# TigreGotico/phoonnx

Measured on AMD Instinct MI355X. Metric: audio samples/sec (22.05 kHz), batch-32 256-phoneme utterances, higher is better.
Workload: dtype f32 (f16x3 split: fp32 operands as two fp16 planes, three MFMA products, fp32 accumulate)

## Files before the change

include/vitsmi.h:

```cpp
#ifndef VITSMI_H
#define VITSMI_H

#include <stddef.h>
#include <stdint.h>

#ifdef __cplusplus
extern "C" {
#endif

typedef struct vits_handle vits_handle;

enum {
    VITS_OK = 0,
    VITS_E_IO = -1,
    VITS_E_FORMAT = -2,
    VITS_E_ARG = -3,
    VITS_E_DEVICE = -4,
    VITS_E_NOMEM = -5,
    VITS_E_RANGE = -6
};

#define VITS_MAX_DIMS 4


// ... 280 lines not shown
                                        vits_enc_chunk_fn fn, void *user);

typedef struct vits_stream_onset {
    int32_t mode;
    float threshold;
    int32_t keep_lead;
    int32_t reserved;
} vits_stream_onset;
typedef int (*vits_enc_chunk_trim_fn)(void *user, const void *bytes, int B, int64_t row_pitch_bytes, int64_t first_sample,
                                      int64_t n_samples, const int32_t *valid, const int32_t *skip, const float *peak,
                                      int64_t total_samples);
int vits_stream_onset_check(const vits_stream_onset *onsets, const vits_stream_format *fmt, int B);
int vits_stream_onset_start(int64_t f, int64_t keep_lead, int64_t delivered_before, int64_t *a);
int vits_run_chunked_enc_trimmed(vits_handle *h, const int64_t *ids, const int64_t *lens, int B, int T, const int64_t *sid,
                                 const vits_noise *noise, const vits_controls *ctl, const vits_stream_format *fmt,
                                 const vits_stream_shaping *shaping, const vits_stream_onset *onsets, int chunk_frames,
                                 vits_enc_chunk_trim_fn fn, void *user);
int vits_run_vocoder_chunked_enc_trimmed(vits_handle *h, const float *z, int B, int F, const int64_t *sid,
                                         const vits_stream_format *fmt, const vits_stream_shaping *shaping,
                                         const vits_stream_onset *onsets, int chunk_frames, vits_enc_chunk_trim_fn fn, void *user);

int vits_warp_emit_end(const vits_warp_seg *segs, int n_segs, int64_t n_in, int64_t n_out, int64_t X, int64_t *ready);
int vits_glide_emit_end(const vits_glide_seg *segs, int n_segs, int64_t n_in, int64_t n_out, int64_t X, int64_t *ready);
int64_t vits_warp_stream_cap(int64_t piece_samples, int64_t S_w);
int vits_run_chunked_glided(vits_handle *h, const int64_t *ids, const int64_t *lens, int B, int T, const int64_t *sid,
                            const vits_noise *noise, const vits_controls *ctl, const vits_contour *contour, int chunk_frames,
                            vits_chunk_fn fn, void *user);
int vits_run_chunked_enc_glided(vits_handle *h, const int64_t *ids, const int64_t *lens, int B, int T, const int64_t *sid,
                                const vits_noise *noise, const vits_controls *ctl, const vits_stream_format *fmt,
                                const vits_stream_shaping *shaping, const vits_stream_onset *onsets, const vits_contour *contour,
                                int chunk_frames, vits_enc_chunk_trim_fn fn, void *user);

enum { VITS_FIT_MET = 0, VITS_FIT_FLOOR = 1, VITS_FIT_CEIL = 2, VITS_FIT_KEPT = 3 };
typedef struct {
    const int32_t *group;
    int n_groups;
    const int64_t *target_frames;
    const int32_t *mode;
} vits_fit;
int vits_fit_plan(const float *w, const int64_t *lens, int B, int T, const vits_fit *fit, int64_t *durations, double *scale,
                  int64_t *frames, int32_t *status);
int vits_run_async_fitted(vits_handle *h, const int64_t *ids, const int64_t *lens, int B, int T, const int64_t *sid,
                          const vits_noise *noise, const vits_controls *ctl, const vits_fit *fit);
int vits_run_chunked_fitted(vits_handle *h, const int64_t *ids, const int64_t *lens, int B, int T, const int64_t *sid,
                            const vits_noise *noise, const vits_controls *ctl, const vits_fit *fit, int chunk_frames,
                            vits_chunk_fn fn, void *user);
int vits_run_chunked_enc_fitted(vits_handle *h, const int64_t *ids, const int64_t *lens, int B, int T, const int64_t *sid,
                                const vits_noise *noise, const vits_controls *ctl, const vits_stream_format *fmt,
                                const vits_stream_shaping *shaping, const vits_stream_onset *onsets, const vits_fit *fit,
                                int chunk_frames, vits_enc_chunk_trim_fn fn, void *user);
int vits_last_fit(vits_handle *h, double *scale, int64_t *frames, int32_t *status, int n);

int vits_reserve(vits_handle *h, int B, int T, int F);
int vits_get_stats(vits_handle *h, vits_stats *out);

typedef struct {
    char kernel[128];
    double flops, bytes;
    float ms;
    int stage;
    int cin, cout, k, dil, t;
} vits_launch_record;
int vits_launch_records(vits_handle *h, vits_launch_record *buf, int n);

void *vits_stream(vits_handle *h);


int vits_test_conv1d(int device_id, const float *x, int B, int Cin, int T, const float *w, const float *bias,
                     int Cout, int K, int dil, int pad_l, int flags, float slope, float *out);
int vits_bench_conv1d(int device_id, int B, int Cin, int Cout, int T, int K, int dil, int hint, int iters,
                      int cfg_override, int ck_override, float *ms_out);
int vits_test_conv_transpose1d(int device_id, const float *x, int B, int Cin, int T, const float *w,
                               const float *bias, int Cout, int K, int stride, float *out);
enum {
    VITS_CONV_PRO_LRELU = 1, VITS_CONV_PRO_MASK = 2, VITS_CONV_EPI_RELU = 4, VITS_CONV_EPI_MASK = 8, VITS_CONV_EPI_RES = 16,
    VITS_CONV_EPI_ACC = 32, VITS_CONV_EPI_DIV = 64, VITS_CONV_EPI_COUPLING = 128, VITS_CONV_EPI_WN = 256,
    VITS_CONV_EPI_WN_FIRST = 512
};
typedef struct {
    int B, Cin, T, Cout;
    int K, dil, pad_l;
    int stride;
    int hint, cfg, ck;
    int flags;
    float slope, div, oslope, oslope2;
    int wn_split;
    const float *x;
    const float *w, *bias;
    const int64_t *lens;
    const float *bias_b;
    int bias_b_stride;
    const float *res;
    int x_cstride;
    int out_cstride;
    int out_rows, out_row0;
    const float *old_out, *old_out2;
    float sentinel;
    float *out, *out2;
    int pl_rows;
    float *planes_out;
    char kernel[128];
    int cfg_used, ck_used;
} vits_test_conv_epi_args;
int vits_test_conv1d_epi(int device_id, vits_test_conv_epi_args *a);
int vits_test_wn_gate(int device_id, const float *a, int B, int H, int T, int form, float *acts);
int vits_test_cond_matvec(int device_id, const float *emb_g, int n_speakers, int gin, const int64_t *sid, int B,
                          const float *W, const float *bias, int rows, float *out);
int vits_test_conv1d_sx(int device_id, const float *x, int B, int Cin, int T, const float *w, const float *bias,
                        int Cout, int K, int dil, int pad_l, int flags, float slope, float *out);
enum { VITS_SX_EPI_RES = 1, VITS_SX_EPI_ACC = 2, VITS_SX_EPI_DIV = 4, VITS_SX_EPI_NO_RAW_STORE = 8 };
enum { VITS_SX_BF16X6 = 0, VITS_SX_F16X3 = 1, VITS_SX_F16 = 2 };
typedef struct {
    int B, Cin, T, Cout;
    int K, dil, pad_l;
    int stride;
    int precision;
    int force16, no_s16, min_cfg;
    int run_cfg;
    int flags;
    const float *x;
    const float *w, *bias;
    const float *res;
    int res_is_x;
    int res_planes;
    float res_slope;
    const float *old_out;
    const float *bias_b;
    int bias_b_stride;
    float div, oslope, oslope2, islope;
    const int64_t *lens;
    int rag_add, rag_mul;
    float sentinel;
    float *out;
    float *planes_out;
    float *res_seen;
    char kernel[128];
    int pack_cfg, run_cfg_used, rawin, s16, ck;
    float peak;
} vits_test_conv_sx_epi_args;
int vits_test_conv1d_sx_epi(int device_id, vits_test_conv_sx_epi_args *a);
int vits_test_conv1d_sx_planar(int device_id, const float *x, int B, int Cin, int T, const float *w, const float *bias,
                               int Cout, int K, int dil, int flags, const int64_t *lens, const float *old, int row_split,
                               int pl_rows, float *out, float *planes_out);
long long vits_test_set_sx_small_max(long long wgs);
int vits_test_conv1d_sx_gate(int device_id, const float *x, int B, int Cin, int T, const float *w, const float *bias,
                             const float *bias_b, int Cout, int K, int dil, int flags, float *out);
int vits_test_conv_transpose1d_sx(int device_id, const float *x, int B, int Cin, int T, const float *w,
                                  const float *bias, int Cout, int K, int stride, float *out);
int vits_bench_conv1d_sx(int device_id, int B, int Cin, int Cout, int T, int K, int dil, int dbg, int iters,
                         float *ms_out);
int vits_test_conv_pair_sx(int device_id, const float *x, int B, int C, int T, const float *w1, const float *b1,
                           const float *w2, const float *b2, int K, int dil1, int dil2, int chain, float slope, float *out,
                           float *ms_out);
enum { VITS_P16_EPI_ACC = 1, VITS_P16_EPI_DIV = 2, VITS_P16_EPI_RAW = 4, VITS_P16_EPI_PLANES = 8 };
typedef struct {
    int B, C, T, K, dil1, dil2, chain;
    int precision;
    int flags;
    float slope, div, sentinel;
    const float *x;
    const float *w1, *b1, *w2, *b2;
    const float *old_out;
    const float *x_tail;
    const int64_t *lens;
    int rag_add, rag_mul;
    float *out;
    float *planes_out;
    float *x_seen;
    float *ms_out;
    char kernel[128];
    int BN, BNo, ovl;
    float peak;
    int guard_ok;
} vits_test_conv_pair16_epi_args;
int vits_test_conv_pair16_epi(int device_id, vits_test_conv_pair16_epi_args *a);
int vits_test_attention(int device_id, const float *qkv, int B, int C, int T, int n_heads, const float *rel_k,
                        const float *rel_v, int window, const int64_t *lens, float *out);
int vits_test_attention16(int device_id, const float *qkv, int B, int C, int T, int n_heads, const float *rel_k,
                          const float *rel_v, int window, const int64_t *lens, float *out, uint16_t *out_planes, int kernel,
                          int reps, float *ms_out);
typedef struct {
    int kernel;
    const float *qkv;
    const uint16_t *qkv_planes;
    int B, C, T, n_heads, window;
    const float *rel_k, *rel_v;
    const int64_t *lens;
    int want_out;
    int want_planes;
    int ns, qt;
    int kh;
    float *out;
    uint16_t *out_planes;
    float peak;
    char kernel_name[128];
} vits_test_attention_form_args;
int vits_test_attention_form(int device_id, vits_test_attention_form_args *a);

int vits_test_resample(int device_id, const float *x, const int64_t *lens, int B, int S, int in_rate, int out_rate, float *y,
                       int64_t S_out);
int vits_test_resample_pieces(int device_id, const float *x, const int64_t *lens, int B, int S, int in_rate, int out_rate,
                              int piece_samples, float *y, int64_t S_out, int64_t *ranges, int max_ranges);
int vits_test_resample_rows(int device_id, const float *x, const int64_t *lens, int B, int S, int in_rate,
                            const int32_t *out_rates, float *y, size_t y_elems, int64_t *n_out);
int vits_test_warp(int device_id, const float *x, const int64_t *counts, int B, int S, const vits_warp_seg *segs,
                   const int32_t *seg_first , float *y, int S_w);
int vits_test_glide(int device_id, const float *x, const int64_t *counts, int B, int S, const vits_glide_seg *segs,
                    const int32_t *seg_first , float *y, int S_w);
int vits_test_warp_pieces(int device_id, const float *x, const int64_t *counts, int B, int S, const vits_warp_seg *segs,
                          const int32_t *seg_first , const int64_t *piece_bounds, int n_pieces, float *y, int S_w,
                          int64_t *ranges, int max_ranges);
int vits_test_glide_pieces(int device_id, const float *x, const int64_t *counts, int B, int S, const vits_glide_seg *segs,
                           const int32_t *seg_first , const int64_t *piece_bounds, int n_pieces, float *y, int S_w,
                           int64_t *ranges, int max_ranges);

int vits_test_durations(int device_id, const float *logw, const int64_t *dur, const int64_t *lens, int B, int T, float length_scale,
                        const float *rows, const float *token_rate, float *w_ceil, int32_t *cum, int32_t *y_len);
int vits_test_fit_durations(int device_id, const float *w, const int64_t *lens, int B, int T, const vits_fit *fit, float *w_ceil,
                            int32_t *cum, int32_t *y_len, double *scale, int64_t *frames, int32_t *status);
int vits_test_expand_prior(int device_id, const float *m_logs, int B, int C, int T, const int32_t *cum, const int64_t *lens,
                           const int32_t *y_len, int F, const float *noise, int64_t noise_stride, int noise_frames,
                           float noise_scale, const float *rows, const uint64_t *seeds, float *z_p);
int vits_test_fill_normal(int device_id, int64_t n, uint64_t seed, uint64_t stream_id, float *out);
int vits_test_fill_normal_rows(int device_id, int B, int channels, int T, const uint64_t *seeds, uint32_t stream, const float *rows,
                               int col, float *out);
int vits_test_post_conv(int device_id, const float *x, int B, int C, int T, const float *w, int K, float slope, const int64_t *vlen,
                        int hop, int kernel, float *out);

int vits_test_layernorm(int device_id, const float *x, const float *out_init, int B, int C, int T, const float *gamma,
                        const float *beta, const int64_t *lens, int flags, int form, int in_place, const float *dw_w,
                        const float *dw_b, int K, int dil, float *out, uint16_t *planes);
typedef struct vits_test_dds_layer {
    const float *dw_w, *dw_b;
    const float *ln1_g, *ln1_b;
    const float *pw_w, *pw_b;
    const float *ln2_g, *ln2_b;
    int32_t dil;
} vits_test_dds_layer;
int vits_test_dds(int device_id, int form, const float *x, int B, int C, int T, const int64_t *lens, int n_layers,
                  const vits_test_dds_layer *layers, int mask_out, const float *head_cond, const float *head_z, int head_ch,
                  const float *head_w, const float *head_b, const float *tail_w, const float *tail_b, int tail_rows, float *out);
int vits_test_cf_pre(int device_id, const float *z, int ch, const float *w, const float *bias, const float *cond, int B, int C, int T,
                     float *out);
int vits_test_rqs_inverse(int device_id, const float *pr, const float *z, int B, int T, const int64_t *lens, int ch0, int nb,
                          float sqrt_c, float *out);
int vits_test_ea_logw(int device_id, const float *z, int ch, float m0, float logs0, const int64_t *lens, int B, int T, float *out);

int vits_test_deliver(int device_id, const float *x, const int64_t *counts, int B, int S, const vits_segment *segs, int n_segs,
                      int n_streams, int encoding, void *dst, size_t dst_bytes, int64_t *stream_samples, int64_t *stream_offsets);

int vits_test_deliver_trimmed(int device_id, const float *x, const int64_t *counts, int B, int S, const vits_segment *segs,
                              const vits_trim *trims, int n_segs, int n_streams, int encoding, void *dst, size_t dst_bytes,
                              int64_t *stream_samples, int64_t *stream_offsets, int64_t *kept_first, int64_t *kept_count);

int vits_test_loudness_blocks(int device_id, const float *x, const int64_t *counts, const int64_t *firsts, int B, int S,
                              int sample_rate, float *e, size_t e_cap, int32_t *n_sub, int32_t *chunk);

int vits_test_deliver_leveled(int device_id, const float *x, const int64_t *counts, int B, int S, const vits_segment *segs,
                              const vits_trim *trims, const vits_level *levels, int n_segs, int n_streams, int encoding,
                              int sample_rate, void *dst, size_t dst_bytes, int64_t *stream_samples, int64_t *stream_offsets,
                              int64_t *kept_first, int64_t *kept_count, double *loudness, float *gain);

int vits_test_deliver_shaped(int device_id, const float *x, const int64_t *counts, int B, int S, const vits_segment *segs,
                             const vits_trim *trims, const vits_level *levels, const vits_shape *shapes, const vits_env_point *points,
                             int64_t n_points, int n_segs, int n_streams, int encoding, int sample_rate, void *dst, size_t dst_bytes,
                             int64_t *stream_samples, int64_t *stream_offsets, int64_t *kept_first, int64_t *kept_count,
                             double *loudness, float *gain);

int vits_test_deliver_limited(int device_id, const float *x, const int64_t *counts, int B, int S, const vits_segment *segs,
                              const vits_trim *trims, const vits_level *levels, const vits_shape *shapes, const vits_env_point *points,
                              int64_t n_points, const vits_limit *limits, int n_segs, int n_streams, int encoding, int sample_rate,
                              void *dst, size_t dst_bytes, int64_t *stream_samples, int64_t *stream_offsets, int64_t *kept_first,
                              int64_t *kept_count, double *loudness, float *gain);

int vits_test_stream_pack(int device_id, const float *x, const int64_t *counts, int B, int S, int piece_samples,
                          const vits_stream_format *fmt, void *bytes, size_t bytes_cap, int64_t *pitches, int32_t *valid,
                          float *peaks, int max_pieces);

int vits_test_stream_pack_shaped(int device_id, const float *x, const int64_t *counts, int B, int S, int piece_samples,
                                 const vits_stream_format *fmt, const vits_stream_shaping *shaping, void *bytes, size_t bytes_cap,
                                 int64_t *pitches, int32_t *valid, float *peaks, int64_t *firsts, int64_t *ns, int max_pieces);

int vits_test_stream_pack_trimmed(int device_id, const float *x, const int64_t *counts, int B, int S, int piece_samples,
                                  const vits_stream_format *fmt, const vits_stream_shaping *shaping, const vits_stream_onset *onsets,
                                  void *bytes, size_t bytes_cap, int64_t *pitches, int32_t *valid, int32_t *skip, float *peaks,
                                  int64_t *firsts, int64_t *ns, int32_t *start, int max_pieces);

#ifdef __cplusplus
}
#endif
#endif
```

phoonnx_amd/_ffi.py:

```python
import ctypes as C
import os

import numpy as np

from . import audio_encoding

_HERE = os.path.dirname(os.path.abspath(__file__))
_LIB = None

VITS_MAX_DIMS = 4


class VitsNoise(C.Structure):
    _fields_ = [("noise_dp", C.c_void_p), ("noise_z", C.c_void_p), ("noise_z_stride", C.c_int64),
                ("seed", C.c_uint64)]


class VitsOutput(C.Structure):
    _fields_ = [("data", C.POINTER(C.c_float)), ("dims", C.c_int64 * 4), ("y_lengths", C.POINTER(C.c_int64))]


class VitsStats(C.Structure):
    _fields_ = [("conv_flops", C.c_double), ("conv_bytes", C.c_double), ("dec_flops", C.c_double),
                ("dec_bytes", C.c_double), ("flow_flops", C.c_double), ("enc_flops", C.c_double),
                ("dp_flops", C.c_double), ("conv_ms", C.c_float), ("dec_ms", C.c_float), ("flow_ms", C.c_float),
                ("enc_ms", C.c_float), ("dp_ms", C.c_float), ("total_ms", C.c_float), ("conv_launches", C.c_int),
                ("total_launches", C.c_int), ("sx_flops", C.c_double), ("sx_ms", C.c_float), ("sx_launches", C.c_int),
                ("f16_peak_max", C.c_float), ("f16_peak_min", C.c_float), ("f16_tracked", C.c_int),
                ("f16_saturated", C.c_int), ("sx_bytes", C.c_double)]


class VitsLaunchRecord(C.Structure):
    _fields_ = [("kernel", C.c_char * 128), ("flops", C.c_double), ("bytes", C.c_double), ("ms", C.c_float),
                ("stage", C.c_int), ("cin", C.c_int), ("cout", C.c_int), ("k", C.c_int), ("dil", C.c_int), ("t", C.c_int)]


class VitsTestConvEpiArgs(C.Structure):
    _fields_ = [(n, C.c_int) for n in ("B", "Cin", "T", "Cout", "K", "dil", "pad_l", "stride", "hint", "cfg", "ck", "flags")] + \
               [(n, C.c_float) for n in ("slope", "div", "oslope", "oslope2")] + [("wn_split", C.c_int)] + \
               [(n, C.c_void_p) for n in ("x", "w", "bias", "lens", "bias_b")] + [("bias_b_stride", C.c_int), ("res", C.c_void_p)] + \
               [(n, C.c_int) for n in ("x_cstride", "out_cstride", "out_rows", "out_row0")] + \
               [("old_out", C.c_void_p), ("old_out2", C.c_void_p), ("sentinel", C.c_float), ("out", C.c_void_p), ("out2", C.c_void_p),
                ("pl_rows", C.c_int), ("planes_out", C.c_void_p), ("kernel", C.c_char * 128), ("cfg_used", C.c_int), ("ck_used", C.c_int)]


class VitsTestConvSxEpiArgs(C.Structure):
    _fields_ = [(n, C.c_int) for n in ("B", "Cin", "T", "Cout", "K", "dil", "pad_l", "stride", "precision", "force16", "no_s16",
                                       "min_cfg", "run_cfg", "flags")] + \
               [(n, C.c_void_p) for n in ("x", "w", "bias", "res")] + \
               [("res_is_x", C.c_int), ("res_planes", C.c_int), ("res_slope", C.c_float), ("old_out", C.c_void_p),
                ("bias_b", C.c_void_p), ("bias_b_stride", C.c_int)] + \
               [(n, C.c_float) for n in ("div", "oslope", "oslope2", "islope")] + \
               [("lens", C.c_void_p), ("rag_add", C.c_int), ("rag_mul", C.c_int), ("sentinel", C.c_float), ("out", C.c_void_p),
                ("planes_out", C.c_void_p), ("res_seen", C.c_void_p), ("kernel", C.c_char * 128)] + \
               [(n, C.c_int) for n in ("pack_cfg", "run_cfg_used", "rawin", "s16", "ck")] + [("peak", C.c_float)]


class VitsTestConvPair16EpiArgs(C.Structure):
    _fields_ = [(n, C.c_int) for n in ("B", "C", "T", "K", "dil1", "dil2", "chain", "precision", "flags")] + \
               [(n, C.c_float) for n in ("slope", "div", "sentinel")] + \
               [(n, C.c_void_p) for n in ("x", "w1", "b1", "w2", "b2", "old_out", "x_tail", "lens")] + \
               [("rag_add", C.c_int), ("rag_mul", C.c_int)] + \
               [(n, C.c_void_p) for n in ("out", "planes_out", "x_seen", "ms_out")] + [("kernel", C.c_char * 128)] + \
               [(n, C.c_int) for n in ("BN", "BNo", "ovl")] + [("peak", C.c_float), ("guard_ok", C.c_int)]


class VitsTestAttentionFormArgs(C.Structure):
    _fields_ = [("kernel", C.c_int), ("qkv", C.c_void_p), ("qkv_planes", C.c_void_p)] + \
               [(n, C.c_int) for n in ("B", "C", "T", "n_heads", "window")] + \
               [(n, C.c_void_p) for n in ("rel_k", "rel_v", "lens")] + \
               [(n, C.c_int) for n in ("want_out", "want_planes", "ns", "qt", "kh")] + \
               [("out", C.c_void_p), ("out_planes", C.c_void_p), ("peak", C.c_float), ("kernel_name", C.c_char * 128)]


class VitsOpenOptions(C.Structure):
    _fields_ = [("device_id", C.c_int), ("gen_precision", C.c_char_p), ("arena_dev", C.c_void_p),
                ("arena_bytes", C.c_size_t), ("host_only", C.c_int), ("layout_only", C.c_int)]


class VitsControls(C.Structure):
    _fields_ = [("scales_rows", C.c_void_p), ("seeds", C.c_void_p), ("durations", C.c_void_p), ("token_rate", C.c_void_p)]


class VitsFit(C.Structure):
    _fields_ = [("group", C.c_void_p), ("n_groups", C.c_int), ("target_frames", C.c_void_p), ("mode", C.c_void_p)]


VITS_FIT_MET, VITS_FIT_FLOOR, VITS_FIT_CEIL, VITS_FIT_KEPT = 0, 1, 2, 3


class VitsWarpSeg(C.Structure):
    _fields_ = [("n0", C.c_int64), ("pos0", C.c_int64), ("k", C.c_int64), ("step", C.c_int32), ("c", C.c_int32),
                ("half_taps", C.c_int32), ("pad_", C.c_int32)]


class VitsIntonation(C.Structure):
    _fields_ = [("token_semitones", C.c_void_p), ("compensate", C.c_int)]


class VitsGlideSeg(C.Structure):
    _fields_ = [("n0", C.c_int64), ("pos0", C.c_int64), ("k", C.c_int64), ("step0", C.c_int32), ("step1", C.c_int32),
                ("pad_", C.c_int32 * 2)]


class VitsContour(C.Structure):
    _fields_ = [("token_semitones", C.c_void_p), ("token_semitones_end", C.c_void_p), ("compensate", C.c_int)]


class VitsSegment(C.Structure):
    _fields_ = [("row", C.c_int32), ("stream", C.c_int32), ("lead_samples", C.c_int64), ("normalize", C.c_int32),
                ("volume", C.c_float)]


class VitsTrim(C.Structure):
    _fields_ = [("mode", C.c_int32), ("threshold", C.c_float), ("keep_lead", C.c_int32), ("keep_tail", C.c_int32),
                ("tail_samples", C.c_int64)]


class VitsTestDdsLayer(C.Structure):
    _fields_ = [("dw_w", C.c_void_p), ("dw_b", C.c_void_p), ("ln1_g", C.c_void_p), ("ln1_b", C.c_void_p), ("pw_w", C.c_void_p),
                ("pw_b", C.c_void_p), ("ln2_g", C.c_void_p), ("ln2_b", C.c_void_p), ("dil", C.c_int32)]


class VitsLevel(C.Structure):
    _fields_ = [("mode", C.c_int32), ("target_lufs", C.c_float), ("max_gain_db", C.c_float), ("peak_ceiling", C.c_float)]


class VitsEnvPoint(C.Structure):
    _fields_ = [("pos", C.c_int32), ("gain", C.c_float)]


class VitsShape(C.Structure):
    _fields_ = [("fade_in", C.c_int32), ("fade_out", C.c_int32), ("curve", C.c_int32), ("n_points", C.c_int32),
                ("first_point", C.c_int64)]


class VitsLimit(C.Structure):
    _fields_ = [("mode", C.c_int32), ("ceiling", C.c_float), ("lookahead", C.c_int32), ("reserved", C.c_int32)]


class VitsStreamFormat(C.Structure):
    _fields_ = [("encoding", C.c_int32), ("ref_peak", C.c_void_p), ("volume", C.c_void_p)]


class VitsStreamShaping(C.Structure):
    pass


STREAM_PLAN_FN = C.CFUNCTYPE(C.c_int, C.c_void_p, C.c_int, C.c_int, C.POINTER(C.c_int64), C.POINTER(C.c_int64), C.POINTER(VitsStreamShaping))

VitsStreamShaping._fields_ = [("shapes", C.c_void_p), ("points", C.c_void_p), ("n_points", C.c_int64), ("ceiling", C.c_void_p),
                              ("lookahead", C.c_int32), ("reserved", C.c_int32), ("plan", STREAM_PLAN_FN), ("plan_user", C.c_void_p)]


class VitsStreamOnset(C.Structure):
    _fields_ = [("mode", C.c_int32), ("threshold", C.c_float), ("keep_lead", C.c_int32), ("reserved", C.c_int32)]


ENCODINGS = {name: (code, audio_encoding.DTYPES[name]) for code, name in enumerate(audio_encoding.ENCODINGS)}


CHUNK_FN = C.CFUNCTYPE(C.c_int, C.c_void_p, C.POINTER(C.c_float), C.c_int, C.c_int64, C.c_int64, C.c_int64)

ENC_CHUNK_FN = C.CFUNCTYPE(C.c_int, C.c_void_p, C.c_void_p, C.c_int, C.c_int64, C.c_int64, C.c_int64, C.POINTER(C.c_int32),
                           C.POINTER(C.c_float), C.c_int64)

ENC_CHUNK_TRIM_FN = C.CFUNCTYPE(C.c_int, C.c_void_p, C.c_void_p, C.c_int, C.c_int64, C.c_int64, C.c_int64, C.POINTER(C.c_int32),
                                C.POINTER(C.c_int32), C.POINTER(C.c_float), C.c_int64)

VITS_E_RANGE = -6


EXPORTS = [
    "vits_open", "vits_open_with_arena", "vits_open_host", "vits_open_layout", "vits_open_opts", "vits_close",
    "vits_run_chunked", "vits_run_vocoder_chunked", "vits_last_error", "vits_num_inputs",
    "vits_input_name", "vits_meta", "vits_hparam", "vits_arena_bytes", "vits_arena_host", "vits_arena_device",
    "vits_run", "vits_free_output", "vits_run_device", "vits_sync", "vits_last_y_lengths", "vits_last_pcm16", "vits_run_vocoder",
    "vits_tap",
    "vits_set_timing", "vits_set_tails", "vits_reserve", "vits_get_stats", "vits_stream", "vits_test_conv1d", "vits_test_conv_transpose1d",
    "vits_test_attention", "vits_test_attention16", "vits_bench_conv1d", "vits_test_conv1d_sx", "vits_test_conv1d_sx_planar", "vits_test_conv1d_sx_gate", "vits_test_set_sx_small_max",
    "vits_test_conv_transpose1d_sx",
    "vits_bench_conv1d_sx", "vits_test_conv_pair_sx", "vits_fetch_output", "vits_run_async", "vits_host_alloc", "vits_host_free",
    "vits_launch_records", "vits_run_async_rows", "vits_run_device_rows", "vits_run_chunked_rows",
    "vits_run_async_ctl", "vits_run_chunked_ctl", "vits_last_durations",
    "vits_set_output_rate", "vits_last_sample_counts", "vits_resample_plan", "vits_test_resample", "vits_test_resample_pieces",
    "vits_set_output_rates", "vits_last_sample_rates", "vits_test_resample_rows",
    "vits_run_async_warped", "vits_last_token_spans", "vits_warp_token", "vits_warp_plan", "vits_test_warp",
    "vits_run_async_glided", "vits_glide_token", "vits_glide_cutoff", "vits_glide_plan", "vits_test_glide",
    "vits_warp_emit_end", "vits_glide_emit_end", "vits_warp_stream_cap", "vits_run_chunked_glided", "vits_run_chunked_enc_glided",
    "vits_test_warp_pieces", "vits_test_glide_pieces",
    "vits_fit_plan", "vits_run_async_fitted", "vits_run_chunked_fitted", "vits_run_chunked_enc_fitted", "vits_last_fit",
    "vits_test_fit_durations",
    "vits_test_durations", "vits_test_expand_prior", "vits_test_fill_normal", "vits_test_fill_normal_rows", "vits_test_post_conv",
    "vits_delivery_plan", "vits_deliver", "vits_test_deliver",
    "vits_trim_range", "vits_delivery_plan_trimmed", "vits_deliver_trimmed", "vits_test_deliver_trimmed",
    "vits_loudness_filter", "vits_loudness_gate", "vits_level_gain", "vits_delivery_plan_leveled", "vits_deliver_leveled",
    "vits_test_loudness_blocks", "vits_test_deliver_leveled",
    "vits_shape_check", "vits_shape_gain", "vits_deliver_shaped", "vits_test_deliver_shaped",
    "vits_limit_check", "vits_limit_gains", "vits_deliver_limited", "vits_test_deliver_limited",
    "vits_run_chunked_enc", "vits_run_vocoder_chunked_enc", "vits_test_stream_pack",
    "vits_stream_shaping_check", "vits_stream_emit_range", "vits_run_chunked_enc_shaped", "vits_run_vocoder_chunked_enc_shaped",
    "vits_test_stream_pack_shaped",
    "vits_stream_onset_check", "vits_stream_onset_start", "vits_run_chunked_enc_trimmed", "vits_run_vocoder_chunked_enc_trimmed",
    "vits_test_stream_pack_trimmed",
    "vits_test_layernorm", "vits_test_dds", "vits_test_cf_pre", "vits_test_rqs_inverse", "vits_test_ea_logw",
    "vits_test_conv1d_epi", "vits_test_wn_gate", "vits_test_cond_matvec", "vits_test_conv1d_sx_epi",
    "vits_test_conv_pair16_epi", "vits_test_attention_form",
]


G2P_EXPORTS = ["g2p_open", "g2p_close", "g2p_last_error", "g2p_hparam", "g2p_num_outputs", "g2p_output_name", "g2p_bucket",
               "g2p_run", "g2p_generate", "g2p_generate_batch", "g2p_test_forced_steps", "g2p_test_linear", "g2p_test_step"]


def lib_path():
    return os.environ.get("VITSMI_LIB") or os.path.join(_HERE, "libvitsmi.so")


def load():
    global _LIB
    if _LIB is not None:
        return _LIB
    path = lib_path()
    if not os.environ.get("VITSMI_LIB"):
        from . import build as _build
        if _build.stale():
            try:
                _build.build()
            except Exception as e:
                raise RuntimeError(f"{path} is missing or was not built from the sources in this tree (source_sha "
                                   f"{_build.source_sha()} vs recorded {_build.read_build_info().get('source_sha')}) "
                                   f"and cannot be rebuilt here: {e}") from e
    lib = C.CDLL(path)
    vp, i64p, f32p = C.c_void_p, C.POINTER(C.c_int64), C.POINTER(C.c_float)
    lib.vits_open.argtypes = [C.c_char_p, C.c_int, C.POINTER(vp)]
    lib.vits_open_with_arena.argtypes = [C.c_char_p, C.c_int, vp, C.c_size_t, C.POINTER(vp)]
    lib.vits_open_host.argtypes = [C.c_char_p, C.POINTER(vp)]
    lib.vits_open_layout.argtypes = [C.c_char_p, C.POINTER(vp)]
    lib.vits_open_opts.argtypes = [C.c_char_p, C.POINTER(VitsOpenOptions), C.POINTER(vp)]
    lib.vits_run_chunked.argtypes = [vp, vp, vp, C.c_int, C.c_int, vp, vp, C.POINTER(VitsNoise), C.c_int, CHUNK_FN, vp]
    lib.vits_run_vocoder_chunked.argtypes = [vp, vp, C.c_int, C.c_int, vp, C.c_int, CHUNK_FN, vp]
    lib.vits_close.argtypes = [vp]
    lib.vits_close.restype = None
    lib.vits_last_error.argtypes = [vp]
    lib.vits_last_error.restype = C.c_char_p
    lib.vits_num_inputs.argtypes = [vp]
    lib.vits_input_name.argtypes = [vp, C.c_int]
    lib.vits_input_name.restype = C.c_char_p
    lib.vits_meta.argtypes = [vp, C.c_char_p, C.c_char_p, C.c_size_t]
    lib.vits_hparam.argtypes = [vp, C.c_char_p, i64p]
    lib.vits_arena_bytes.argtypes = [vp]
    lib.vits_arena_bytes.restype = C.c_size_t
    lib.vits_arena_host.argtypes = [vp]
    lib.vits_arena_host.restype = vp
    lib.vits_arena_device.argtypes = [vp]
    lib.vits_arena_device.restype = vp
    run_args = [vp, vp, vp, C.c_int, C.c_int, vp, vp, C.POINTER(VitsNoise), C.POINTER(VitsOutput)]
    lib.vits_run.argtypes = run_args
    lib.vits_run_device.argtypes = run_args
    lib.vits_run_async.argtypes = run_args[:-1]
    lib.vits_run_async_rows.argtypes = run_args[:-1] + [vp]
    lib.vits_run_device_rows.argtypes = run_args[:-1] + [vp, C.POINTER(VitsOutput)]
    lib.vits_run_chunked_rows.argtypes = [vp, vp, vp, C.c_int, C.c_int, vp, vp, C.POINTER(VitsNoise), vp, C.c_int, CHUNK_FN, vp]
    lib.vits_run_async_ctl.argtypes = [vp, vp, vp, C.c_int, C.c_int, vp, C.POINTER(VitsNoise), C.POINTER(VitsControls)]
    lib.vits_run_chunked_ctl.argtypes = [vp, vp, vp, C.c_int, C.c_int, vp, C.POINTER(VitsNoise), C.POINTER(VitsControls),
                                         C.c_int, CHUNK_FN, vp]
    lib.vits_run_chunked_enc.argtypes = [vp, vp, vp, C.c_int, C.c_int, vp, C.POINTER(VitsNoise), C.POINTER(VitsControls),
                                         C.POINTER(VitsStreamFormat), C.c_int, ENC_CHUNK_FN, vp]
    lib.vits_run_vocoder_chunked_enc.argtypes = [vp, vp, C.c_int, C.c_int, vp, C.POINTER(VitsStreamFormat), C.c_int, ENC_CHUNK_FN, vp]
    lib.vits_stream_shaping_check.argtypes = [C.POINTER(VitsStreamShaping), C.POINTER(VitsStreamFormat), C.c_int]
    lib.vits_stream_emit_range.argtypes = [C.c_int64, C.c_int64, C.c_int, C.c_int64, C.c_int, i64p, i64p]
    lib.vits_run_chunked_enc_shaped.argtypes = [vp, vp, vp, C.c_int, C.c_int, vp, C.POINTER(VitsNoise), C.POINTER(VitsControls),
                                                C.POINTER(VitsStreamFormat), C.POINTER(VitsStreamShaping), C.c_int, ENC_CHUNK_FN, vp]
    lib.vits_run_vocoder_chunked_enc_shaped.argtypes = [vp, vp, C.c_int, C.c_int, vp, C.POINTER(VitsStreamFormat),
                                                        C.POINTER(VitsStreamShaping), C.c_int, ENC_CHUNK_FN, vp]
    lib.vits_test_stream_pack_shaped.argtypes = [C.c_int, vp, vp, C.c_int, C.c_int, C.c_int, C.POINTER(VitsStreamFormat),
                                                 C.POINTER(VitsStreamShaping), vp, C.c_size_t, vp, vp, vp, vp, vp, C.c_int]
    lib.vits_stream_onset_check.argtypes = [C.POINTER(VitsStreamOnset), C.POINTER(VitsStreamFormat), C.c_int]
    lib.vits_stream_onset_start.argtypes = [C.c_int64, C.c_int64, C.c_int64, i64p]
    lib.vits_run_chunked_enc_trimmed.argtypes = [vp, vp, vp, C.c_int, C.c_int, vp, C.POINTER(VitsNoise), C.POINTER(VitsControls),
                                                 C.POINTER(VitsStreamFormat), C.POINTER(VitsStreamShaping), C.POINTER(VitsStreamOnset),
                                                 C.c_int, ENC_CHUNK_TRIM_FN, vp]
    lib.vits_run_vocoder_chunked_enc_trimmed.argtypes = [vp, vp, C.c_int, C.c_int, vp, C.POINTER(VitsStreamFormat),
                                                         C.POINTER(VitsStreamShaping), C.POINTER(VitsStreamOnset), C.c_int,
                                                         ENC_CHUNK_TRIM_FN, vp]
    lib.vits_test_stream_pack_trimmed.argtypes = [C.c_int, vp, vp, C.c_int, C.c_int, C.c_int, C.POINTER(VitsStreamFormat),
                                                  C.POINTER(VitsStreamShaping), C.POINTER(VitsStreamOnset), vp, C.c_size_t, vp, vp, vp, vp,
                                                  vp, vp, vp, C.c_int]
    lib.vits_test_stream_pack.argtypes = [C.c_int, vp, vp, C.c_int, C.c_int, C.c_int, C.POINTER(VitsStreamFormat), vp, C.c_size_t,
                                          vp, vp, vp, C.c_int]
    lib.vits_last_durations.argtypes = [vp, i64p, C.c_size_t]
    lib.vits_set_output_rate.argtypes = [vp, C.c_int, C.c_int]
    lib.vits_last_sample_counts.argtypes = [vp, i64p, C.c_int]
    lib.vits_resample_plan.argtypes = [C.c_int, C.c_int, i64p, i64p, i64p, vp, C.c_size_t]
    lib.vits_test_resample.argtypes = [C.c_int, vp, vp, C.c_int, C.c_int, C.c_int, C.c_int, vp, C.c_int64]
    lib.vits_test_resample_pieces.argtypes = [C.c_int, vp, vp, C.c_int, C.c_int, C.c_int, C.c_int, C.c_int, vp, C.c_int64, vp, C.c_int]
    lib.vits_set_output_rates.argtypes = [vp, C.c_int, vp, C.c_int]
    lib.vits_last_sample_rates.argtypes = [vp, vp, C.c_int]
    lib.vits_test_resample_rows.argtypes = [C.c_int, vp, vp, C.c_int, C.c_int, C.c_int, vp, vp, C.c_size_t, vp]
    lib.vits_run_async_warped.argtypes = [vp, vp, vp, C.c_int, C.c_int, vp, C.POINTER(VitsNoise), C.POINTER(VitsControls),
                                          C.POINTER(VitsIntonation)]
    lib.vits_last_token_spans.argtypes = [vp, i64p, C.c_size_t]
    lib.vits_warp_token.argtypes = [C.c_float, i64p, i64p, C.POINTER(C.c_int32)]
    lib.vits_warp_plan.argtypes = [vp, vp, C.c_int, C.c_int, vp, vp, i64p]
    lib.vits_test_warp.argtypes = [C.c_int, vp, vp, C.c_int, C.c_int, vp, vp, vp, C.c_int]
    lib.vits_run_async_glided.argtypes = [vp, vp, vp, C.c_int, C.c_int, vp, C.POINTER(VitsNoise), C.POINTER(VitsControls),
                                          C.POINTER(VitsContour)]
    lib.vits_glide_token.argtypes = [C.c_float, C.c_float, i64p, i64p, C.POINTER(C.c_float)]
    lib.vits_glide_cutoff.argtypes = [C.c_int64, i64p, C.POINTER(C.c_int32)]
    lib.vits_glide_plan.argtypes = [vp, vp, vp, C.c_int, C.c_int, vp, vp, i64p]
    lib.vits_test_glide.argtypes = [C.c_int, vp, vp, C.c_int, C.c_int, vp, vp, vp, C.c_int]
    for name in ("vits_warp_emit_end", "vits_glide_emit_end"):
        getattr(lib, name).argtypes = [vp, C.c_int, C.c_int64, C.c_int64, C.c_int64, i64p]
    lib.vits_warp_stream_cap.argtypes = [C.c_int64, C.c_int64]
    lib.vits_warp_stream_cap.restype = C.c_int64
    lib.vits_run_chunked_glided.argtypes = [vp, vp, vp, C.c_int, C.c_int, vp, C.POINTER(VitsNoise), C.POINTER(VitsControls),
                                            C.POINTER(VitsContour), C.c_int, CHUNK_FN, vp]
    lib.vits_run_chunked_enc_glided.argtypes = [vp, vp, vp, C.c_int, C.c_int, vp, C.POINTER(VitsNoise), C.POINTER(VitsControls),
                                                C.POINTER(VitsStreamFormat), C.POINTER(VitsStreamShaping), C.POINTER(VitsStreamOnset),
                                                C.POINTER(VitsContour), C.c_int, ENC_CHUNK_TRIM_FN, vp]
    for name in ("vits_test_warp_pieces", "vits_test_glide_pieces"):
        getattr(lib, name).argtypes = [C.c_int, vp, vp, C.c_int, C.c_int, vp, vp, vp, C.c_int, vp, C.c_int, vp, C.c_int]
    lib.vits_fit_plan.argtypes = [vp, vp, C.c_int, C.c_int, C.POINTER(VitsFit), vp, vp, vp, vp]
    lib.vits_run_async_fitted.argtypes = [vp, vp, vp, C.c_int, C.c_int, vp, C.POINTER(VitsNoise), C.POINTER(VitsControls),
                                          C.POINTER(VitsFit)]
    lib.vits_run_chunked_fitted.argtypes = [vp, vp, vp, C.c_int, C.c_int, vp, C.POINTER(VitsNoise), C.POINTER(VitsControls),
                                            C.POINTER(VitsFit), C.c_int, CHUNK_FN, vp]
    lib.vits_run_chunked_enc_fitted.argtypes = [vp, vp, vp, C.c_int, C.c_int, vp, C.POINTER(VitsNoise), C.POINTER(VitsControls),
                                                C.POINTER(VitsStreamFormat), C.POINTER(VitsStreamShaping), C.POINTER(VitsStreamOnset),
                                                C.POINTER(VitsFit), C.c_int, ENC_CHUNK_TRIM_FN, vp]
    lib.vits_last_fit.argtypes = [vp, vp, vp, vp, C.c_int]
    lib.vits_test_fit_durations.argtypes = [C.c_int, vp, vp, C.c_int, C.c_int, C.POINTER(VitsFit), vp, vp, vp, vp, vp, vp]
    lib.vits_test_durations.argtypes = [C.c_int, vp, vp, vp, C.c_int, C.c_int, C.c_float, vp, vp, vp, vp, vp]
    lib.vits_test_expand_prior.argtypes = [C.c_int, vp, C.c_int, C.c_int, C.c_int, vp, vp, vp, C.c_int, vp, C.c_int64, C.c_int,
                                           C.c_float, vp, vp, vp]
    lib.vits_test_fill_normal.argtypes = [C.c_int, C.c_int64, C.c_uint64, C.c_uint64, vp]
    lib.vits_test_fill_normal_rows.argtypes = [C.c_int, C.c_int, C.c_int, C.c_int, vp, C.c_uint32, vp, C.c_int, vp]
    lib.vits_test_post_conv.argtypes = [C.c_int, vp, C.c_int, C.c_int, C.c_int, vp, C.c_int, C.c_float, vp, C.c_int, C.c_int, vp]
    lib.vits_test_layernorm.argtypes = [C.c_int, vp, vp, C.c_int, C.c_int, C.c_int, vp, vp, vp, C.c_int, C.c_int, C.c_int, vp, vp,
                                        C.c_int, C.c_int, vp, vp]
    lib.vits_test_dds.argtypes = [C.c_int, C.c_int, vp, C.c_int, C.c_int, C.c_int, vp, C.c_int, C.POINTER(VitsTestDdsLayer), C.c_int,
                                  vp, vp, C.c_int, vp, vp, vp, vp, C.c_int, vp]
    lib.vits_test_cf_pre.argtypes = [C.c_int, vp, C.c_int, vp, vp, vp, C.c_int, C.c_int, C.c_int, vp]
    lib.vits_test_rqs_inverse.argtypes = [C.c_int, vp, vp, C.c_int, C.c_int, vp, C.c_int, C.c_int, C.c_float, vp]
    lib.vits_test_ea_logw.argtypes = [C.c_int, vp, C.c_int, C.c_float, C.c_float, vp, C.c_int, C.c_int, vp]
    lib.vits_delivery_plan.argtypes = [vp, C.c_int, vp, C.c_int, C.c_int, C.c_int, vp, vp, i64p]
    lib.vits_deliver.argtypes = [vp, vp, C.c_int, C.c_int, C.c_int, vp, C.c_size_t, vp, vp]
    lib.vits_test_deliver.argtypes = [C.c_int, vp, vp, C.c_int, C.c_int, vp, C.c_int, C.c_int, C.c_int, vp, C.c_size_t, vp, vp]
    lib.vits_trim_range.argtypes = [C.c_int64, C.c_int64, C.c_int64, C.POINTER(VitsTrim), i64p, i64p]
    lib.vits_delivery_plan_trimmed.argtypes = [vp, C.c_int, vp, vp, C.c_int, C.c_int, C.c_int, vp, vp, i64p]
    lib.vits_deliver_trimmed.argtypes = [vp, vp, vp, C.c_int, C.c_int, C.c_int, vp, C.c_size_t, vp, vp, vp, vp]
    lib.vits_test_deliver_trimmed.argtypes = [C.c_int, vp, vp, C.c_int, C.c_int, vp, vp, C.c_int, C.c_int, C.c_int, vp, C.c_size_t,
                                              vp, vp, vp, vp]
    lib.vits_loudness_filter.argtypes = [C.c_int, vp, vp]
    lib.vits_loudness_gate.argtypes = [vp, vp, C.c_int, C.c_int32, vp, vp, vp, vp]
    lib.vits_level_gain.argtypes = [C.c_double, C.c_float, C.POINTER(VitsLevel), C.POINTER(C.c_float)]
    lib.vits_delivery_plan_leveled.argtypes = [vp, C.c_int, vp, vp, vp, C.c_int, C.c_int, C.c_int, C.c_int, vp, vp, i64p]
    lib.vits_deliver_leveled.argtypes = [vp, vp, vp, vp, C.c_int, C.c_int, C.c_int, C.c_int, vp, C.c_size_t, vp, vp, vp, vp, vp, vp]
    lib.vits_test_loudness_blocks.argtypes = [C.c_int, vp, vp, vp, C.c_int, C.c_int, C.c_int, vp, C.c_size_t, vp, vp]
    lib.vits_test_deliver_leveled.argtypes = [C.c_int, vp, vp, C.c_int, C.c_int, vp, vp, vp, C.c_int, C.c_int, C.c_int, C.c_int, vp,
                                              C.c_size_t, vp, vp, vp, vp, vp, vp]
    lib.vits_shape_check.argtypes = [vp, C.c_int, vp, C.c_int64]
    lib.vits_shape_gain.argtypes = [C.POINTER(VitsShape), vp, C.c_int64, C.c_int64, C.c_int64, C.POINTER(C.c_float)]
    lib.vits_deliver_shaped.argtypes = [vp, vp, vp, vp, vp, vp, C.c_int64, C.c_int, C.c_int, C.c_int, C.c_int, vp, C.c_size_t, vp, vp, vp,
                                        vp, vp, vp]
    lib.vits_test_deliver_shaped.argtypes = [C.c_int, vp, vp, C.c_int, C.c_int, vp, vp, vp, vp, vp, C.c_int64, C.c_int, C.c_int, C.c_int,
                                             C.c_int, vp, C.c_size_t, vp, vp, vp, vp, vp, vp]
    lib.vits_limit_check.argtypes = [vp, vp, C.c_int]
    lib.vits_limit_gains.argtypes = [vp, C.c_int64, C.POINTER(VitsLimit), vp]
    lib.vits_deliver_limited.argtypes = [vp, vp, vp, vp, vp, vp, C.c_int64, vp, C.c_int, C.c_int, C.c_int, C.c_int, vp, C.c_size_t, vp,
                                         vp, vp, vp, vp, vp]
    lib.vits_test_deliver_limited.argtypes = [C.c_int, vp, vp, C.c_int, C.c_int, vp, vp, vp, vp, vp, C.c_int64, vp, C.c_int, C.c_int,
                                              C.c_int, C.c_int, vp, C.c_size_t, vp, vp, vp, vp, vp, vp]
    lib.vits_free_output.argtypes = [vp, C.POINTER(VitsOutput)]
    lib.vits_free_output.restype = None
    lib.vits_sync.argtypes = [vp]
    lib.vits_last_y_lengths.argtypes = [vp, i64p, C.c_int]
    lib.vits_last_pcm16.argtypes = [vp, C.c_int, C.c_float, vp, C.c_size_t]
    lib.vits_run_vocoder.argtypes = [vp, vp, C.c_int, C.c_int, vp, C.POINTER(VitsOutput)]
    lib.vits_tap.argtypes = [vp, C.c_char_p, vp, C.c_size_t, i64p]
    lib.vits_set_timing.argtypes = [vp, C.c_int]
    lib.vits_set_tails.argtypes = [vp, C.c_int]
    lib.vits_reserve.argtypes = [vp, C.c_int, C.c_int, C.c_int]
    lib.vits_get_stats.argtypes = [vp, C.POINTER(VitsStats)]
    lib.vits_stream.argtypes = [vp]
    lib.vits_stream.restype = vp
    lib.vits_fetch_output.argtypes = [vp, vp, C.c_size_t, C.c_size_t]
    lib.vits_host_alloc.argtypes = [C.c_size_t]
    lib.vits_host_alloc.restype = vp
    lib.vits_host_free.argtypes = [vp]
    lib.vits_host_free.restype = None
    lib.vits_launch_records.argtypes = [vp, C.POINTER(VitsLaunchRecord), C.c_int]
    lib.vits_test_conv1d.argtypes = [C.c_int, vp, C.c_int, C.c_int, C.c_int, vp, vp, C.c_int, C.c_int, C.c_int,
                                     C.c_int, C.c_int, C.c_float, vp]
    lib.vits_test_conv_transpose1d.argtypes = [C.c_int, vp, C.c_int, C.c_int, C.c_int, vp, vp, C.c_int, C.c_int,
                                               C.c_int, vp]
    lib.vits_test_attention.argtypes = [C.c_int, vp, C.c_int, C.c_int, C.c_int, C.c_int, vp, vp, C.c_int, vp, vp]
    lib.vits_test_attention16.argtypes = [C.c_int, vp, C.c_int, C.c_int, C.c_int, C.c_int, vp, vp, C.c_int, vp, vp, vp,
                                          C.c_int, C.c_int, f32p]
    lib.vits_bench_conv1d.argtypes = [C.c_int] * 11 + [f32p]
    lib.vits_test_conv1d_sx.argtypes = lib.vits_test_conv1d.argtypes
    lib.vits_test_conv_transpose1d_sx.argtypes = lib.vits_test_conv_transpose1d.argtypes
    lib.vits_test_conv1d_sx_planar.argtypes = [C.c_int, vp, C.c_int, C.c_int, C.c_int, vp, vp, C.c_int, C.c_int, C.c_int, C.c_int,
                                               vp, vp, C.c_int, C.c_int, vp, vp]
    lib.vits_test_set_sx_small_max.argtypes = [C.c_longlong]
    lib.vits_test_set_sx_small_max.restype = C.c_longlong
    lib.vits_test_conv1d_sx_gate.argtypes = [C.c_int, vp, C.c_int, C.c_int, C.c_int, vp, vp, vp, C.c_int, C.c_int, C.c_int, C.c_int, vp]
    lib.vits_bench_conv1d_sx.argtypes = [C.c_int] * 9 + [f32p]
    lib.vits_test_conv1d_epi.argtypes = [C.c_int, C.POINTER(VitsTestConvEpiArgs)]
    lib.vits_test_conv1d_sx_epi.argtypes = [C.c_int, C.POINTER(VitsTestConvSxEpiArgs)]
    lib.vits_test_conv_pair16_epi.argtypes = [C.c_int, C.POINTER(VitsTestConvPair16EpiArgs)]
    lib.vits_test_attention_form.argtypes = [C.c_int, C.POINTER(VitsTestAttentionFormArgs)]
    lib.vits_test_wn_gate.argtypes = [C.c_int, vp, C.c_int, C.c_int, C.c_int, C.c_int, vp]
    lib.vits_test_cond_matvec.argtypes = [C.c_int, vp, C.c_int, C.c_int, vp, C.c_int, vp, vp, C.c_int, vp]
    lib.vits_test_conv_pair_sx.argtypes = [C.c_int, vp, C.c_int, C.c_int, C.c_int, vp, vp, vp, vp, C.c_int, C.c_int,
                                           C.c_int, C.c_int, C.c_float, vp, f32p]
    lib.g2p_open.argtypes = [C.c_char_p, C.c_int, C.POINTER(vp)]
    lib.g2p_close.argtypes = [vp]
    lib.g2p_close.restype = None
    lib.g2p_last_error.argtypes = [vp]
    lib.g2p_last_error.restype = C.c_char_p
    lib.g2p_hparam.argtypes = [vp, C.c_char_p, i64p]
    lib.g2p_num_outputs.argtypes = [vp]
    lib.g2p_output_name.argtypes = [vp, C.c_int]
    lib.g2p_output_name.restype = C.c_char_p
    lib.g2p_bucket.argtypes = [vp, C.c_int, C.c_int]
    lib.g2p_run.argtypes = [vp, vp, C.c_int, vp, vp, C.c_int, vp]
    lib.g2p_generate.argtypes = [vp, vp, C.c_int, C.c_int, C.c_int64, C.c_int64, vp, C.POINTER(C.c_int)]
    lib.g2p_generate_batch.argtypes = [vp, vp, vp, C.c_int, C.c_int, C.c_int64, C.c_int64, vp, vp]
    lib.g2p_test_forced_steps.argtypes = [vp, vp, vp, C.c_int, vp, C.c_int, vp]
    lib.g2p_test_linear.argtypes = [C.c_int, C.c_int, vp, vp, C.c_int, vp, C.c_int, C.c_int, vp, C.c_int64, C.c_int64, C.c_int, vp]
    lib.g2p_test_step.argtypes = [C.c_int, C.c_int, C.c_int, vp, vp, vp, C.c_int, vp, vp, C.c_int, C.c_float, C.c_float, vp, vp]
    _LIB = lib
    return lib


def ptr(a):
    return None if a is None else a.ctypes.data_as(C.c_void_p)


def last_error(h=None):
    return load().vits_last_error(h).decode("utf-8", "replace")
```

phoonnx_amd/csrc/conv_sx_pair.hip.hpp:

```cpp
#pragma once
#include <cstdlib>
#include "conv_geom.hpp"
#include "conv_sx_engine.hip.hpp"

namespace vitsmi {

struct SxPairArgs {
    const float *xr;
    float islope, mslope;
    int T;
    const u32x4 *wp1, *wp2;
    const float *bias1, *bias2;
    float wscale1, wscale2;
    float *out_raw;
    const float *zeros;
    int C, nchunks;
    int K1, dil1, pad1;
    int K2, dil2, pad2;
    int LW1;
    unsigned x_bytes;
    int LW2;
    unsigned y_chunk_bytes;
    int BNo, NT, B;
    int flags;
    float div;
    unsigned *peak;
    struct Chain {
        const u32x4 *wp1, *wp2;
        const float *bias1, *bias2;
        float wscale1, wscale2;
        int K1, dil1, K2, dil2;
        int xoff, yoff;
    } ch[3];
    int nchain;
    unsigned a_ring;
    unsigned bias_off;
    unsigned long long *prof;
    SxRagged rag;
    int xgs = 0;
};

#ifndef SX_PAIR_PROF
#define SX_PAIR_PROF 0
#endif
#ifndef SX_PAIR_SHARED_A
#define SX_PAIR_SHARED_A 0
#endif
#ifndef SX_PAIR_ALIAS
#define SX_PAIR_ALIAS 0
#endif
#ifndef SX_PAIR_DEPTH32
#define SX_PAIR_DEPTH32 2
#endif
#ifndef SX_PAIR_DEPTH64
#define SX_PAIR_DEPTH64 2
#endif
#ifndef SX_PAIR_EARLY_ACC
#define SX_PAIR_EARLY_ACC 0
#endif
#ifndef SX_PAIR_WGS32
#define SX_PAIR_WGS32 3
#endif
#ifndef SX_PAIR_EARLY32
#define SX_PAIR_EARLY32 1
#endif
#ifndef SX_PAIR_ST_SC1
#define SX_PAIR_ST_SC1 0
#endif
#ifndef SX_PAIR_ONE_READ64
#define SX_PAIR_ONE_READ64 1
#endif
#ifndef SX_PAIR_ONE_READ32
#define SX_PAIR_ONE_READ32 1
#endif
template <int MW, int NW, int WM, int WN, int EPI, bool CHAIN, int NCH = 1>
__global__ __launch_bounds__(256, (NW == 2 && !SX_PAIR_EARLY_ACC && NCH == 1) ? SX_PAIR_WGS32 : 2) void conv_sx_pair_kernel(SxPairArgs a) {
    constexpr int BN = NW * WN * 32, NH = NW / 2;
    static_assert(NCH == 1 || (CHAIN && NW == 2 && (EPI & EPI_ACC) == 0), "fused chains: 32 channels, no external running sum");
    constexpr bool ONE_READ = NW == 4 ? SX_PAIR_ONE_READ64 != 0 : SX_PAIR_ONE_READ32 != 0;
    constexpr bool EARLY = ONE_READ || (NW == 2 && SX_PAIR_EARLY32);
    constexpr int DEPTH = NW == 2 ? SX_PAIR_DEPTH32 : SX_PAIR_DEPTH64;
    static_assert(DEPTH >= 2 && DEPTH <= 6, "wait_a covers up to five younger sets");
    constexpr bool ACC = (EPI & EPI_ACC) != 0 && SX_PAIR_EARLY_ACC;
    static_assert(!(ONE_READ && ACC), "the running sum is not pulled into the single-read prologue");
    static_assert(WM * WN == 4 && MW == 1 && BN == 256, "one block row per wave, 256 columns");
    constexpr int NPW = 2, STEPBYTES = WM * MW * NPW * 1024;
    constexpr int MAXCH = WM * 2;
    extern __shared__ __attribute__((aligned(16))) unsigned char lds_sx[];
    const int tid = threadIdx.x, lane = tid & 63;
    const int wave = __builtin_amdgcn_readfirstlane(tid >> 6);
    const int wm = wave / WN, wn = wave % WN;
    const int l31 = lane & 31, hi = lane >> 5;
    const int wg_xcd = blockIdx.x & 7, wg_seq = blockIdx.x >> 3;
    const int tile_nb = __builtin_amdgcn_readfirstlane(sx_xcd_tile(wg_seq, wg_xcd, a.xgs));
    if (tile_nb >= a.NT * a.B) return;
    const int b = tile_nb / a.NT, t0 = (tile_nb - b * a.NT) * a.BNo;
    const int t1 = t0 - a.pad2;
    const int T = a.T, LW = a.LW1;
    const int TV = __builtin_amdgcn_readfirstlane(sx_valid_cols(a.rag, b, T));
    if (t0 >= TV) return;
    const uint32_t lds0 = (uint32_t)(uintptr_t)lds_sx;
    const uint32_t XB = a.x_bytes;
    const char *wbase1 = reinterpret_cast<const char *>(a.wp1) + wm * (MW * NPW * 1024);
    const char *wbase2 = reinterpret_cast<const char *>(a.wp2) + wm * (MW * NPW * 1024);
    const float *xrb = a.xr + (int64_t)b * a.C * T;
    float pk = 0.f;

    struct ASet {
        u32x4 fa[2];
    };
    const uint32_t voff0 = (uint32_t)lane * 16u;
    auto load_a = [&](ASet &f, const char *wb, int step) {
        const char *sb = wb + (int64_t)step * STEPBYTES;
        f.fa[0] = global_read128<0>(voff0, sb);
        f.fa[1] = global_read128<1024>(voff0, sb);
    };

    f32x4 pre[NW / 2][2][4], ad[EARLY && ACC ? NW / 2 : 1][2][4];
    auto load_res = [&](const float *base, f32x4 (*dst)[2][4]) {
        static_for<NW / 2>([&](auto R) {
            constexpr int rr = decltype(R)::value;
#pragma unroll
            for (int j = 0; j < 2; j++) {
                const int row0 = wm * 32;
                const int t = t1 + (wn * NW + rr * 2 + j) * 32 + l31;
                const int tl = t < 0 ? 0 : (t < T ? t : T - 1);
#pragma unroll
                for (int q = 0; q < 4; q++) {
                    const float *p = base + ((int64_t)((row0 >> 3) + q) * T + tl) * 8 + 4 * hi;
                    if constexpr (EARLY) dst[rr][j][q] = __builtin_bit_cast(f32x4, global_read128_v<0>(p));
                    else dst[rr][j][q] = *reinterpret_cast<const f32x4 *>(p);
                }
            }
        });
    };
    auto load_pre = [&]() { load_res(xrb, pre); };

#if SX_PAIR_PROF
    auto stamp = [&]() {
        unsigned long long t;
        __builtin_amdgcn_sched_barrier(0);
        asm volatile("s_memtime %0\n\ts_waitcnt lgkmcnt(0)" : "=s"(t)::"memory");
        __builtin_amdgcn_sched_barrier(0);
        return t;
    };
    unsigned long long tp[8];
    tp[0] = stamp();
#endif
    if constexpr (NW == 2 && WM == 1 && NCH == 1 && SX_PAIR_SHARED_A != 0)
        for (int g = 0; g < 3; g++)
            if (g < ((a.nchunks * a.K1) >> 1)) {
                const int sub = wave >> 1, pl = wave & 1;
                lds_dma<16>(wbase1 + (int64_t)(2 * g + sub) * STEPBYTES + pl * 1024 + lane * 16,
                            reinterpret_cast<float *>(lds_sx + a.a_ring + (unsigned)((g * 2 + sub) * 2048 + pl * 1024)));
            }
    constexpr bool BIAS_LDS = NCH == 1;
    if constexpr (BIAS_LDS) {
        if (wave == 0) {
            constexpr int CC = WM * 32;
            const int k = lane - (lane >= CC / 4 ? CC / 4 : 0);
            const float *bp = lane < CC / 4 ? a.bias1 : a.bias2;
            const void *src = (bp && lane < CC / 2) ? static_cast<const void *>(bp + 4 * k) : static_cast<const void *>(a.zeros + 4 * (lane & 31));
            lds_dma<16>(src, reinterpret_cast<float *>(lds_sx + a.bias_off));
        }
    }
    auto bias_from_lds = [&](int conv, f32x4 (&bq)[4]) __attribute__((always_inline)) {
        u32x4 t4[4];
#pragma unroll
        for (int q = 0; q < 4; q++)
            asm volatile("ds_read_b128 %0, %1" : "=v"(t4[q]) : "v"(lds0 + a.bias_off + (uint32_t)(conv * (WM * 32) + wm * 32 + 8 * q + 4 * hi) * 4u) : "memory");
        asm volatile("s_waitcnt lgkmcnt(0)" ::: "memory");
        __builtin_amdgcn_sched_barrier(0);
#pragma unroll
        for (int q = 0; q < 4; q++) bq[q] = __builtin_bit_cast(f32x4, t4[q]);
    };
    constexpr int NXC = 3;
    if constexpr (ONE_READ) {
        constexpr int NXH = MAXCH, NG = 2 * MAXCH;
        const int HW = LW - 256, pad1 = a.pad1;
        const int nhc = HW * NG, nxh = (nhc + 255) >> 8;
        u32x4 hst[NXH][2];
        bool hin[NXH], hok[NXH];
        uint32_t hlds[NXH];
        const float *hp[NXH];
#pragma unroll
        for (int it = 0; it < NXH; it++) {
            const int h = it * 256 + tid;
            hin[it] = h < nhc;
            const int g = hin[it] ? h / HW : 0;
            const int c = hin[it] ? h - g * HW : 0;
            const int col = c < pad1 ? c : c + 256;
            const int t = t1 - pad1 + col;
            hok[it] = hin[it] && t >= 0 && t < TV;
            hp[it] = xrb + (hok[it] ? ((int64_t)g * T + t) * 8 : (int64_t)0);
            hlds[it] = lds0 + (uint32_t)(g >> 1) * XB + (uint32_t)((g & 1) * LW + col) * 16u;
        }
        static_for<NXH>([&](auto I) {
            constexpr int it = decltype(I)::value;
            if (it < nxh) {
                hst[it][0] = global_read128_v<0>(hp[it]);
                hst[it][1] = global_read128_v<16>(hp[it]);
            }
        });
        load_pre();
        const float isl = a.islope;
        static_for<NW>([&](auto N) {
            constexpr int n = decltype(N)::value;
            asm volatile("s_waitcnt vmcnt(%0)" ::"n"(4 * (NW - 1 - n)) : "memory");
            __builtin_amdgcn_sched_barrier(0);
#if SX_PAIR_PROF
            if constexpr (n == 0) tp[1] = stamp();
#endif
            if constexpr (n == 0) {
                static_for<NXH>([&](auto I) {
                    constexpr int it = decltype(I)::value;
                    if (it < nxh && hin[it]) {
                        float v[8];
#pragma unroll
                        for (int e = 0; e < 8; e++) {
                            const float x = hok[it] ? __uint_as_float(hst[it][e >> 2][e & 3]) : 0.f;
                            v[e] = fmaxf(x, x * isl);
                        }
                        unsigned p0[4], p1[4];
#pragma unroll
                        for (int e = 0; e < 4; e++) split2h_pair_pk(v[2 * e], v[2 * e + 1], p0[e], p1[e], pk);
                        ds_write128(hlds[it], u32x4{p0[0], p0[1], p0[2], p0[3]});
                        ds_write128(hlds[it] + (uint32_t)(2 * LW) * 16u, u32x4{p1[0], p1[1], p1[2], p1[3]});
                    }
                });
            }
            const int col = (wn * NW + n) * 32 + l31;
            const int t = t1 + col;
            const bool ok = t >= 0 && t < TV;
#pragma unroll
            for (int q = 0; q < 4; q++) {
                float v[4];
#pragma unroll
                for (int e = 0; e < 4; e++) {
                    const float x = ok ? pre[n / 2][n % 2][q][e] : 0.f;
                    v[e] = fmaxf(x, x * isl);
                }
                unsigned wa[2], wb[2];
                split2h_pair_pk(v[0], v[1], wa[0], wa[1], pk);
                split2h_pair_pk(v[2], v[3], wb[0], wb[1], pk);
                const int g = 4 * wm + q;
                const uint32_t cell = lds0 + (uint32_t)(g >> 1) * XB + (uint32_t)((g & 1) * LW + pad1 + col) * 16u + 8u * hi;
                asm volatile("ds_write_b64 %0, %1" ::"v"(cell), "v"(u32x2{wa[0], wb[0]}) : "memory");
                asm volatile("ds_write_b64 %0, %1" ::"v"(cell + (uint32_t)(2 * LW) * 16u), "v"(u32x2{wa[1], wb[1]}) : "memory");
            }
            asm volatile("" : "+v"(pk));
        });
    } else {
        u32x4 xst[MAXCH][NXC][2];
        const int nxc = (2 * LW + 255) >> 8;
        uint32_t xroff[NXC];
        bool xrok[NXC];
        int xkh[NXC], xcol[NXC];
#pragma unroll
        for (int it = 0; it < NXC; it++) {
            const int i = it * 256 + tid;
            const int kh = (i >= LW ? 1 : 0) + (i >= 2 * LW ? 1 : 0);
            const int col = i - kh * LW;
            const int t = t1 - a.pad1 + col;
            xkh[it] = kh;
            xcol[it] = col;
            xrok[it] = it < nxc && kh < 2 && t >= 0 && t < TV;
            xroff[it] = xrok[it] ? (uint32_t)(((int64_t)kh * T + t) * 32) : 0u;
        }
        static_for<MAXCH>([&](auto CH) {
            constexpr int ch = decltype(CH)::value;
            const float *cbase = xrb + (int64_t)(2 * ch) * T * 8;
            static_for<NXC>([&](auto I) {
                constexpr int it = decltype(I)::value;
                if (it < nxc) {
                    xst[ch][it][0] = global_read128_x<0>(xroff[it], cbase);
                    xst[ch][it][1] = global_read128_x<16>(xroff[it], cbase);
                }
            });
        });
        if constexpr (EARLY) {
            load_pre();
            if constexpr (ACC) {
                load_res(a.out_raw + (int64_t)b * a.C * T, ad);
                asm volatile("s_waitcnt vmcnt(16)" ::: "memory");
            } else
                asm volatile("s_waitcnt vmcnt(8)" ::: "memory");
        } else
            asm volatile("s_waitcnt vmcnt(0)" ::: "memory");
#if SX_PAIR_PROF
        tp[1] = stamp();
#endif
        const float isl = a.islope;
        static_for<MAXCH>([&](auto CH) {
            constexpr int ch = decltype(CH)::value;
            static_for<NXC>([&](auto I) {
                constexpr int it = decltype(I)::value;
                if (it < nxc && xkh[it] < 2) {
                    float v[8];
#pragma unroll
                    for (int e = 0; e < 8; e++) {
                        const float x = xrok[it] ? __uint_as_float(xst[ch][it][e >> 2][e & 3]) : 0.f;
                        v[e] = fmaxf(x, x * isl);
                    }
                    unsigned p0[4], p1[4];
#pragma unroll
                    for (int e = 0; e < 4; e++) split2h_pair_pk(v[2 * e], v[2 * e + 1], p0[e], p1[e], pk);
                    const uint32_t ad = lds0 + (uint32_t)ch * XB + (uint32_t)(xkh[it] * LW + xcol[it]) * 16u;
                    ds_write128(ad, u32x4{p0[0], p0[1], p0[2], p0[3]});
                    ds_write128(ad + (uint32_t)(2 * LW) * 16u, u32x4{p1[0], p1[1], p1[2], p1[3]});
                }
            });
        });
    }

    f32x16 acc[NW];
    auto zero_acc = [&]() {
#pragma unroll
        for (int n = 0; n < NW; n++)
#pragma unroll
            for (int r = 0; r < 16; r++) acc[n][r] = 0.f;
    };
    zero_acc();
    u32x4 fb[NW][2];
    auto load_b_half = [&](auto H, uint32_t rows, uint32_t pstride) {
        constexpr int h = decltype(H)::value;
        static_for<NH>([&](auto N) {
            constexpr int n = h * NH + decltype(N)::value;
            fb[n][0] = ds_read128<n * 512>(rows);
            fb[n][1] = ds_read128<n * 512>(rows + pstride);
        });
    };
    auto mma_half = [&](const ASet &f, auto H) {
        constexpr int h = decltype(H)::value;
#pragma unroll
        for (int c = 0; c < 3; c++)
#pragma unroll
            for (int n = h * NH; n < (h + 1) * NH; n++) {
                const f16x8 ga = c == 0 ? __builtin_bit_cast(f16x8, f.fa[1])
                                        : (c == 1 ? __builtin_bit_cast(f16x8, f.fa[0]) * (_Float16)0.00048828125f
                                                  : __builtin_bit_cast(f16x8, f.fa[0]));
                const f16x8 gb = __builtin_bit_cast(f16x8, fb[n][c == 1 ? 1 : 0]);
                acc[n] = __builtin_amdgcn_mfma_f32_32x32x16_f16(ga, gb, acc[n], 0, 0, 0);
            }
    };
    auto wait_lds_older_half = [&]() {
        if constexpr (NH * 2 == 2) asm volatile("s_waitcnt lgkmcnt(2)" ::: "memory");
        else asm volatile("s_waitcnt lgkmcnt(4)" ::: "memory");
    };
    const std::integral_constant<int, 0> H0{};
    const std::integral_constant<int, 1> H1{};

    auto wait_a = [&](int younger) {
        switch (younger) {
            case 0: asm volatile("s_waitcnt vmcnt(0)" ::: "memory"); break;
            case 1: asm volatile("s_waitcnt vmcnt(2)" ::: "memory"); break;
            case 2: asm volatile("s_waitcnt vmcnt(4)" ::: "memory"); break;
            case 3: asm volatile("s_waitcnt vmcnt(6)" ::: "memory"); break;
            case 4: asm volatile("s_waitcnt vmcnt(8)" ::: "memory"); break;
            default: asm volatile("s_waitcnt vmcnt(10)" ::: "memory"); break;
        }
    };
    auto run_conv = [&](ASet(&fs)[DEPTH + 1], const char *wb, int K, int dil, uint32_t rows0, uint32_t chunk_bytes,
                        uint32_t pstride) {
        constexpr int NS = DEPTH + 1;
        const int S = a.nchunks * K;
        int chunk = 0, tap = 0;
        static_for<DEPTH - 1>([&](auto I) {
            constexpr int i = decltype(I)::value + 1;
            if (i < S) load_a(fs[i], wb, i);
        });
        load_b_half(H0, rows0, pstride);
        load_b_half(H1, rows0, pstride);
        auto step = [&](ASet &fc, ASet &fload, int s) {
            const int left = S - 1 - s;
            wait_a(left < DEPTH - 1 ? left : DEPTH - 1);
            __builtin_amdgcn_sched_barrier(0);
            if (s + DEPTH < S && !SX_NOA) load_a(fload, wb, s + DEPTH);
            int ntap = tap + 1, nchunk = chunk;
            if (ntap == K) {
                ntap = 0;
                nchunk++;
            }
            const bool more = s + 1 < S;
            const uint32_t next = rows0 + (uint32_t)nchunk * chunk_bytes + (uint32_t)(ntap * dil) * 16u;
            __builtin_amdgcn_sched_barrier(0);
            wait_lds_older_half();
            __builtin_amdgcn_sched_barrier(0);
            mma_half(fc, H0);
            __builtin_amdgcn_sched_barrier(0);
            if (more) {
                load_b_half(H0, next, pstride);
                wait_lds_older_half();
            } else
                asm volatile("s_waitcnt lgkmcnt(0)" ::: "memory");
            __builtin_amdgcn_sched_barrier(0);
            mma_half(fc, H1);
            __builtin_amdgcn_sched_barrier(0);
            if (more) load_b_half(H1, next, pstride);
            __builtin_amdgcn_sched_barrier(0);
            tap = ntap;
            chunk = nchunk;
        };
        int s = 0;
        for (; s + NS <= S; s += NS)
            static_for<NS>([&](auto I) {
                constexpr int i = decltype(I)::value;
                step(fs[i], fs[(i + DEPTH) % NS], s + i);
            });
        __builtin_amdgcn_sched_barrier(0);
        asm volatile("s_waitcnt lgkmcnt(0)" ::: "memory");
        __builtin_amdgcn_sched_barrier(0);
        static_for<NS - 1>([&](auto I) {
            constexpr int i = decltype(I)::value;
            if (s + i < S) step(fs[i], fs[(i + DEPTH) % NS], s + i);
        });
    };

    constexpr bool SHA = NW == 2 && WM == 1 && NCH == 1 && SX_PAIR_SHARED_A != 0;
    constexpr int RG = 3;
    auto sha_dma = [&](const char *wb, int g) {
        const int sub = wave >> 1, pl = wave & 1;
        const char *src = wb + (int64_t)(2 * g + sub) * STEPBYTES + pl * 1024 + lane * 16;
        lds_dma<16>(src, reinterpret_cast<float *>(lds_sx + a.a_ring + (unsigned)(((g % RG) * 2 + sub) * 2048 + pl * 1024)));
    };
    auto sha_prefetch = [&](const char *wb, int K) {
        const int NG = (a.nchunks * K) >> 1;
#pragma unroll
        for (int g = 0; g < RG; g++)
            if (g < NG) sha_dma(wb, g);
    };
    auto wait_vm_le = [&](int n) {
        switch (n) {
            case 0: asm volatile("s_waitcnt vmcnt(0)" ::: "memory"); break;
            case 1: asm volatile("s_waitcnt vmcnt(1)" ::: "memory"); break;
            default: asm volatile("s_waitcnt vmcnt(2)" ::: "memory"); break;
        }
    };
    auto run_conv_sha = [&](ASet &fa0, ASet &fa1, const char *wb, int K, int dil, uint32_t rows0, uint32_t chunk_bytes,
                            uint32_t pstride) {
        const int S = a.nchunks * K, NG = S >> 1;
        const uint32_t alds = lds0 + a.a_ring + (uint32_t)lane * 16u;
        auto read_a = [&](ASet &f, int st) {
            const uint32_t ad = alds + (uint32_t)((((st >> 1) % RG) * 2 + (st & 1)) * 2048);
            f.fa[0] = ds_read128<0>(ad);
            f.fa[1] = ds_read128<1024>(ad);
        };
        int chunk = 0, tap = 0;
        wait_vm_le((NG < RG ? NG : RG) - 1);
        __builtin_amdgcn_s_barrier();
        __builtin_amdgcn_sched_barrier(0);
        read_a(fa0, 0);
        load_b_half(H0, rows0, pstride);
        load_b_half(H1, rows0, pstride);
        auto step = [&](ASet &fc, ASet &fload, int st, bool boundary) {
            int ntap = tap + 1, nchunk = chunk;
            if (ntap == K) {
                ntap = 0;
                nchunk++;
            }
            const bool more = st + 1 < S;
            const uint32_t next = rows0 + (uint32_t)nchunk * chunk_bytes + (uint32_t)(ntap * dil) * 16u;
            __builtin_amdgcn_sched_barrier(0);
            wait_lds_older_half();
            __builtin_amdgcn_sched_barrier(0);
            mma_half(fc, H0);
            __builtin_amdgcn_sched_barrier(0);
            if (more) {
                if (boundary && NG > RG) {
                    const int g = st >> 1;
                    const int last = g + RG - 1 < NG - 1 ? g + RG - 1 : NG - 1;
                    wait_vm_le(last - (g + 1));
                    __builtin_amdgcn_s_barrier();
                    __builtin_amdgcn_sched_barrier(0);
                    if (g + RG < NG) sha_dma(wb, g + RG);
                }
                read_a(fload, st + 1);
                load_b_half(H0, next, pstride);
                asm volatile("s_waitcnt lgkmcnt(4)" ::: "memory");
            } else
                asm volatile("s_waitcnt lgkmcnt(0)" ::: "memory");
            __builtin_amdgcn_sched_barrier(0);
            mma_half(fc, H1);
            __builtin_amdgcn_sched_barrier(0);
            if (more) load_b_half(H1, next, pstride);
            __builtin_amdgcn_sched_barrier(0);
            tap = ntap;
            chunk = nchunk;
        };
        for (int g = 0; g < NG; g++) {
            step(fa0, fa1, 2 * g, false);
            step(fa1, fa0, 2 * g + 1, true);
        }
    };

    struct ChainPar {
        const char *wb1, *wb2;
        const float *bias1, *bias2;
        float ws1, ws2;
        int K1, dil1, K2, dil2;
        uint32_t xoff, yoff;
    };
    auto chain_par = [&](int ci) {
        ChainPar c;
        if constexpr (NCH == 1) {
            c = ChainPar{wbase1, wbase2, a.bias1, a.bias2, a.wscale1, a.wscale2, a.K1, a.dil1, a.K2, a.dil2, 0u, 0u};
        } else {
            const auto &h = a.ch[ci];
            c = ChainPar{reinterpret_cast<const char *>(h.wp1) + wm * (MW * NPW * 1024),
                         reinterpret_cast<const char *>(h.wp2) + wm * (MW * NPW * 1024),
                         h.bias1, h.bias2, h.wscale1, h.wscale2, h.K1, h.dil1, h.K2, h.dil2, (uint32_t)h.xoff, (uint32_t)h.yoff};
        }
        return c;
    };
    static_assert(NCH == 1 || EARLY, "fused chains keep x in registers from the prologue on");
    const uint32_t ylds = NCH > 1 ? lds0 + (uint32_t)a.nchunks * XB : lds0;
    f32x4 xkeep[NCH > 1 ? NW / 2 : 1][2][4], tot[NCH > 1 ? NW / 2 : 1][2][4];
#if SX_PAIR_ALIAS
    ASet f1s[DEPTH + 1];
    ASet(&f2s)[DEPTH + 1] = f1s;
#else
    ASet f1s[DEPTH + 1], f2s[DEPTH + 1];
#endif
#pragma unroll 1
    for (int ci = 0; ci < NCH; ci++) {
    const ChainPar cp = chain_par(ci);
    if constexpr (NCH > 1) {
        if (ci > 0) {
#pragma unroll
            for (int rr = 0; rr < NW / 2; rr++)
#pragma unroll
                for (int j = 0; j < 2; j++)
#pragma unroll
                    for (int q = 0; q < 4; q++) pre[rr][j][q] = xkeep[rr][j][q];
            zero_acc();
        }
    }
    if constexpr (!SHA) load_a(f1s[0], cp.wb1, 0);
    if (ci == 0) {
        asm volatile("s_waitcnt lgkmcnt(0)" ::: "memory");
#if SX_PAIR_PROF
        tp[2] = stamp();
#endif
        __builtin_amdgcn_s_barrier();
#if SX_PAIR_PROF
        tp[3] = stamp();
#endif
    }
    __builtin_amdgcn_sched_barrier(0);
    if constexpr (SHA)
        run_conv_sha(f1s[0], f1s[1], cp.wb1, cp.K1, cp.dil1, lds0 + (uint32_t)(hi * LW + wn * (NW * 32) + l31 + (int)cp.xoff) * 16u,
                     XB, (uint32_t)(2 * LW) * 16u);
    else
        run_conv(f1s, cp.wb1, cp.K1, cp.dil1, lds0 + (uint32_t)(hi * LW + wn * (NW * 32) + l31 + (int)cp.xoff) * 16u, XB,
                 (uint32_t)(2 * LW) * 16u);

#if SX_PAIR_PROF
    tp[4] = stamp();
#endif
    if constexpr (CHAIN && !EARLY) load_pre();

    if constexpr (!SHA) load_a(f2s[0], cp.wb2, 0);
    asm volatile("s_waitcnt lgkmcnt(0)" ::: "memory");
    __builtin_amdgcn_s_barrier();
    __builtin_amdgcn_sched_barrier(0);
    if constexpr (SHA) sha_prefetch(cp.wb2, cp.K2);
    {
        const float wsc = cp.ws1, msl = a.mslope;
        const float *biasp = cp.bias1 ? cp.bias1 : a.zeros;
        const int b_on = cp.bias1 ? 1 : 0;
        const uint32_t YC = a.y_chunk_bytes, LW2 = (uint32_t)a.LW2;
        const int row0 = wm * 32;
        f32x4 bq[4];
        if constexpr (BIAS_LDS) bias_from_lds(0, bq);
        else {
#pragma unroll
            for (int q = 0; q < 4; q++) bq[q] = *reinterpret_cast<const f32x4 *>(biasp + (row0 + 8 * q + 4 * hi) * b_on);
        }
#pragma unroll
        for (int n = 0; n < NW; n++) {
            const int col = (wn * NW + n) * 32 + l31;
            const int t = t1 + col;
            const bool live = t >= 0 && t < TV;
#pragma unroll
            for (int q = 0; q < 4; q++) {
                float o[4];
#pragma unroll
                for (int e = 0; e < 4; e++) {
                    float v = __builtin_fmaf(acc[n][4 * q + e], wsc, bq[q][e]);
                    if constexpr (CHAIN) {
                        if constexpr (NCH > 1) {
                            if (ci == 0) xkeep[n / 2][n % 2][q][e] = pre[n / 2][n % 2][q][e];
                        }
                        v += pre[n / 2][n % 2][q][e];
                        pre[n / 2][n % 2][q][e] = v;
                    }
                    o[e] = live ? fmaxf(v, v * msl) : 0.f;
                }
                unsigned wa[2], wb[2];
                split2h_pair_pk(o[0], o[1], wa[0], wa[1], pk);
                split2h_pair_pk(o[2], o[3], wb[0], wb[1], pk);
                const int g = 4 * wm + q;
                const uint32_t cell = ylds + (uint32_t)(g >> 1) * YC + ((uint32_t)(g & 1) * LW2 + (uint32_t)(col + a.pad2)) * 16u + 8u * hi;
                asm volatile("ds_write_b64 %0, %1" ::"v"(cell), "v"(u32x2{wa[0], wb[0]}) : "memory");
                asm volatile("ds_write_b64 %0, %1" ::"v"(cell + 2u * LW2 * 16u), "v"(u32x2{wa[1], wb[1]}) : "memory");
            }
            asm volatile("" : "+v"(pk));
        }
    }
    zero_acc();
    asm volatile("s_waitcnt lgkmcnt(0)" ::: "memory");
    __builtin_amdgcn_s_barrier();
    __builtin_amdgcn_sched_barrier(0);
#if SX_PAIR_PROF
    tp[5] = stamp();
#endif

    if constexpr (SHA)
        run_conv_sha(f2s[0], f2s[1], cp.wb2, cp.K2, cp.dil2, ylds + (uint32_t)(hi * a.LW2 + wn * (NW * 32) + l31 + (int)cp.yoff) * 16u,
                     a.y_chunk_bytes, (uint32_t)(2 * a.LW2) * 16u);
    else
        run_conv(f2s, cp.wb2, cp.K2, cp.dil2, ylds + (uint32_t)(hi * a.LW2 + wn * (NW * 32) + l31 + (int)cp.yoff) * 16u,
                 a.y_chunk_bytes, (uint32_t)(2 * a.LW2) * 16u);
#if SX_PAIR_PROF
    tp[6] = stamp();
#endif
    if constexpr (!CHAIN && !EARLY) load_pre();

    {
        constexpr int flags = EPI;
        float *rawb = a.out_raw + (int64_t)b * a.C * T;
        const float wsc = cp.ws2, rdiv = a.div;
        const float *biasp = cp.bias2 ? cp.bias2 : a.zeros;
        const int b_on = cp.bias2 ? 1 : 0;
        const int row0 = wm * 32;
        f32x4 bq[4];
        if constexpr (BIAS_LDS) bias_from_lds(1, bq);
        else {
#pragma unroll
            for (int q = 0; q < 4; q++) bq[q] = *reinterpret_cast<const f32x4 *>(biasp + (row0 + 8 * q + 4 * hi) * b_on);
        }
        static_for<NW / 2>([&](auto R) {
            constexpr int rr = decltype(R)::value;
            f32x4 adl[2][4];
            if constexpr ((flags & EPI_ACC) != 0 && !(EARLY && ACC)) {
#pragma unroll
                for (int j = 0; j < 2; j++) {
                    const int t = t1 + (wn * NW + rr * 2 + j) * 32 + l31;
                    const int tl = t < 0 ? 0 : (t < T ? t : T - 1);
#pragma unroll
                    for (int q = 0; q < 4; q++)
                        adl[j][q] = *reinterpret_cast<const f32x4 *>(rawb + ((int64_t)((row0 >> 3) + q) * T + tl) * 8 + 4 * hi);
                }
            }
#pragma unroll
            for (int j = 0; j < 2; j++) {
                const int n = rr * 2 + j;
                const int col = (wn * NW + n) * 32 + l31;
                const int t = t1 + col;
                const bool kept = !(col < a.pad2 || col >= a.pad2 + a.BNo || t >= TV);
                if constexpr (NCH == 1) {
                    if (!kept) continue;
                }
#pragma unroll
                for (int q = 0; q < 4; q++) {
                    f32x4 v;
#pragma unroll
                    for (int e = 0; e < 4; e++) v[e] = __builtin_fmaf(acc[n][4 * q + e], wsc, bq[q][e]);
                    v += pre[rr][j][q];
                    if constexpr (NCH > 1) {
                        if (ci > 0) v += tot[rr][j][q];
                        tot[rr][j][q] = v;
                        if (ci < NCH - 1 || !kept) continue;
                    }
                    if constexpr ((flags & EPI_ACC) != 0) {
                        if constexpr (EARLY && ACC) v += ad[rr][j][q];
                        else v += adl[j][q];
                    }
                    if constexpr ((flags & EPI_DIV) != 0) {
#pragma unroll
                        for (int e = 0; e < 4; e++) v[e] = v[e] / rdiv;
                    }
#if SX_PAIR_ST_SC1
                    {
                        float *sp = rawb + ((int64_t)((row0 >> 3) + q) * T + t) * 8 + 4 * hi;
                        const f32x4 sv = v;
                        asm volatile("global_store_dwordx4 %0, %1, off sc1" ::"v"(sp), "v"(sv) : "memory");
                    }
#else
                    *reinterpret_cast<f32x4 *>(rawb + ((int64_t)((row0 >> 3) + q) * T + t) * 8 + 4 * hi) = v;
#endif
                }
            }
        });
    }
    }
#if SX_PAIR_PROF
    asm volatile("s_waitcnt vmcnt(0)" ::: "memory");
    tp[7] = stamp();
    if (a.prof && tid == 0) {
        for (int i = 0; i < 7; i++) atomicAdd(a.prof + i, tp[i + 1] - tp[i]);
        atomicAdd(a.prof + 7, 1ull);
    }
#endif
    if (a.peak) sx_publish_peak(a.peak, (int)blockIdx.x, pk);
}

template <int MW, int NW, int WM, int WN, int EPI, bool CHAIN, int NCH = 1>
inline hipError_t launch_conv_sx_pair_k(const SxPairArgs &a, dim3 grid, size_t lds, hipStream_t stream) {
    static std::atomic<uint64_t> attr_done{0};
    auto kern = conv_sx_pair_kernel<MW, NW, WM, WN, EPI, CHAIN, NCH>;
    if (hipError_t e = sx_allow_big_lds(reinterpret_cast<const void *>(kern), attr_done); e != hipSuccess) return e;
    if (g_launch_name_on)
        snprintf(g_launch_name, sizeof g_launch_name, "conv_sx_pair_kernel<%d, %d, %d, %d, %d, %s, %d>", MW, NW, WM, WN, EPI,
                 CHAIN ? "true" : "false", NCH);
    kern<<<grid, 256, lds, stream>>>(a);
    return hipGetLastError();
}

inline bool sx_pair_supported(int C, int cfg, int K1, int dil1, int K2, int dil2) {
    if (K1 < 3 || K2 < 3 || dil1 < 1 || dil2 < 1) return false;
    if (!((C == 64 && cfg == 1) || (C == 32 && cfg == 2))) return false;
    const int LW1 = 256 + (K1 - 1) * dil1;
    if (2 * LW1 > kSxRawStageCells) return false;
    const int halo2 = (K2 - 1) * dil2;
    static const int keep_min = [] {
        const char *e = std::getenv("VITSMI_PAIR_MIN_KEEP");
        return e ? std::atoi(e) : 160;
    }();
    if (halo2 % 2 || 256 - halo2 < keep_min) return false;
    static const int keep64 = [] {
        const char *e = std::getenv("VITSMI_PAIR_MIN_KEEP64");
        return e ? std::atoi(e) : 200;
    }();
    if (C == 64 && 256 - halo2 < keep64) return false;
    const size_t lds_y = (size_t)(C / 16) * 4 * (size_t)((256 + halo2 / 2 + 7) / 8 * 8) * 16 + (size_t)(halo2 / 2) * 16;
    const size_t lds_x = (size_t)(C / 16) * 4 * LW1 * 16;
    return (lds_y > lds_x ? lds_y : lds_x) <= kLdsTwoPerCu;
}

hipError_t launch_conv_sx_pair(SxPairArgs a, int cfg, int B, hipStream_t stream, bool chain = false);
hipError_t launch_conv_sx_mrf(SxPairArgs a, int B, hipStream_t stream);
#ifdef VITSMI_IMPL_PAIR
hipError_t launch_conv_sx_pair(SxPairArgs a, int cfg, int B, hipStream_t stream, bool chain) {
    a.LW1 = 256 + (a.K1 - 1) * a.dil1;
    a.x_bytes = (unsigned)((size_t)4 * a.LW1 * 16);
    if (a.dil2 < 1) a.dil2 = 1;
    const int halo2 = (a.K2 - 1) * a.dil2;
    if (a.pad2 * 2 != halo2) return hipErrorInvalidValue;
    a.LW2 = (256 + a.pad2 + 7) / 8 * 8;
    a.y_chunk_bytes = (unsigned)(4 * a.LW2 * 16);
    a.BNo = 256 - halo2;
    a.NT = (a.T + a.BNo - 1) / a.BNo;
    a.B = B;
    a.nchunks = a.C / 16;
    if (a.islope == 0.f) a.islope = 1.f;
    if (a.mslope == 0.f) a.mslope = 1.f;
    if (a.wscale1 == 0.f) a.wscale1 = 1.f;
    if (a.wscale2 == 0.f) a.wscale2 = 1.f;
    if ((long long)a.T * 64 + 64 >= (1ll << 32)) return hipErrorInvalidValue;
    const size_t lds_x = (size_t)a.nchunks * a.x_bytes, lds_y = (size_t)a.nchunks * a.y_chunk_bytes + (size_t)a.pad2 * 16;
    size_t lds = lds_x > lds_y ? lds_x : lds_y;
    if (lds > kLdsTwoPerCu || !sx_pair_supported(a.C, cfg, a.K1, a.dil1, a.K2, a.dil2)) return hipErrorInvalidValue;
    if (cfg != 1 && SX_PAIR_SHARED_A) {
        a.a_ring = (unsigned)((lds + 1023) / 1024 * 1024);
        lds = a.a_ring + 3 * 4096;
    }
    a.bias_off = (unsigned)((lds + 15) / 16 * 16);
    lds = a.bias_off + 1024;
    const long long nb = (long long)a.NT * B;
    if (nb == 0) return hipSuccess;
    a.xgs = a.NT >= (2 << sx_xcd_group_shift()) ? sx_xcd_group_shift() : 0;
    const long long per_round = 8ll << a.xgs;
    const long long wgs = (nb + per_round - 1) / per_round * per_round;
    if (wgs >= (1ll << 31)) return hipErrorInvalidValue;
    dim3 grid((unsigned)wgs, 1, 1);
    const int epi = a.flags & (EPI_ACC | EPI_DIV);
    if ((epi & EPI_DIV) && !(epi & EPI_ACC)) return hipErrorInvalidValue;
#define SX_PAIR_CASES(MW, NW, WM, WN, CH)                                                                        \
    switch (epi) {                                                                                               \
        case 0: return launch_conv_sx_pair_k<MW, NW, WM, WN, 0, CH>(a, grid, lds, stream);                       \
        case EPI_ACC: return launch_conv_sx_pair_k<MW, NW, WM, WN, EPI_ACC, CH>(a, grid, lds, stream);           \
        default: return launch_conv_sx_pair_k<MW, NW, WM, WN, EPI_ACC | EPI_DIV, CH>(a, grid, lds, stream);      \
    }
    if (cfg == 1) {
        if (chain) {
            SX_PAIR_CASES(1, 4, 2, 2, true)
        }
        SX_PAIR_CASES(1, 4, 2, 2, false)
    }
    if (chain) {
        SX_PAIR_CASES(1, 2, 1, 4, true)
    }
    SX_PAIR_CASES(1, 2, 1, 4, false)
#undef SX_PAIR_CASES
}
#endif

struct SxMrfGeom {
    int pad1, pad2, LW1, LW2;
    size_t lds;
};
inline bool sx_mrf_geom(int C, int n, const int *K1, const int *dil1, const int *K2, const int *dil2, SxMrfGeom *g) {
    if (C != 32 || n < 2 || n > 3) return false;
    int p1 = 0, p2 = 0;
    for (int i = 0; i < n; i++) {
        if (K1[i] < 3 || K2[i] < 3 || !(K1[i] & 1) || !(K2[i] & 1) || dil1[i] < 1 || dil2[i] < 1) return false;
        const int a1 = (K1[i] - 1) / 2 * dil1[i], a2 = (K2[i] - 1) / 2 * dil2[i];
        p1 = a1 > p1 ? a1 : p1;
        p2 = a2 > p2 ? a2 : p2;
    }
    const int LW1 = 256 + 2 * p1;
    if (2 * LW1 > kSxRawStageCells) return false;
    if (256 - 2 * p2 < 160) return false;
    const int LW2 = (256 + p2 + 7) / 8 * 8;
    const size_t lds = (size_t)(C / 16) * 4 * LW1 * 16 + (size_t)(C / 16) * 4 * LW2 * 16 + (size_t)p2 * 16;
    if (lds > kLdsTwoPerCu) return false;
    if (g) *g = SxMrfGeom{p1, p2, LW1, LW2, lds};
    return true;
}

#ifdef VITSMI_IMPL_PAIR
hipError_t launch_conv_sx_mrf(SxPairArgs a, int B, hipStream_t stream) {
    int K1[3], d1[3], K2[3], d2[3];
    if (a.nchain < 2 || a.nchain > 3) return hipErrorInvalidValue;
    for (int i = 0; i < a.nchain; i++) {
        K1[i] = a.ch[i].K1;
        d1[i] = a.ch[i].dil1;
        K2[i] = a.ch[i].K2;
        d2[i] = a.ch[i].dil2;
    }
    SxMrfGeom g;
    if (!sx_mrf_geom(a.C, a.nchain, K1, d1, K2, d2, &g)) return hipErrorInvalidValue;
    for (int i = 0; i < a.nchain; i++) {
        a.ch[i].xoff = g.pad1 - (K1[i] - 1) / 2 * d1[i];
        a.ch[i].yoff = g.pad2 - (K2[i] - 1) / 2 * d2[i];
        if (a.ch[i].wscale1 == 0.f) a.ch[i].wscale1 = 1.f;
        if (a.ch[i].wscale2 == 0.f) a.ch[i].wscale2 = 1.f;
    }
    a.pad1 = g.pad1;
    a.pad2 = g.pad2;
    a.LW1 = g.LW1;
    a.x_bytes = (unsigned)((size_t)4 * a.LW1 * 16);
    a.LW2 = g.LW2;
    a.y_chunk_bytes = (unsigned)(4 * a.LW2 * 16);
    a.BNo = 256 - 2 * g.pad2;
    a.NT = (a.T + a.BNo - 1) / a.BNo;
    a.B = B;
    a.nchunks = a.C / 16;
    if (a.islope == 0.f) a.islope = 1.f;
    if (a.mslope == 0.f) a.mslope = 1.f;
    if ((long long)a.T * 64 + 64 >= (1ll << 32)) return hipErrorInvalidValue;
    const long long nb = (long long)a.NT * B;
    if (nb == 0) return hipSuccess;
    a.xgs = a.NT >= (2 << sx_xcd_group_shift()) ? sx_xcd_group_shift() : 0;
    const long long per_round = 8ll << a.xgs;
    const long long wgs = (nb + per_round - 1) / per_round * per_round;
// ... 10 lines not shown
```

phoonnx_amd/csrc/sx_split.hip.hpp:

```cpp
#pragma once
#include <hip/hip_runtime.h>
#include <stdint.h>

#include <atomic>

#include "conv_geom.hpp"

namespace vitsmi {

typedef float sxf32x2 __attribute__((ext_vector_type(2)));
typedef _Float16 f16x2 __attribute__((ext_vector_type(2)));
typedef unsigned u32x4 __attribute__((ext_vector_type(4)));
typedef unsigned u32x2 __attribute__((ext_vector_type(2)));

constexpr int kSxPeakSlots = 64;
constexpr float kF16Max = 65504.f;

inline thread_local bool g_launch_name_on = false;
inline thread_local char g_launch_name[128];

__device__ __forceinline__ unsigned cvt_pk_f16(float lo, float hi) {
    const sxf32x2 v = {lo, hi};
    return __builtin_bit_cast(unsigned, __builtin_convertvector(v, f16x2));
}
__device__ __forceinline__ void split2h_pair(float x, float y, unsigned &w0, unsigned &w1) {
    x = __builtin_amdgcn_fmed3f(x, -65504.f, 65504.f);
    y = __builtin_amdgcn_fmed3f(y, -65504.f, 65504.f);
    w0 = cvt_pk_f16(x, y);
    const f16x2 h = __builtin_bit_cast(f16x2, w0);
    w1 = cvt_pk_f16((x - (float)h[0]) * 2048.f, (y - (float)h[1]) * 2048.f);
}
__device__ __forceinline__ void split2h_pair_pk(float x, float y, unsigned &w0, unsigned &w1, float &pk) {
    pk = __builtin_fmaxf(pk, __builtin_fmaxf(__builtin_fabsf(x), __builtin_fabsf(y)));
    split2h_pair(x, y, w0, w1);
}
__device__ __forceinline__ unsigned cvt1h_pair_pk(float x, float y, float &pk) {
    pk = __builtin_fmaxf(pk, __builtin_fmaxf(__builtin_fabsf(x), __builtin_fabsf(y)));
    return cvt_pk_f16(__builtin_amdgcn_fmed3f(x, -65504.f, 65504.f), __builtin_amdgcn_fmed3f(y, -65504.f, 65504.f));
}
__device__ __forceinline__ void unact4h(u32x2 w, float unslope, float (&o)[4]) {
    const unsigned wx = w.x, wy = w.y;
    const f16x2 a = __builtin_bit_cast(f16x2, wx), b = __builtin_bit_cast(f16x2, wy);
    const float v[4] = {(float)a[0], (float)a[1], (float)b[0], (float)b[1]};
#pragma unroll
    for (int e = 0; e < 4; e++) o[e] = v[e] < 0.f ? v[e] * unslope : v[e];
}

constexpr int kSxPeakStride = 32;
inline hipError_t sx_allow_big_lds(const void *kern, std::atomic<uint64_t> &done) {
    int dev = 0;
    if (hipGetDevice(&dev) != hipSuccess) return hipGetLastError();
    const uint64_t bit = 1ull << (dev & 63);
    if (done.load(std::memory_order_acquire) & bit) return hipSuccess;
    const hipError_t e = hipFuncSetAttribute(kern, hipFuncAttributeMaxDynamicSharedMemorySize, kSxMaxDynLds);
    if (e == hipSuccess) done.fetch_or(bit, std::memory_order_release);
    return e;
}
__device__ __forceinline__ void sx_publish_peak_at(unsigned *slots, int slot_idx, float pk, float *s_pk) {
#pragma unroll
    for (int o = 32; o > 0; o >>= 1) pk = __builtin_fmaxf(pk, __shfl_xor(pk, o, 64));
    __syncthreads();
    if ((threadIdx.x & 63) == 0) s_pk[threadIdx.x >> 6] = pk;
    __syncthreads();
    if (threadIdx.x == 0) {
        pk = __builtin_fmaxf(__builtin_fmaxf(s_pk[0], s_pk[1]), __builtin_fmaxf(s_pk[2], s_pk[3]));
        unsigned *slot = slots + (slot_idx & (kSxPeakSlots - 1)) * kSxPeakStride;
        const unsigned bits = __float_as_uint(pk);
        if (bits > __builtin_nontemporal_load(slot)) atomicMax(slot, bits);
    }
}
__device__ __forceinline__ void sx_publish_peak(unsigned *slots, int slot_idx, float pk) {
    __shared__ float s_pk[4];
#pragma unroll
    for (int o = 32; o > 0; o >>= 1) pk = __builtin_fmaxf(pk, __shfl_xor(pk, o, 64));
    if ((threadIdx.x & 63) == 0) s_pk[threadIdx.x >> 6] = pk;
    __syncthreads();
    if (threadIdx.x == 0) {
        pk = __builtin_fmaxf(__builtin_fmaxf(s_pk[0], s_pk[1]), __builtin_fmaxf(s_pk[2], s_pk[3]));
        unsigned *slot = slots + (slot_idx & (kSxPeakSlots - 1)) * kSxPeakStride;
        const unsigned bits = __float_as_uint(pk);
        if (bits > __builtin_nontemporal_load(slot)) atomicMax(slot, bits);
    }
}

__device__ __forceinline__ float tanh_nb(float v) {
    const float t = __builtin_fabsf(v), s = v * v;
    float p = 62.0f / 2835.0f;
    p = __builtin_fmaf(p, s, -17.0f / 315.0f);
    p = __builtin_fmaf(p, s, 2.0f / 15.0f);
    p = __builtin_fmaf(p, s, -1.0f / 3.0f);
    p = __builtin_fmaf(p * s, v, v);
    const float e = __builtin_amdgcn_exp2f(t * 2.8853900817779268f);
    float r = __builtin_fmaf(-2.0f, __builtin_amdgcn_rcpf(1.0f + e), 1.0f);
    r = __builtin_copysignf(r, v);
    return t < 0.3f ? p : r;
}
__device__ __forceinline__ float sigmoid_nb(float v) {
    return __builtin_amdgcn_rcpf(1.0f + __builtin_amdgcn_exp2f(-v * 1.4426950408889634f));
}

}
```

phoonnx_amd/csrc/vitsmi.hip:

```cpp
#include <climits>
#include <hip/hip_runtime.h>

#include <cmath>
#include <cstdarg>
#include <chrono>
#include <cstdio>
#include <cstring>
#include <mutex>
#include <string>
#include <vector>

#include "../../include/vitsmi.h"
#include "conv_geom.hpp"
#include "conv_sx_engine.hip.hpp"
#include "conv_sx_pair.hip.hpp"
#include "conv_sx_pair16.hip.hpp"
#include "attention16.hip.hpp"
#include "conv_sx_small.hip.hpp"
#include "delivery.hip.hpp"
#include "delivery_run.hip.hpp"
#include "fit.hip.hpp"
#include "shape.hip.hpp"
#include "kernels.hip.hpp"
#include "loudness.hip.hpp"
// ... 525 lines not shown

constexpr int kAttMaxHeadWidth = 128;
template <int DKB, int KH>
void launch_attention_t(hipStream_t st, dim3 grid, const float *qkv, float *att, const float *rel_k, const float *rel_v,
                        const int *len, int H, int T, int dk, int window, uint16_t *planes, unsigned *peak) {
    if (g_launch_name_on) snprintf(g_launch_name, sizeof g_launch_name, "attention_relpos_kernel<%d, %d>", DKB, KH);
    attention_relpos_kernel<DKB, KH><<<grid, 256 * KH, 0, st>>>(qkv, att, rel_k, rel_v, len, H, T, dk, window, planes, peak);
}
void launch_attention(hipStream_t st, int B, int T, int n_heads, int dk, int window, const float *qkv, float *att,
                      const float *rel_k, const float *rel_v, const int *len, int H, uint16_t *planes = nullptr,
                      unsigned *peak = nullptr, int kh = 0) {
    static const bool nosplit = std::getenv("VITSMI_ATT_NOSPLIT") != nullptr;
    const bool one_half = kh ? kh == 1 : nosplit;
    dim3 ag((T + 127) / 128, n_heads, B);
    const int dkb = (dk + 31) / 32;
#define VITSMI_ATT(DKB)                                                                                             \
    do {                                                                                                            \
        if (one_half) launch_attention_t<DKB, 1>(st, ag, qkv, att, rel_k, rel_v, len, H, T, dk, window, planes, peak); \
        else launch_attention_t<DKB, 2>(st, ag, qkv, att, rel_k, rel_v, len, H, T, dk, window, planes, peak);          \
    } while (0)
    switch (dkb) {
        case 1: VITSMI_ATT(1); break;
        case 2: VITSMI_ATT(2); break;
        case 3: VITSMI_ATT(3); break;
        default: VITSMI_ATT(4); break;
    }
#undef VITSMI_ATT
}

template <int DKS, int NS, int QT>
hipError_t launch_attention16_t(hipStream_t st, const Att16Args &a) {
    constexpr int lds = NS * 4 * (DKS * 2) * 1024 + 9 * DKS * 32 * 4 + 16 + 64 * QT * kAtt16RelPitch * 4;
    static std::atomic<uint64_t> done{0};
    if (lds > 64 * 1024)
        if (hipError_t e = sx_allow_big_lds(reinterpret_cast<const void *>(&attention_relpos16_kernel<DKS, NS, QT>), done)) return e;
    const int ntile = (a.T + 64 * QT - 1) / (64 * QT), npair = a.nh * a.B;
    if (g_launch_name_on) snprintf(g_launch_name, sizeof g_launch_name, "attention_relpos16_kernel<%d, %d, %d>", DKS, NS, QT);
    attention_relpos16_kernel<DKS, NS, QT><<<dim3(((npair + 7) / 8) * 8 * ntile), 256, lds, st>>>(a);
    return hipSuccess;
}
hipError_t launch_attention16(hipStream_t st, int B, int T, int n_heads, int dk, int window, const uint16_t *qkv_pl, float *att,
                              uint16_t *att_pl, const float *rel_k, const float *rel_v, const int *len, int H, unsigned *peak,
                              unsigned long long *prof = nullptr, int ns_arg = 0, int qt_arg = 0) {
    static const int env_ns = [] { const char *e = std::getenv("VITSMI_ATT16_NS"); return e ? std::atoi(e) : 0; }();
    static const int env_qt = [] { const char *e = std::getenv("VITSMI_ATT16_QT"); return e ? std::atoi(e) : 0; }();
    Att16Args a{};
    a.qkv_pl = qkv_pl;
    a.out = att;
    a.out_pl = att_pl;
    a.relk = rel_k;
    a.relv = rel_v;
    a.len = len;
    a.Hc = H;
    a.T = T;
    a.dk = dk;
    a.win = window;
    a.nh = n_heads;
    a.B = B;
    a.peak = att_pl ? peak : nullptr;
    a.prof = prof;
    const int ns = ns_arg ? ns_arg : (env_ns ? env_ns : 2), qt = qt_arg ? qt_arg : (env_qt ? env_qt : 1);
    if (dk == 32) return launch_attention16_t<1, 3, 1>(st, a);
    if (dk == 64) return launch_attention16_t<2, 3, 1>(st, a);
    if (qt == 2) return ns >= 3 ? launch_attention16_t<3, 3, 2>(st, a) : launch_attention16_t<3, 2, 2>(st, a);
    if (ns >= 4) return launch_attention16_t<3, 4, 1>(st, a);
    return ns == 3 ? launch_attention16_t<3, 3, 1>(st, a) : launch_attention16_t<3, 2, 1>(st, a);
}

void launch_durations(hipStream_t st, int B, int T, const float *logw, const int *len, float length_scale, const float *rows,
                      const float *token_rate, float *w_ceil, int *cum, int *y_len) {
    duration_kernel<<<B, 256, 0, st>>>(logw, len, length_scale, rows, token_rate, w_ceil, cum, y_len, T);
}

void launch_fit_weights(hipStream_t st, int B, int T, const float *logw, const int *len, float length_scale, const float *rows,
                        const float *token_rate, float *w) {
    fit_weight_kernel<<<dim3((T + 255) / 256, B), 256, 0, st>>>(logw, len, length_scale, rows, token_rate, w, T);
}

void launch_fit_durations(hipStream_t st, int B, int T, int G, const float *w, const int *len, const int *group, const int64_t *target,
                          const int *mode, float *w_ceil, int *cum, int *y_len, FitResult *res) {
    fit_duration_kernel<<<G, 256, 0, st>>>(w, len, group, target, mode, B, T, w_ceil, cum, y_len, res);
}

void launch_forced_durations(hipStream_t st, int B, int T, const int64_t *dur, const int *len, float *w_ceil, int *cum, int *y_len) {
    forced_duration_kernel<<<B, 256, 0, st>>>(dur, len, w_ceil, cum, y_len, T);
}

void launch_fill_normal_rows(hipStream_t st, int B, int channels, int T, float *out, const uint64_t *seeds, uint32_t stream,
                             const float *rows, int col) {
    fill_normal_rows_kernel<<<dim3((unsigned)(((T + 3) / 4 + 63) / 64), channels, B), 64, 0, st>>>(out, T, seeds, stream, rows, col);
}

void launch_fill_normal(hipStream_t st, float *out, int64_t n, uint64_t seed, uint64_t stream_id) {
    fill_normal_kernel<<<(unsigned)((n / 4 + 256) / 256), 256, 0, st>>>(out, n, seed, stream_id);
}

void launch_expand_prior(hipStream_t st, int B, int C, int T, int F, const float *m_p, const float *logs_p, int64_t bstride,
                         const int *cum, const int *len, const int *y_len, const float *noise, int64_t noise_stride,
                         float noise_scale, const float *rows, const uint64_t *seeds, float *z_p, int Fnoise) {
    expand_prior_strided_kernel<<<dim3((F + 255) / 256, (C + 3) / 4, B), 64, 0, st>>>(m_p, logs_p, bstride, cum, len, y_len, noise,
                                                                                     noise_stride, noise_scale, rows, seeds, z_p, C,
                                                                                     T, F, Fnoise);
}

size_t post_conv_lds(int C, int K) { return ((size_t)C * (256 + K - 1) + (size_t)C * K) * sizeof(float); }
void launch_post_conv(hipStream_t st, int B, int C, int K, int T, const float *x, const float *w, float *out, float slope,
                      const int *vlen, int hop) {
    const size_t lds = post_conv_lds(C, K);
    post_conv_tanh_kernel<<<dim3((T + 255) / 256, B), 256, lds, st>>>(x, w, out, C, K, T, slope, vlen, hop);
}

size_t post_conv_blocked_lds(int C, int K) { return (size_t)C * (256 + K - 1) * sizeof(float); }
void launch_post_conv_blocked(hipStream_t st, int B, int C, int K, int T, const float *x, const float *w, float *out, float slope,
                              const int *vlen, int hop, bool generic = false) {
    const size_t lds = post_conv_blocked_lds(C, K);
    if (K == 7 && !generic)
        post_conv_tanh_blocked_kernel<7><<<dim3((T + 255) / 256, B), 256, lds, st>>>(x, w, out, C, K, T, slope, vlen, hop);
    else
        post_conv_tanh_blocked_kernel<0><<<dim3((T + 255) / 256, B), 256, lds, st>>>(x, w, out, C, K, T, slope, vlen, hop);
}

void conv_sx_planar(Ctx &c, const ConvDesc &d, const uint16_t *x_pl, int T, float *out, uint16_t *out_pl, int flags,
                    SxOpt o = {}) {
    o.row_split = d.Cout;
    o.pl_rows = out_pl ? d.Cout : 0;
    conv_sx(c, d, x_pl, T, out, out_pl, SX_WN_RMW | flags, o);
}

void split_planes(Ctx &c, const float *x, uint16_t *pl, int C, int T, const int *len) {
    sx_split_planes_kernel<<<dim3((T + 255) / 256, C / 8, c.B), 256, 0, c.st>>>(x, (int64_t)C * T, T, len, pl, C, T, 1,
                                                                                range_slots(c.h, true));
    c.note(hipGetLastError());
    c.h->stats.total_launches++;
}

void fused_launch_end(Ctx &c, bool ev, const ConvDesc *const *members, int n, const ConvDesc &rec, int T, double fl, double by) {
    vits_stats &st = c.h->stats;
    if (ev) conv_event_end(c, true, fl, by, rec, T);
    for (int i = 0; i < n; i++) conv_account(c, *members[i], T);
    st.conv_launches -= n - 1;
    st.total_launches -= n - 1;
    st.sx_flops += fl;
    st.sx_bytes += by;
    st.sx_launches++;
}

bool sx_pair_ok(const vits_handle *h, const ConvDesc &c1, const ConvDesc &c2) {
    static const bool off = std::getenv("VITSMI_SX_NO_PAIR") != nullptr;
    return !off && h->gen_nprod == 2 && c1.f16 && c2.f16 && c1.rawin && c2.rawin && c1.cfg == c2.cfg && c1.ups == 1 &&
           c2.ups == 1 && c1.Cin == c1.Cout && c2.Cin == c2.Cout && c1.Cin == c2.Cin && c2.padL * 2 == (c2.K - 1) * c2.dil &&
           sx_pair_supported(c1.Cin, c1.cfg, c1.K, c1.dil, c2.K, c2.dil);
}

void conv_sx_pair(Ctx &c, const ConvDesc &c1, const ConvDesc &c2, const float *x, int T, float *out, int flags, float div,
                  float slope, bool chain = false) {
    SxPairArgs a{};
    a.xr = x;
    a.islope = slope;
    a.mslope = slope;
    a.T = T;
    a.wp1 = reinterpret_cast<const u32x4 *>(c.P(c1.w_off));
    a.wp2 = reinterpret_cast<const u32x4 *>(c.P(c2.w_off));
    a.bias1 = c.P(c1.b_off);
    a.bias2 = c.P(c2.b_off);
    a.wscale1 = c1.wscale;
    a.wscale2 = c2.wscale;
    a.out_raw = out;
    a.zeros = c.P(c.m.zeros_off);
    a.C = c1.Cin;
    a.K1 = c1.K;
    a.dil1 = c1.dil;
    a.pad1 = c1.padL;
    a.K2 = c2.K;
    a.dil2 = c2.dil;
    a.pad2 = c2.padL;
    a.flags = flags & (EPI_ACC | EPI_DIV);
    a.div = div;
    vits_handle *h = c.h;
    a.rag = c.rag_at(T);
    a.peak = range_slots(h, true);
#if SX_PAIR_PROF
    {
        static unsigned long long *rows = nullptr;
        static int idx = 0;
        if (!rows) {
            hipMalloc((void **)&rows, 64 * 8 * sizeof(unsigned long long));
            hipMemset(rows, 0, 64 * 8 * sizeof(unsigned long long));
        }
        if (h->stats.sx_launches == 0 || idx >= 64) idx = 0;
        a.prof = rows + (idx++ % 64) * 8;
        if (std::getenv("VITSMI_PAIR_PROF_DUMP") && idx == 1) {
            unsigned long long hrows[64 * 8];
            hipDeviceSynchronize();
            hipMemcpy(hrows, rows, sizeof hrows, hipMemcpyDeviceToHost);
            for (int r = 0; r < 64; r++)
                if (hrows[r * 8 + 7]) {
                    fprintf(stderr, "pairprof row %d wgs %llu:", r, hrows[r * 8 + 7]);
                    for (int i = 0; i < 7; i++) fprintf(stderr, " %.0f", (double)hrows[r * 8 + i] / (double)hrows[r * 8 + 7]);
                    fprintf(stderr, "\n");
                }
            hipMemset(rows, 0, sizeof hrows);
        }
    }
#endif
    const bool ev = conv_event_begin(c);
    c.note(launch_conv_sx_pair(a, c1.cfg, c.B, c.st, chain));
    const double wf = c.work_frac();
    const double fl = 2.0 * (c1.macs_per_t + c2.macs_per_t) * (double)T * c.B * wf;
    const double by = 4.0 * c.B * ((double)(c1.Cin + c1.Cout) * T + (double)(c2.Cin + c2.Cout) * T) * wf;
    const ConvDesc *const members[] = {&c1, &c2};
    fused_launch_end(c, ev, members, 2, c1, T, fl, by);
}

bool sx_pair16_ok(const vits_handle *h, const ConvDesc &c1, const ConvDesc &c2) {
    static const bool off = [] {
        const char *e = std::getenv("VITSMI_PAIR16");
        return (e && e[0] == '0') || std::getenv("VITSMI_SX_NO_PAIR") != nullptr;
    }();
    if (off || c1.Cin != c1.Cout || c2.Cin != c2.Cout || c1.Cin != c2.Cin || c1.ups != 1 || c2.ups != 1) return false;
    if (c1.padL * 2 != (c1.K - 1) * c1.dil || c2.padL * 2 != (c2.K - 1) * c2.dil) return false;
    const bool h1 = c1.h1 && c2.h1, f3 = c1.f16 && c2.f16 && c1.s16 && c2.s16 && !c1.rawin && !c2.rawin;
    if (!h1 && !f3) return false;
    if (c1.cfg != c2.cfg || c1.cfg != (c1.Cin == 64 ? 1 : 2)) return false;
    (void)h;
    return sx_pair16_plan(c1.Cin, h1 ? 1 : 2, c1.K, c1.dil, c2.K, c2.dil, nullptr) != 0;
}

static SxPair16Args sx_pair16_args(const ConvDesc &c1, const ConvDesc &c2, const float *A, const float *zeros, const uint16_t *x, int T,
                                   float *out_raw, uint16_t *out_pl, int flags, float div, float slope, SxRagged rag, unsigned *peak) {
    SxPair16Args a{};
    const int C = c1.Cin;
    const auto P = [A](int64_t off) { return off >= 0 ? A + off : nullptr; };
    a.xpl = x;
    a.x_bstride = (int64_t)3 * C * T;
    a.islope = a.mslope = a.oslope = slope;
    a.T = T;
    a.wp1 = reinterpret_cast<const u32x4 *>(P(c1.w_off));
    a.wp2 = reinterpret_cast<const u32x4 *>(P(c2.w_off));
    a.bias1 = P(c1.b_off);
    a.bias2 = P(c2.b_off);
    a.wscale1 = c1.wscale;
    a.wscale2 = c2.wscale;
    a.out_raw = out_raw;
    a.raw_bstride = (int64_t)C * T;
    a.out_pl = out_pl;
    a.pl_bstride = (int64_t)3 * C * T;
    a.zeros = zeros;
    a.K1 = c1.K; a.dil1 = c1.dil; a.pad1 = c1.padL;
    a.K2 = c2.K; a.dil2 = c2.dil; a.pad2 = c2.padL;
    a.flags = flags;
    a.div = div;
    a.rag = rag;
    a.peak = peak;
    return a;
}

void conv_sx_pair16(Ctx &c, const ConvDesc &c1, const ConvDesc &c2, const uint16_t *x, int T, float *out_raw, uint16_t *out_pl, int flags,
                    float div, float slope, bool chain) {
    const bool h1 = c1.h1;
    const int C = c1.Cin;
    vits_handle *h = c.h;
    const SxPair16Args a = sx_pair16_args(c1, c2, c.A, c.P(c.m.zeros_off), x, T, out_raw, out_pl, flags, div, slope, c.rag_at(T),
                                          range_slots(h, true));
    const double ebytes = h1 ? 2.0 : 4.0;
    const bool ev = conv_event_begin(c);
    c.note(launch_conv_sx_pair16(a, C, h1 ? 1 : 2, c.B, c.st, chain));
    const double fl = 2.0 * (c1.macs_per_t + c2.macs_per_t) * (double)T * c.B * c.work_frac();
    const double by = ebytes * c.B * ((double)(c1.Cin + c1.Cout) * T + (double)(c2.Cin + c2.Cout) * T) * c.work_frac();
    const ConvDesc *const members[] = {&c1, &c2};
    fused_launch_end(c, ev, members, 2, c1, T, fl, by);
}

bool sx_mrf_ok(const vits_handle *h, const UpStageDesc &stg) {
    const bool off = std::getenv("VITSMI_SX_MRF") == nullptr;
    const int n = (int)stg.rbs.size();
    if (off || n < 2 || n > 3) return false;
    int K1[3], d1[3], K2[3], d2[3];
    for (int j = 0; j < n; j++) {
        const auto &rb = stg.rbs[j];
        if (rb.type1 || rb.n != 2 || !sx_pair_ok(h, rb.c1[0], rb.c1[1]) || rb.c1[0].padL * 2 != (rb.c1[0].K - 1) * rb.c1[0].dil)
            return false;
        K1[j] = rb.c1[0].K;
        d1[j] = rb.c1[0].dil;
        K2[j] = rb.c1[1].K;
        d2[j] = rb.c1[1].dil;
    }
    return sx_mrf_geom(stg.rbs[0].c1[0].Cin, n, K1, d1, K2, d2, nullptr);
}

void conv_sx_mrf(Ctx &c, const UpStageDesc &stg, const float *x, int T, float *out, float slope) {
    const int n = (int)stg.rbs.size();
    SxPairArgs a{};
    a.xr = x;
    a.islope = slope;
    a.mslope = slope;
    a.T = T;
    a.out_raw = out;
    a.zeros = c.P(c.m.zeros_off);
    a.C = stg.rbs[0].c1[0].Cin;
    a.div = (float)n;
    a.nchain = n;
    double macs = 0, bytes = 0;
    const ConvDesc *members[6];
    for (int j = 0; j < n; j++) {
        const ConvDesc &c1 = stg.rbs[j].c1[0], &c2 = stg.rbs[j].c1[1];
        members[2 * j] = &c1;
        members[2 * j + 1] = &c2;
        auto &ch = a.ch[j];
        ch.wp1 = reinterpret_cast<const u32x4 *>(c.P(c1.w_off));
        ch.wp2 = reinterpret_cast<const u32x4 *>(c.P(c2.w_off));
        ch.bias1 = c.P(c1.b_off);
        ch.bias2 = c.P(c2.b_off);
        ch.wscale1 = c1.wscale;
        ch.wscale2 = c2.wscale;
        ch.K1 = c1.K;
        ch.dil1 = c1.dil;
        ch.K2 = c2.K;
        ch.dil2 = c2.dil;
        macs += c1.macs_per_t + c2.macs_per_t;
        bytes += 4.0 * ((double)(c1.Cin + c1.Cout) + (double)(c2.Cin + c2.Cout));
    }
    vits_handle *h = c.h;
    a.rag = c.rag_at(T);
    a.peak = range_slots(h, true);
    macs *= c.work_frac();
    bytes *= c.work_frac();
    const bool ev = conv_event_begin(c);
    c.note(launch_conv_sx_mrf(a, c.B, c.st));
    fused_launch_end(c, ev, members, 2 * n, stg.rbs[n - 1].c1[0], T, 2.0 * macs * (double)T * c.B, bytes * T * c.B);
}

void *pinned_get(vits_handle *h, size_t bytes) {
    PinnedPool &p = h->pin;
// ... 3691 lines not shown
    unsigned *dpk = D.fill<unsigned>((size_t)kSxPeakSlots * kSxPeakStride);
    TCHECK(D.err);
    const dim3 grid((T + 255) / 256, C / 8, B);
    sx_split_planes_kernel<<<grid, 256>>>(dx, (int64_t)CT, T, nullptr, dxp, C, T, mode);
    sx_block_kernel<<<grid, 256>>>(dimg, (int64_t)CT, T, nullptr, draw, C, T);
    sx_split_planes_kernel<<<grid, 256>>>(dsen, (int64_t)CT, T, nullptr, dop, C, T, mode);
    TCHECK(hipGetLastError());
    TCHECK(hipMemcpy(draw + n, graw.data(), G * 4, hipMemcpyHostToDevice));
    TCHECK(hipMemcpy(dop + n * 3, gpl.data(), G * 2, hipMemcpyHostToDevice));
    const int kflags = ((flags & VITS_P16_EPI_ACC) ? EPI_ACC : 0) | ((flags & VITS_P16_EPI_DIV) ? EPI_DIV : 0) |
                       ((flags & VITS_P16_EPI_RAW) ? P16_HAS_RAW : 0) | ((flags & VITS_P16_EPI_PLANES) ? P16_HAS_PL : 0);
    const SxRagged rag = dlen ? SxRagged{dlen, p->rag_add, p->rag_mul} : SxRagged{nullptr, 0, 0};
    SxPair16Args a = sx_pair16_args(d1, d2, dA, dA, dxp, T, draw, dop, kflags, p->div == 0.f ? 1.f : p->div, slope, rag, dpk);
    SxPair16Tile tile{};
    auto go = [&] { return launch_conv_sx_pair16(a, C, npl, B, nullptr, chain, &tile); };
    const bool name_was_on = g_launch_name_on;
    g_launch_name_on = true;
    g_launch_name[0] = 0;
    const hipError_t le = go();
    g_launch_name_on = name_was_on;
    if (le != hipSuccess) return fail(nullptr, VITS_E_DEVICE, "pair16 epilogue hook: launch_conv_sx_pair16: %s", hipGetErrorString(le));
    TCHECK(hipDeviceSynchronize());
    std::snprintf(p->kernel, sizeof p->kernel, "%s", g_launch_name);
    p->BN = tile.BN;
    p->BNo = tile.BNo;
    p->ovl = tile.ovl ? 1 : 0;
    if (p->out) {
        sx_unblock_kernel<<<grid, 256>>>(draw, nullptr, dout, C, T, mode);
        TCHECK(hipGetLastError());
        TCHECK(hipDeviceSynchronize());
        TCHECK(download(p->out, dout, n));
    }
    if (p->planes_out) {
        sx_unblock_kernel<<<grid, 256>>>(nullptr, dop, dout, C, T, mode);
        TCHECK(hipGetLastError());
        TCHECK(hipDeviceSynchronize());
        TCHECK(download(p->planes_out, dout, n));
    }
    if (p->x_seen) {
        sx_unblock_kernel<<<grid, 256>>>(nullptr, dxp, dout, C, T, mode);
        TCHECK(hipGetLastError());
        TCHECK(hipDeviceSynchronize());
        TCHECK(download(p->x_seen, dout, n));
        const float un = 1.f / slope;
        for (size_t i = 0; i < n; i++)
            if (p->x_seen[i] < 0.f) p->x_seen[i] *= un;
    }
    {
        std::vector<float> gr(G);
        std::vector<uint16_t> hp(n * 3 + G);
        TCHECK(download(gr.data(), draw + n, G));
        TCHECK(download(hp.data(), dop, hp.size()));
        bool ok = std::memcmp(gr.data(), graw.data(), G * 4) == 0 && std::memcmp(hp.data() + n * 3, gpl.data(), G * 2) == 0;
        for (int b = 0; b < B && ok; b++)
            for (size_t i = (size_t)npl * CT; i < 3 * CT && ok; i++) ok = hp[(size_t)b * 3 * CT + i] == 0;
        p->guard_ok = ok ? 1 : 0;
    }
    {
        std::vector<unsigned> slots((size_t)kSxPeakSlots * kSxPeakStride);
        TCHECK(download(slots.data(), dpk, slots.size()));
        unsigned top = 0;
        for (int s = 0; s < kSxPeakSlots; s++) top = std::max(top, slots[(size_t)s * kSxPeakStride]);
        std::memcpy(&p->peak, &top, 4);
    }
#if P16_PROF
    {
        const size_t nwg = 1 << 17;
        unsigned long long *dprof = D.fill<unsigned long long>(nwg * 8);
        TCHECK(D.err);
        a.prof = dprof;
        TCHECK(go());
        TCHECK(hipDeviceSynchronize());
        std::vector<unsigned long long> hp(nwg * 8);
        TCHECK(download(hp.data(), dprof, nwg * 8));
        double sum[7] = {0, 0, 0, 0, 0, 0, 0};
        unsigned long long nt = 0, wgs = 0;
        for (size_t w = 0; w < nwg; w++)
            if (hp[w * 8 + 7]) {
                wgs++;
                nt += hp[w * 8 + 7];
                for (int i = 0; i < 7; i++) sum[i] += (double)hp[w * 8 + i];
            }
        fprintf(stderr, "p16prof C %d npl %d K %d wgs %llu tiles %llu | x wait %.0f  barrier %.0f  phase1 %.0f  hand-over %.0f  phase2 %.0f  epilogue %.0f  drain %.0f (cycles per TILE)\n",
                C, npl, K, wgs, nt, sum[0] / nt, sum[1] / nt, sum[2] / nt, sum[3] / nt, sum[4] / nt, sum[5] / nt, sum[6] / nt);
        a.prof = nullptr;
    }
#endif
    if (p->ms_out) TCHECK(time_launches(10, go, p->ms_out));
    return VITS_OK;
}

int vits_test_conv_pair_sx(int device_id, const float *x, int B, int C, int T, const float *w1, const float *b1,
                           const float *w2, const float *b2, int K, int dil1, int dil2, int chain, float slope, float *out,
                           float *ms_out) {
    if (int rc = test_dev(device_id)) return rc;
    const int kern = (chain >> 1) & 3;
    const bool from_plane = (chain & 8) != 0;
    chain &= 1;
    if (kern) {
        vits_test_conv_pair16_epi_args e{};
        e.B = B, e.C = C, e.T = T, e.K = K, e.dil1 = dil1, e.dil2 = dil2, e.chain = chain;
        e.precision = kern == 2 ? VITS_SX_F16 : VITS_SX_F16X3;
        e.flags = from_plane ? VITS_P16_EPI_PLANES : VITS_P16_EPI_RAW;
        e.slope = slope, e.div = 1.f, e.sentinel = 0.f;
        e.x = x, e.w1 = w1, e.b1 = b1, e.w2 = w2, e.b2 = b2;
        (from_plane ? e.planes_out : e.out) = out;
        e.ms_out = ms_out;
        return vits_test_conv_pair16_epi(device_id, &e);
    }
    ConvDesc d1, d2;
    std::vector<float> arena;
    const TestPack o = sx_test_pack(SxPack::F16X2);
    std::string e = pack_test_conv(w1, b1, C, C, K, dil1, dil1 * (K - 1) / 2, 3, &d1, &arena, o);
    if (e.empty()) e = pack_test_conv(w2, b2, C, C, K, dil2, dil2 * (K - 1) / 2, 3, &d2, &arena, o);
    if (!e.empty()) return fail(nullptr, VITS_E_ARG, "%s", e.c_str());
    const size_t n = (size_t)B * C * T;
    DevBufs D;
    if (!d1.rawin || !d2.rawin || d1.cfg != d2.cfg || !sx_pair_supported(C, d1.cfg, d1.K, d1.dil, d2.K, d2.dil))
        return fail(nullptr, VITS_E_ARG, "this conv pair cannot run fused (C %d, kernel %d, dilation %d)", C, K, dil1);
    float *dA = D.up(arena.data(), arena.size());
    float *dx = D.up(x, n, 16);
    float *dxr = D.alloc<float>(n, 16);
    float *draw = D.fill<float>(n, 0, 16);
    float *dout = D.alloc<float>(n, 16);
    TCHECK(D.err);
    sx_block_kernel<<<dim3((T + 255) / 256, C / 8, B), 256>>>(dx, (int64_t)C * T, T, nullptr, dxr, C, T);
    SxPairArgs a{};
    a.xr = dxr;
    a.islope = a.mslope = slope;
    a.T = T;
    a.wp1 = reinterpret_cast<const u32x4 *>(dA + d1.w_off);
    a.wp2 = reinterpret_cast<const u32x4 *>(dA + d2.w_off);
    a.bias1 = d1.b_off >= 0 ? dA + d1.b_off : nullptr;
    a.bias2 = d2.b_off >= 0 ? dA + d2.b_off : nullptr;
    a.wscale1 = d1.wscale;
    a.wscale2 = d2.wscale;
    a.out_raw = draw;
    a.zeros = dA;
    a.C = C;
    a.K1 = d1.K; a.dil1 = d1.dil; a.pad1 = d1.padL;
    a.K2 = d2.K; a.dil2 = d2.dil; a.pad2 = d2.padL;
    a.div = 1.f;
    auto go = [&] { return launch_conv_sx_pair(a, d1.cfg, B, nullptr, chain != 0); };
    TCHECK(go());
    TCHECK(hipDeviceSynchronize());
    if (ms_out) TCHECK(time_launches(10, go, ms_out));
    sx_unblock_kernel<<<dim3((T + 255) / 256, C / 8, B), 256>>>(draw, nullptr, dout, C, T, 1);
    TCHECK(hipGetLastError());
    TCHECK(hipDeviceSynchronize());
    TCHECK(download(out, dout, n));
    return VITS_OK;
}

int vits_bench_conv1d_sx(int device_id, int B, int Cin, int Cout, int T, int K, int dil, int dbg, int iters,
                         float *ms_out) {
    if (int rc = test_dev(device_id)) return rc;
    std::vector<float> w((size_t)Cout * Cin * K), x((size_t)B * Cin * T);
    bench_fill(w, x);
    ConvDesc d;
    std::vector<float> arena;
    TestPack o = sx_test_pack((dbg & 64) ? SxPack::F16X1 : ((dbg & 128) ? SxPack::F16X2 : SxPack::BF16X3));
    o.sx.no_s16 = (dbg & (1 | 2 | 16 | 256)) != 0;
    std::string e = pack_test_conv(w.data(), nullptr, Cin, Cout, K, dil, dil * (K - 1) / 2, 3, &d, &arena, o);
    if (!e.empty()) return fail(nullptr, VITS_E_ARG, "%s", e.c_str());
    const size_t nx = x.size(), no = (size_t)B * Cout * T;
    DevBufs D;
    float *dA = D.up(arena.data(), arena.size());
    float *dx = D.up(x.data(), nx);
    uint16_t *dxp = D.alloc<uint16_t>(nx * 3);
    float *draw = D.alloc<float>(no);
    float *dres = D.fill<float>(no);
    uint16_t *dop = D.alloc<uint16_t>(no * 3);
    unsigned long long *dprof = (dbg & 16) ? D.fill<unsigned long long>(8) : nullptr;
    TCHECK(D.err);
    sx_split_planes_kernel<<<dim3((T + 255) / 256, Cin / 8, B), 256>>>(dx, (int64_t)Cin * T, T, nullptr, dxp, Cin, T,
                                                                       d.h1 ? 2 : (d.f16 ? 1 : 0));
    SxArgs a = sx_args(d, dA, dA, T);
    a.xp = reinterpret_cast<const u32x4 *>(dxp);
    a.out_pl = dop;
    a.oslope2 = 0.1f;
    a.flags = ((dbg & 1) ? DBG_NO_DMA : 0) | ((dbg & 2) ? DBG_NO_EPI : 0);
    if (dbg & 8) {
        a.flags |= EPI_RES;
        if (d.h1) {
            a.res_pl = reinterpret_cast<const uint16_t *>(dres);
            a.res_unslope = 10.f;
        } else {
            a.res = dres;
            a.out_raw = draw;
        }
    }
    if (d.rawin) {
        a.xr = dx;
        a.islope = 0.1f;
        a.out_pl = nullptr;
        a.out_raw = draw;
    }
    a.prof = dprof;
    auto go = [&] { return launch_conv_sx(a, d.cfg, B, nullptr, d.rawin, d.h1 ? 1 : (d.f16 ? 2 : 6)); };
    for (int i = 0; i < 2; i++) TCHECK(go());
    TCHECK(hipDeviceSynchronize());
    if (dprof) TCHECK(hipMemset(dprof, 0, 64));
    float ms = 0.f;
    TCHECK(time_launches(iters, go, &ms));
    if (ms_out) {
        ms_out[0] = ms;
        ms_out[1] = (float)d.cfg;
        ms_out[2] = 0.f;
        if (dprof) {
            unsigned long long hp[8];
            TCHECK(download(hp, dprof, 8));
            for (int i = 0; i < 5; i++) ms_out[3 + i] = hp[5] ? (float)((double)hp[i] / (double)hp[5]) : 0.f;
            ms_out[2] = hp[7] ? (float)((double)hp[6] / (double)hp[7] * 0.1) : 0.f;
        }
    }
    return VITS_OK;
}

int vits_test_attention(int device_id, const float *qkv, int B, int C, int T, int n_heads, const float *rel_k,
                        const float *rel_v, int window, const int64_t *lens, float *out) {
    if (int rc = test_dev(device_id)) return rc;
    if (window > 4 || C % n_heads) return fail(nullptr, VITS_E_ARG, "bad attention test arguments");
    int dk = C / n_heads;
    if (dk > kAttMaxHeadWidth) return fail(nullptr, VITS_E_ARG, "attention head width %d > %d is unsupported", dk, kAttMaxHeadWidth);
    size_t nq = (size_t)B * 3 * C * T, no = (size_t)B * C * T, nr = (size_t)(2 * window + 1) * dk;
    std::vector<int> l32(B);
    for (int b = 0; b < B; b++) l32[b] = (int)lens[b];
    DevBufs D;
    float *dq = D.up(qkv, nq);
    float *dout = D.alloc<float>(no);
    float *drk = D.up(rel_k, nr);
    float *drv = D.up(rel_v, nr);
    int *dlen = D.up(l32.data(), (size_t)B);
    TCHECK(D.err);
    launch_attention(nullptr, B, T, n_heads, dk, window, dq, dout, drk, drv, dlen, C);
    TCHECK(hipGetLastError());
    TCHECK(hipDeviceSynchronize());
    TCHECK(download(out, dout, no));
    return VITS_OK;
}

int vits_test_attention16(int device_id, const float *qkv, int B, int C, int T, int n_heads, const float *rel_k,
                          const float *rel_v, int window, const int64_t *lens, float *out, uint16_t *out_planes, int kernel,
                          int reps, float *ms_out) {
    if (int rc = test_dev(device_id)) return rc;
    if (window > 4 || C % n_heads || C % 8) return fail(nullptr, VITS_E_ARG, "bad attention test arguments");
    int dk = C / n_heads;
    if (kernel == 1 && !(dk % 32 == 0 && dk <= 96)) return fail(nullptr, VITS_E_ARG, "attention16 needs a head width of 32, 64 or 96");
    if (dk > kAttMaxHeadWidth) return fail(nullptr, VITS_E_ARG, "attention head width %d > %d is unsupported", dk, kAttMaxHeadWidth);
    size_t nq = (size_t)B * 3 * C * T, no = (size_t)B * C * T, nr = (size_t)(2 * window + 1) * dk;
    std::vector<int> l32(B);
    for (int b = 0; b < B; b++) l32[b] = (int)lens[b];
    DevBufs D;
    float *dq = D.up(qkv, nq);
    uint16_t *dqp = D.alloc<uint16_t>(nq * 3);
    uint16_t *dop = D.fill<uint16_t>(no * 3, 0xff);
    unsigned *dpk = D.fill<unsigned>((size_t)kSxPeakSlots * kSxPeakStride);
    float *dout = D.fill<float>(no, 0xff);
    float *drk = D.up(rel_k, nr);
    float *drv = D.up(rel_v, nr);
    int *dlen = D.up(l32.data(), (size_t)B);
    unsigned long long *dprof = nullptr;
    const int prof_wgs = ((n_heads * B + 7) / 8) * 8 * ((T + 63) / 64);
#if ATT16_PROF
    dprof = D.fill<unsigned long long>((size_t)prof_wgs * 4);
#endif
    TCHECK(D.err);
    sx_split_planes_kernel<<<dim3((T + 255) / 256, 3 * C / 8, B), 256>>>(dq, (int64_t)3 * C * T, T, nullptr, dqp, 3 * C, T, 1, dpk);
    auto go = [&] {
        if (kernel == 1) (void)launch_attention16(nullptr, B, T, n_heads, dk, window, dqp, dout, dop, drk, drv, dlen, C, dpk, dprof);
        else launch_attention(nullptr, B, T, n_heads, dk, window, dq, dout, drk, drv, dlen, C, dk % 8 == 0 ? dop : nullptr, dpk);
        return hipSuccess;
    };
    go();
    TCHECK(hipGetLastError());
    TCHECK(hipDeviceSynchronize());
    if (reps > 0 && ms_out) TCHECK(time_launches(reps, go, ms_out));
    if (dprof && kernel == 1) {
        std::vector<unsigned long long> hp((size_t)prof_wgs * 4);
        TCHECK(download(hp.data(), dprof, hp.size()));
        double d[3] = {0, 0, 0};
        unsigned long long t0 = ~0ull, t1 = 0;
        int n = 0;
        for (int w = 0; w < prof_wgs; w++) {
            if (!hp[w * 4 + 3]) continue;
            for (int k = 0; k < 3; k++) d[k] += (double)(hp[w * 4 + k + 1] - hp[w * 4 + k]);
            t0 = hp[w * 4] < t0 ? hp[w * 4] : t0;
            t1 = hp[w * 4 + 3] > t1 ? hp[w * 4 + 3] : t1;
            n++;
        }
        if (n) std::fprintf(stderr, "att16 stamps B=%d T=%d: %d workgroups; cycles prologue %.0f loop %.0f epilogue %.0f; first start -> last end %llu\n",
                            B, T, n, d[0] / n, d[1] / n, d[2] / n, t1 - t0);
    }
    TCHECK(download(out, dout, no));
    if (out_planes) TCHECK(download(out_planes, dop, no * 3));
    return VITS_OK;
}

int vits_test_attention_form(int device_id, vits_test_attention_form_args *p) {
    if (int rc = test_dev(device_id)) return rc;
    if (!p) return fail(nullptr, VITS_E_ARG, "no attention test arguments");
    const int B = p->B, C = p->C, T = p->T, n_heads = p->n_heads, window = p->window;
    if (B <= 0 || C <= 0 || T <= 0 || n_heads <= 0 || window < 0 || !p->rel_k || !p->rel_v || !p->lens)
        return fail(nullptr, VITS_E_ARG, "bad attention test arguments");
    if (window > 4) return fail(nullptr, VITS_E_ARG, "attention window %d > 4 is unsupported", window);
    if (C % n_heads) return fail(nullptr, VITS_E_ARG, "%d channels do not divide into %d heads", C, n_heads);
// ... 953 lines not shown
```

phoonnx_amd/session.py:

```python
import contextlib
import ctypes as C
import dataclasses
import time
from collections import namedtuple
from dataclasses import dataclass
from typing import Dict, List, Optional, Sequence

import numpy as np

from . import _ffi


class SessionError(RuntimeError):
    """Raised for every failure of the engine (onnxruntime raises its own
    InvalidArgument/RuntimeException at voice.py:374; callers there do not catch either)."""


class RangeError(SessionError):
    """VITS_E_RANGE: the f16x3 generator arithmetic met an activation beyond the range of its fp16 operand planes
    (|x| > 65504) or a non-finite value.  The engine reports this instead of returning clamped audio; `MiSession`
    (range_fallback=True, the default) then reopens the voice with the bf16x6 arithmetic (fp32 range) and repeats the
    call, so user code only sees this when the fallback is switched off or impossible (borrowed weight arena)."""


# ... 2164 lines not shown
    a.old_out, a.old_out2, a.sentinel = _ffi.ptr(old_out), _ffi.ptr(old_out2), CONV_EPI_SENTINEL
    a.out, a.out2, a.pl_rows, a.planes_out = _ffi.ptr(out), _ffi.ptr(o2), pl_rows, _ffi.ptr(pl)
    rc = lib.vits_test_conv1d_epi(device_id, C.byref(a))
    if rc != 0:
        raise SessionError(_ffi.last_error(None))
    return {"out": out, "out2": o2, "planes": pl, "kernel": a.kernel.decode(), "cfg": a.cfg_used, "ck": a.ck_used}


SX_EPI_FLAGS = {"res": 1, "acc": 2, "div": 4, "no_raw_store": 8}
SX_PRECISIONS = {"bf16x6": 0, "f16x3": 1, "f16": 2}


def test_conv1d_sx_epi(x, w, bias=None, flags=(), precision="f16x3", dil=1, pad_l=None, stride=1, force16=False, no_s16=False,
                       min_cfg=0, run_cfg=-1, res=None, res_is_x=False, res_planes=False, res_slope=1.0, old_out=None,
                       bias_b=None, div=1.0, oslope=1.0, oslope2=1.0, islope=1.0, raw=True, planes=False, lens=None,
                       rag_add=0, rag_mul=1, sentinel=CONV_EPI_SENTINEL, device_id=0):
    lib = _ffi.load()
    f32 = lambda a: None if a is None else np.ascontiguousarray(a, np.float32)
    x, w, bias, bias_b, res, old_out = (f32(a) for a in (x, w, bias, bias_b, res, old_out))
    B, Cin, T = x.shape
    Cout, K = (w.shape[1] if stride > 1 else w.shape[0]), w.shape[2]
    To = T * stride
    ln = None if lens is None else np.ascontiguousarray(lens, np.int64)
    for name, arr, shape in (("w", w, (Cin, Cout, K) if stride > 1 else (Cout, Cin, K)), ("bias", bias, (Cout,)),
                             ("res", res, (B, Cout, To)), ("old_out", old_out, (B, Cout, To)), ("lens", ln, (B,))):
        if arr is not None and arr.shape != shape:
            raise ValueError(f"{name} has shape {arr.shape}, the launch needs {shape}")
    if bias_b is not None and (bias_b.ndim != 2 or bias_b.shape[0] != B):
        raise ValueError(f"bias_b has shape {bias_b.shape}, the launch needs ({B}, stride)")
    out = np.empty((B, Cout, To), np.float32) if raw else None
    pl = np.empty((B, Cout, To), np.float32) if planes else None
    seen = np.empty((B, Cout, To), np.float32) if (res_planes and res is not None) else None
    a = _ffi.VitsTestConvSxEpiArgs()
    a.B, a.Cin, a.T, a.Cout, a.K, a.dil, a.stride = B, Cin, T, Cout, K, dil, stride
    a.pad_l = dil * (K - 1) // 2 if pad_l is None else pad_l
    a.precision, a.force16, a.no_s16, a.min_cfg, a.run_cfg = SX_PRECISIONS[precision], int(force16), int(no_s16), min_cfg, run_cfg
    a.flags = sum(SX_EPI_FLAGS[f] for f in flags)
    a.x, a.w, a.bias, a.res, a.old_out, a.bias_b, a.lens = (_ffi.ptr(v) for v in (x, w, bias, res, old_out, bias_b, ln))
    a.res_is_x, a.res_planes, a.res_slope = int(res_is_x), int(res_planes), res_slope
    a.bias_b_stride = 0 if bias_b is None else bias_b.shape[1]
    a.div, a.oslope, a.oslope2, a.islope = div, oslope, oslope2, islope
    a.rag_add, a.rag_mul, a.sentinel = rag_add, rag_mul, sentinel
    a.out, a.planes_out, a.res_seen = _ffi.ptr(out), _ffi.ptr(pl), _ffi.ptr(seen)
    rc = lib.vits_test_conv1d_sx_epi(device_id, C.byref(a))
    if rc != 0:
        raise SessionError(_ffi.last_error(None))
    return {"out": out, "planes": pl, "res_seen": seen, "kernel": a.kernel.decode(), "pack_cfg": a.pack_cfg, "run_cfg": a.run_cfg_used,
            "rawin": bool(a.rawin), "s16": bool(a.s16), "ck": a.ck, "peak": float(a.peak)}


def test_wn_gate(a, blocked=False, device_id=0):
    lib = _ffi.load()
    a = np.ascontiguousarray(a, np.float32)
    B, C2, T = a.shape
    if C2 % 2:
        raise ValueError("a holds the tanh rows and as many sigmoid rows")
    out = np.empty((B, C2 // 2, T), np.float32)
    rc = lib.vits_test_wn_gate(device_id, _ffi.ptr(a), B, C2 // 2, T, 1 if blocked else 0, _ffi.ptr(out))
    if rc != 0:
        raise SessionError(_ffi.last_error(None))
    return out


def test_cond_matvec(emb_g, sid, W, bias=None, device_id=0):
    lib = _ffi.load()
    emb_g = np.ascontiguousarray(emb_g, np.float32)
    W = np.ascontiguousarray(W, np.float32)
    b = None if bias is None else np.ascontiguousarray(bias, np.float32)
    sid = np.ascontiguousarray(sid, np.int64)
    if emb_g.ndim != 2 or W.ndim != 2 or W.shape[1] != emb_g.shape[1] or sid.ndim != 1 or (b is not None and b.shape != W.shape[:1]):
        raise ValueError("emb_g [n_speakers, gin], W [rows, gin], bias [rows], sid [B]")
    out = np.empty((len(sid), W.shape[0]), np.float32)
    rc = lib.vits_test_cond_matvec(device_id, _ffi.ptr(emb_g), emb_g.shape[0], emb_g.shape[1], _ffi.ptr(sid), len(sid),
                                   _ffi.ptr(W), _ffi.ptr(b), W.shape[0], _ffi.ptr(out))
    if rc != 0:
        raise SessionError(_ffi.last_error(None))
    return out


def test_conv1d_sx_gate(x, w, bias, g, dil=1, small=False, planes=False, device_id=0):
    lib = _ffi.load()
    x = np.ascontiguousarray(x, np.float32)
    B, Cin, T = x.shape
    C2, _, K = w.shape
    H = C2 // 2
    perm = np.concatenate([np.concatenate([np.arange(p, p + 32), H + np.arange(p, p + 32)]) for p in range(0, H, 32)])
    wp = np.ascontiguousarray(np.asarray(w, np.float32)[perm])
    bp = np.ascontiguousarray(np.asarray(bias, np.float32)[perm])
    gg = np.ascontiguousarray(g, np.float32)
    out = np.empty((B, H, T), np.float32)
    rc = lib.vits_test_conv1d_sx_gate(device_id, _ffi.ptr(x), B, Cin, T, _ffi.ptr(wp), _ffi.ptr(bp), _ffi.ptr(gg), C2, K, dil,
                                      (1 if small else 0) | (2 if planes else 0), _ffi.ptr(out))
    if rc != 0:
        raise SessionError(_ffi.last_error(None))
    return out


def test_conv_pair_sx(x, w1, b1, w2, b2, dil1=1, dil2=1, chain=False, slope=0.1, device_id=0, timed=False, kernel="pair",
                      from_plane=False):
    lib = _ffi.load()
    x = np.ascontiguousarray(x, np.float32)
    w1 = np.ascontiguousarray(w1, np.float32)
    w2 = np.ascontiguousarray(w2, np.float32)
    B, Cc, T = x.shape
    K = w1.shape[2]
    if w1.shape != (Cc, Cc, K) or w2.shape != (Cc, Cc, K):
        raise ValueError("both convs are C -> C with the same kernel size")
    b1 = None if b1 is None else np.ascontiguousarray(b1, np.float32)
    b2 = None if b2 is None else np.ascontiguousarray(b2, np.float32)
    out = np.empty_like(x)
    ms = C.c_float(0.0)
    rc = lib.vits_test_conv_pair_sx(device_id, _ffi.ptr(x), B, Cc, T, _ffi.ptr(w1), _ffi.ptr(b1), _ffi.ptr(w2),
                                    _ffi.ptr(b2), K, dil1, dil2,
                                    (1 if chain else 0) | ({"pair": 0, "pair16": 1, "pair16_f16": 2}[kernel] << 1) | (8 if from_plane else 0),
                                    float(slope), _ffi.ptr(out),
                                    C.byref(ms) if timed else None)
    if rc != 0:
        raise SessionError(_ffi.last_error(None))
    return (out, float(ms.value)) if timed else out


P16_EPI_FLAGS = {"acc": 1, "div": 2, "raw": 4, "planes": 8}


def test_conv_pair16_epi(x, w1, b1, w2, b2, flags=("raw",), dil1=1, dil2=1, chain=False, slope=0.1, precision="f16x3", div=1.0,
                         old_out=None, lens=None, rag_add=0, rag_mul=1, x_tail=None, sentinel=CONV_EPI_SENTINEL, device_id=0):
    lib = _ffi.load()
    f32 = lambda a: None if a is None else np.ascontiguousarray(a, np.float32)
    x, w1, b1, w2, b2, old_out, x_tail = (f32(a) for a in (x, w1, b1, w2, b2, old_out, x_tail))
    B, Cc, T = x.shape
    K = w1.shape[2]
    ln = None if lens is None else np.ascontiguousarray(lens, np.int64)
    for name, arr, shape in (("w1", w1, (Cc, Cc, K)), ("w2", w2, (Cc, Cc, K)), ("b1", b1, (Cc,)), ("b2", b2, (Cc,)),
                             ("old_out", old_out, (B, Cc, T)), ("x_tail", x_tail, (B, Cc, T)), ("lens", ln, (B,))):
        if arr is not None and arr.shape != shape:
            raise ValueError(f"{name} has shape {arr.shape}, the launch needs {shape}")
    out = np.empty((B, Cc, T), np.float32)
    pl = np.empty((B, Cc, T), np.float32) if "planes" in flags else None
    seen = np.empty((B, Cc, T), np.float32)
    a = _ffi.VitsTestConvPair16EpiArgs()
    a.B, a.C, a.T, a.K, a.dil1, a.dil2, a.chain = B, Cc, T, K, dil1, dil2, int(bool(chain))
    a.precision, a.flags = SX_PRECISIONS[precision], sum(P16_EPI_FLAGS[f] for f in flags)
    a.slope, a.div, a.sentinel = slope, div, sentinel
    a.x, a.w1, a.b1, a.w2, a.b2, a.old_out, a.x_tail, a.lens = (_ffi.ptr(v) for v in (x, w1, b1, w2, b2, old_out, x_tail, ln))
    a.rag_add, a.rag_mul = rag_add, rag_mul
    a.out, a.planes_out, a.x_seen = _ffi.ptr(out), _ffi.ptr(pl), _ffi.ptr(seen)
    rc = lib.vits_test_conv_pair16_epi(device_id, C.byref(a))
    if rc != 0:
        raise SessionError(_ffi.last_error(None))
    return {"out": out, "planes": pl, "x_seen": seen, "kernel": a.kernel.decode(), "BN": a.BN, "BNo": a.BNo, "ovl": bool(a.ovl),
            "peak": float(a.peak), "guard_ok": bool(a.guard_ok)}


def bench_conv1d_sx(B, Cin, Cout, T, K, dil=1, dbg=0, iters=20, device_id=0):
    lib = _ffi.load()
    res = np.zeros(8, np.float32)
    rc = lib.vits_bench_conv1d_sx(device_id, B, Cin, Cout, T, K, dil, dbg, iters,
                                  res.ctypes.data_as(_ffi.C.POINTER(_ffi.C.c_float)))
    if rc != 0:
        raise SessionError(_ffi.last_error(None))
    if dbg & 16:
        return float(res[0]), int(res[1]), [float(v) for v in res[3:8]] + [float(res[2])]
    return float(res[0]), int(res[1])


def test_conv_transpose1d(x, w, bias, stride, device_id=0, sx=False):
    lib = _ffi.load()
    x = np.ascontiguousarray(x, np.float32)
    w = np.ascontiguousarray(w, np.float32)
    B, Cin, T = x.shape
    _, Cout, K = w.shape
    b = None if bias is None else np.ascontiguousarray(bias, np.float32)
    out = np.empty((B, Cout, T * stride), np.float32)
    fn = lib.vits_test_conv_transpose1d_sx if sx else lib.vits_test_conv_transpose1d
    rc = fn(device_id, _ffi.ptr(x), B, Cin, T, _ffi.ptr(w), _ffi.ptr(b), Cout, K, -stride if sx == "f16" else stride,
            _ffi.ptr(out))
    if rc != 0:
        raise SessionError(_ffi.last_error(None))
    return out


def test_attention16(qkv, n_heads, rel_k, rel_v, lens, device_id=0, kernel=1, planes=False, reps=0):
    lib = _ffi.load()
    qkv = np.ascontiguousarray(qkv, np.float32)
    B, C3, T = qkv.shape
    Cc = C3 // 3
    rel_k = np.ascontiguousarray(rel_k, np.float32)
    rel_v = np.ascontiguousarray(rel_v, np.float32)
    window = (rel_k.shape[0] - 1) // 2
    lens = np.ascontiguousarray(lens, np.int64)
    out = np.empty((B, Cc, T), np.float32)
    opl = np.empty((B, 3, Cc // 8, T, 8), np.uint16) if planes else None
    ms = (C.c_float * 1)()
    rc = lib.vits_test_attention16(device_id, _ffi.ptr(qkv), B, Cc, T, n_heads, _ffi.ptr(rel_k), _ffi.ptr(rel_v), window,
                                   _ffi.ptr(lens), _ffi.ptr(out), _ffi.ptr(opl) if planes else None, int(kernel), int(reps), ms)
    if rc != 0:
        raise SessionError(_ffi.last_error(None))
    res = (out,)
    if planes:
        res += (opl,)
    if reps > 0:
        res += (float(ms[0]),)
    return res[0] if len(res) == 1 else res


def test_attention_form(qkv, n_heads, rel_k, rel_v, lens, kernel=16, want_out=True, want_planes=True, ns=0, qt=0, kh=0,
                        qkv_planes=None, device_id=0):
    lib = _ffi.load()
    qkv = np.ascontiguousarray(qkv, np.float32)
    B, C3, T = qkv.shape
    Cc = C3 // 3
    rel_k = np.ascontiguousarray(rel_k, np.float32)
    rel_v = np.ascontiguousarray(rel_v, np.float32)
    window = (rel_k.shape[0] - 1) // 2
    lens = np.ascontiguousarray(lens, np.int64)
    if C3 != 3 * Cc or n_heads <= 0 or Cc % n_heads or lens.shape != (B,):
        raise ValueError(f"q|k|v {qkv.shape} with {n_heads} heads and lens {lens.shape}")
    dk = Cc // n_heads
    if rel_k.shape != (2 * window + 1, dk) or rel_v.shape != rel_k.shape:
        raise ValueError(f"relative embeddings {rel_k.shape} / {rel_v.shape}, head width {dk}")
    qp = None
    if qkv_planes is not None:
        qp = np.ascontiguousarray(qkv_planes, np.uint16)
        if C3 % 8 or qp.shape != (B, 3, C3 // 8, T, 8):
            raise ValueError(f"q|k|v planes {qp.shape}, the launch needs {(B, 3, C3 // 8, T, 8)}")
    out = np.empty((B, Cc, T), np.float32)
    opl = np.empty((B, 3, Cc // 8, T, 8), np.uint16) if Cc % 8 == 0 else None
    a = _ffi.VitsTestAttentionFormArgs()
    a.kernel, a.qkv, a.qkv_planes = int(kernel), _ffi.ptr(qkv), _ffi.ptr(qp)
    a.B, a.C, a.T, a.n_heads, a.window = B, Cc, T, n_heads, window
    a.rel_k, a.rel_v, a.lens = _ffi.ptr(rel_k), _ffi.ptr(rel_v), _ffi.ptr(lens)
    a.want_out, a.want_planes, a.ns, a.qt, a.kh = int(bool(want_out)), int(bool(want_planes)), int(ns), int(qt), int(kh)
    a.out, a.out_planes = _ffi.ptr(out), _ffi.ptr(opl)
    rc = lib.vits_test_attention_form(device_id, C.byref(a))
    if rc != 0:
        raise SessionError(_ffi.last_error(None))
    return {"out": out, "planes": opl, "peak": float(a.peak), "kernel": a.kernel_name.decode()}


def test_attention(qkv, n_heads, rel_k, rel_v, lens, device_id=0):
    lib = _ffi.load()
    qkv = np.ascontiguousarray(qkv, np.float32)
    B, C3, T = qkv.shape
    Cc = C3 // 3
    rel_k = np.ascontiguousarray(rel_k, np.float32)
    rel_v = np.ascontiguousarray(rel_v, np.float32)
    window = (rel_k.shape[0] - 1) // 2
    lens = np.ascontiguousarray(lens, np.int64)
    out = np.empty((B, Cc, T), np.float32)
    rc = lib.vits_test_attention(device_id, _ffi.ptr(qkv), B, Cc, T, n_heads, _ffi.ptr(rel_k), _ffi.ptr(rel_v), window,
                                 _ffi.ptr(lens), _ffi.ptr(out))
    if rc != 0:
        raise SessionError(_ffi.last_error(None))
    return out


def _resample_test_args(x, lens, in_rate, out_rate):
    x = np.ascontiguousarray(x, np.float32)
    lens = np.ascontiguousarray(lens, np.int64)
    if x.ndim != 2 or lens.shape != (x.shape[0],):
        raise SessionError(f"x must be [B, S] and lens [B], got {x.shape} / {lens.shape}")
    L, M, _ = resample_plan(in_rate, out_rate)
    return x, lens, L, M


def test_resample(x, lens, in_rate, out_rate, device_id=0):
    x, lens, L, M = _resample_test_args(x, lens, in_rate, out_rate)
    B, S = x.shape
    counts = -(-np.clip(lens, 0, S) * L // M)
    y = np.full((B, max(1, int(counts.max()))), np.nan, np.float32)
    rc = _ffi.load().vits_test_resample(device_id, _ffi.ptr(x), _ffi.ptr(lens), B, S, int(in_rate), int(out_rate), _ffi.ptr(y),
                                        y.shape[1])
    if rc != 0:
        raise SessionError(f"vits_test_resample failed [{rc}]: {_ffi.last_error(None)}")
    return y, counts


def test_resample_rows(x, lens, in_rate, out_rates, device_id=0):
    x = np.ascontiguousarray(x, np.float32)
    lens = np.ascontiguousarray(lens, np.int64)
    rates = np.asarray([int(r or 0) for r in out_rates], np.int32)
    if x.ndim != 2 or lens.shape != (x.shape[0],) or rates.shape != lens.shape:
        raise SessionError(f"x must be [B, S], lens and out_rates [B], got {x.shape} / {lens.shape} / {rates.shape}")
    B, S = x.shape
    cap = -(-S * max(int(rates.max()), int(in_rate)) // max(int(in_rate), 1)) + 1
    buf = np.full(B * cap, np.nan, np.float32)
    counts = np.zeros(B, np.int64)
    rc = _ffi.load().vits_test_resample_rows(device_id, _ffi.ptr(x), _ffi.ptr(lens), B, S, int(in_rate), _ffi.ptr(rates), _ffi.ptr(buf),
                                             buf.size, _ffi.ptr(counts))
    if rc != 0:
        raise SessionError(f"vits_test_resample_rows failed [{rc}]: {_ffi.last_error(None)}")
    S_out = int(counts.max())
    if S_out == 0:
        return np.zeros((B, 1), np.float32), counts
    return buf[:B * S_out].reshape(B, S_out).copy(), counts


def warp_token(semitones):
    step, c, Kh = C.c_int64(), C.c_int64(), C.c_int32()
    rc = _ffi.load().vits_warp_token(float(semitones), C.byref(step), C.byref(c), C.byref(Kh))
    if rc != 0:
        raise SessionError(f"vits_warp_token failed [{rc}]: {_ffi.last_error(None)}")
    return step.value, c.value, Kh.value


def warp_plan(durations, semitones, hop):
# ... 585 lines not shown
```

Measured before the change: 143.2 million.

## Specialize fused conv pair kernel for interior tiles and use mixed-FMA fp16 split

Splits the fused conv-pair kernel body into a template with an interior flag. Tiles whose whole halo lies inside the valid range take a path that drops the clamping and bounds masks on loads, stores and activations. The fp16 two-plane split now uses v_fma_mixlo/hi and v_max3 to compute the residual plane and the peak in fewer instructions. Test hooks check that the new split gives bit-identical results to the old one. The cost is two instantiations per configuration, which adds code size and may change register pressure.

```diff
diff --git a/include/vitsmi.h b/include/vitsmi.h
--- a/include/vitsmi.h
+++ b/include/vitsmi.h
@@ -456,6 +456,24 @@
 int vits_test_conv_pair_sx(int device_id, const float *x, int B, int C, int T, const float *w1, const float *b1,
                            const float *w2, const float *b2, int K, int dil1, int dil2, int chain, float slope, float *out,
                            float *ms_out);
+enum { VITS_PAIR_EPI_ACC = 1, VITS_PAIR_EPI_DIV = 2 };
+typedef struct {
+    int B, C, T, K, dil1, dil2, chain;
+    int flags;
+    float slope, div;
+    const float *x;
+    const float *w1, *b1, *w2, *b2;
+    const int64_t *lens;
+    const float *out_init;
+    float *out;
+    char kernel[128];
+    int BNo;
+} vits_test_conv_pair_sx_epi_args;
+int vits_test_conv_pair_sx_epi(int device_id, vits_test_conv_pair_sx_epi_args *a);
+int vits_test_split_identity(const float *x, int64_t n, uint16_t *h1_old, uint16_t *h1_fused);
+int64_t vits_test_split_identity_sweep(uint32_t first, uint64_t count, uint32_t *first_bad);
+int vits_test_split_forms(int device_id, const float *x, int n, float slope, int form, uint16_t *h0, uint16_t *h1, float *pk,
+                          float *rec);
 enum { VITS_P16_EPI_ACC = 1, VITS_P16_EPI_DIV = 2, VITS_P16_EPI_RAW = 4, VITS_P16_EPI_PLANES = 8 };
 typedef struct {
     int B, C, T, K, dil1, dil2, chain;
diff --git a/phoonnx_amd/_ffi.py b/phoonnx_amd/_ffi.py
--- a/phoonnx_amd/_ffi.py
+++ b/phoonnx_amd/_ffi.py
@@ -63,6 +63,13 @@
                [("rag_add", C.c_int), ("rag_mul", C.c_int)] + \
                [(n, C.c_void_p) for n in ("out", "planes_out", "x_seen", "ms_out")] + [("kernel", C.c_char * 128)] + \
                [(n, C.c_int) for n in ("BN", "BNo", "ovl")] + [("peak", C.c_float), ("guard_ok", C.c_int)]
+
+
+class VitsTestConvPairSxEpiArgs(C.Structure):
+    _fields_ = [(n, C.c_int) for n in ("B", "C", "T", "K", "dil1", "dil2", "chain", "flags")] + \
+               [(n, C.c_float) for n in ("slope", "div")] + \
+               [(n, C.c_void_p) for n in ("x", "w1", "b1", "w2", "b2", "lens", "out_init", "out")] + \
+               [("kernel", C.c_char * 128), ("BNo", C.c_int)]
 
 
 class VitsTestAttentionFormArgs(C.Structure):
@@ -205,7 +212,7 @@
     "vits_test_stream_pack_trimmed",
     "vits_test_layernorm", "vits_test_dds", "vits_test_cf_pre", "vits_test_rqs_inverse", "vits_test_ea_logw",
     "vits_test_conv1d_epi", "vits_test_wn_gate", "vits_test_cond_matvec", "vits_test_conv1d_sx_epi",
-    "vits_test_conv_pair16_epi", "vits_test_attention_form",
+    "vits_test_conv_pair16_epi", "vits_test_attention_form", "vits_test_conv_pair_sx_epi", "vits_test_split_forms", "vits_test_split_identity", "vits_test_split_identity_sweep",
 ]
 
 
@@ -410,6 +417,11 @@
     lib.vits_test_conv1d_epi.argtypes = [C.c_int, C.POINTER(VitsTestConvEpiArgs)]
     lib.vits_test_conv1d_sx_epi.argtypes = [C.c_int, C.POINTER(VitsTestConvSxEpiArgs)]
     lib.vits_test_conv_pair16_epi.argtypes = [C.c_int, C.POINTER(VitsTestConvPair16EpiArgs)]
+    lib.vits_test_conv_pair_sx_epi.argtypes = [C.c_int, C.POINTER(VitsTestConvPairSxEpiArgs)]
+    lib.vits_test_split_identity.argtypes = [vp, C.c_int64, vp, vp]
+    lib.vits_test_split_identity_sweep.argtypes = [C.c_uint32, C.c_uint64, C.POINTER(C.c_uint32)]
+    lib.vits_test_split_identity_sweep.restype = C.c_int64
+    lib.vits_test_split_forms.argtypes = [C.c_int, vp, C.c_int, C.c_float, C.c_int, vp, vp, vp, vp]
     lib.vits_test_attention_form.argtypes = [C.c_int, C.POINTER(VitsTestAttentionFormArgs)]
     lib.vits_test_wn_gate.argtypes = [C.c_int, vp, C.c_int, C.c_int, C.c_int, C.c_int, vp]
     lib.vits_test_cond_matvec.argtypes = [C.c_int, vp, C.c_int, C.c_int, vp, C.c_int, vp, vp, C.c_int, vp]
diff --git a/phoonnx_amd/csrc/conv_sx_pair.hip.hpp b/phoonnx_amd/csrc/conv_sx_pair.hip.hpp
--- a/phoonnx_amd/csrc/conv_sx_pair.hip.hpp
+++ b/phoonnx_amd/csrc/conv_sx_pair.hip.hpp
@@ -67,14 +67,17 @@
 #ifndef SX_PAIR_ST_SC1
 #define SX_PAIR_ST_SC1 0
 #endif
+#ifndef SX_PAIR_INTERIOR
+#define SX_PAIR_INTERIOR 1
+#endif
 #ifndef SX_PAIR_ONE_READ64
 #define SX_PAIR_ONE_READ64 1
 #endif
 #ifndef SX_PAIR_ONE_READ32
 #define SX_PAIR_ONE_READ32 1
 #endif
-template <int MW, int NW, int WM, int WN, int EPI, bool CHAIN, int NCH = 1>
-__global__ __launch_bounds__(256, (NW == 2 && !SX_PAIR_EARLY_ACC && NCH == 1) ? SX_PAIR_WGS32 : 2) void conv_sx_pair_kernel(SxPairArgs a) {
+template <int MW, int NW, int WM, int WN, int EPI, bool CHAIN, int NCH, bool INTR>
+__device__ __forceinline__ void conv_sx_pair_body(const SxPairArgs &a, const int b, const int t0, const int TV, float &pk) {
     constexpr int BN = NW * WN * 32, NH = NW / 2;
     static_assert(NCH == 1 || (CHAIN && NW == 2 && (EPI & EPI_ACC) == 0), "fused chains: 32 channels, no external running sum");
     constexpr bool ONE_READ = NW == 4 ? SX_PAIR_ONE_READ64 != 0 : SX_PAIR_ONE_READ32 != 0;
@@ -91,20 +94,13 @@
     const int wave = __builtin_amdgcn_readfirstlane(tid >> 6);
     const int wm = wave / WN, wn = wave % WN;
     const int l31 = lane & 31, hi = lane >> 5;
-    const int wg_xcd = blockIdx.x & 7, wg_seq = blockIdx.x >> 3;
-    const int tile_nb = __builtin_amdgcn_readfirstlane(sx_xcd_tile(wg_seq, wg_xcd, a.xgs));
-    if (tile_nb >= a.NT * a.B) return;
-    const int b = tile_nb / a.NT, t0 = (tile_nb - b * a.NT) * a.BNo;
     const int t1 = t0 - a.pad2;
     const int T = a.T, LW = a.LW1;
-    const int TV = __builtin_amdgcn_readfirstlane(sx_valid_cols(a.rag, b, T));
-    if (t0 >= TV) return;
     const uint32_t lds0 = (uint32_t)(uintptr_t)lds_sx;
     const uint32_t XB = a.x_bytes;
     const char *wbase1 = reinterpret_cast<const char *>(a.wp1) + wm * (MW * NPW * 1024);
     const char *wbase2 = reinterpret_cast<const char *>(a.wp2) + wm * (MW * NPW * 1024);
     const float *xrb = a.xr + (int64_t)b * a.C * T;
-    float pk = 0.f;
 
     struct ASet {
         u32x4 fa[2];
@@ -127,6 +123,11 @@
                 const int tl = t < 0 ? 0 : (t < T ? t : T - 1);
 #pragma unroll
                 for (int q = 0; q < 4; q++) {
+                    if constexpr (INTR && EARLY) {
+                        const char *rowb = reinterpret_cast<const char *>(base + (int64_t)((row0 >> 3) + q) * T * 8);
+                        dst[rr][j][q] = __builtin_bit_cast(f32x4, global_read128<0>(((uint32_t)t * 8u + 4u * (uint32_t)hi) * 4u, rowb));
+                        continue;
+                    }
                     const float *p = base + ((int64_t)((row0 >> 3) + q) * T + tl) * 8 + 4 * hi;
                     if constexpr (EARLY) dst[rr][j][q] = __builtin_bit_cast(f32x4, global_read128_v<0>(p));
                     else dst[rr][j][q] = *reinterpret_cast<const f32x4 *>(p);
@@ -191,7 +192,7 @@
             const int c = hin[it] ? h - g * HW : 0;
             const int col = c < pad1 ? c : c + 256;
             const int t = t1 - pad1 + col;
-            hok[it] = hin[it] && t >= 0 && t < TV;
+            hok[it] = hin[it] && (INTR || (t >= 0 && t < TV));
             hp[it] = xrb + (hok[it] ? ((int64_t)g * T + t) * 8 : (int64_t)0);
             hlds[it] = lds0 + (uint32_t)(g >> 1) * XB + (uint32_t)((g & 1) * LW + col) * 16u;
         }
@@ -218,12 +219,12 @@
                         float v[8];
 #pragma unroll
                         for (int e = 0; e < 8; e++) {
-                            const float x = hok[it] ? __uint_as_float(hst[it][e >> 2][e & 3]) : 0.f;
-                            v[e] = fmaxf(x, x * isl);
+                            const float x = (INTR || hok[it]) ? __uint_as_float(hst[it][e >> 2][e & 3]) : 0.f;
+                            v[e] = lrelu_max(x, isl);
                         }
                         unsigned p0[4], p1[4];
 #pragma unroll
-                        for (int e = 0; e < 4; e++) split2h_pair_pk(v[2 * e], v[2 * e + 1], p0[e], p1[e], pk);
+                        for (int e = 0; e < 4; e++) sx_pair_split(v[2 * e], v[2 * e + 1], p0[e], p1[e], pk);
                         ds_write128(hlds[it], u32x4{p0[0], p0[1], p0[2], p0[3]});
                         ds_write128(hlds[it] + (uint32_t)(2 * LW) * 16u, u32x4{p1[0], p1[1], p1[2], p1[3]});
                     }
@@ -231,18 +232,18 @@
             }
             const int col = (wn * NW + n) * 32 + l31;
             const int t = t1 + col;
-            const bool ok = t >= 0 && t < TV;
+            const bool ok = INTR || (t >= 0 && t < TV);
 #pragma unroll
             for (int q = 0; q < 4; q++) {
                 float v[4];
 #pragma unroll
                 for (int e = 0; e < 4; e++) {
                     const float x = ok ? pre[n / 2][n % 2][q][e] : 0.f;
-                    v[e] = fmaxf(x, x * isl);
+                    v[e] = lrelu_max(x, isl);
                 }
                 unsigned wa[2], wb[2];
-                split2h_pair_pk(v[0], v[1], wa[0], wa[1], pk);
-                split2h_pair_pk(v[2], v[3], wb[0], wb[1], pk);
+                sx_pair_split(v[0], v[1], wa[0], wa[1], pk);
+                sx_pair_split(v[2], v[3], wb[0], wb[1], pk);
                 const int g = 4 * wm + q;
                 const uint32_t cell = lds0 + (uint32_t)(g >> 1) * XB + (uint32_t)((g & 1) * LW + pad1 + col) * 16u + 8u * hi;
                 asm volatile("ds_write_b64 %0, %1" ::"v"(cell), "v"(u32x2{wa[0], wb[0]}) : "memory");
@@ -264,7 +265,7 @@
             const int t = t1 - a.pad1 + col;
             xkh[it] = kh;
             xcol[it] = col;
-            xrok[it] = it < nxc && kh < 2 && t >= 0 && t < TV;
+            xrok[it] = it < nxc && kh < 2 && (INTR || (t >= 0 && t < TV));
             xroff[it] = xrok[it] ? (uint32_t)(((int64_t)kh * T + t) * 32) : 0u;
         }
         static_for<MAXCH>([&](auto CH) {
@@ -300,11 +301,11 @@
 #pragma unroll
                     for (int e = 0; e < 8; e++) {
                         const float x = xrok[it] ? __uint_as_float(xst[ch][it][e >> 2][e & 3]) : 0.f;
-                        v[e] = fmaxf(x, x * isl);
+                        v[e] = lrelu_max(x, isl);
                     }
                     unsigned p0[4], p1[4];
 #pragma unroll
-                    for (int e = 0; e < 4; e++) split2h_pair_pk(v[2 * e], v[2 * e + 1], p0[e], p1[e], pk);
+                    for (int e = 0; e < 4; e++) sx_pair_split(v[2 * e], v[2 * e + 1], p0[e], p1[e], pk);
                     const uint32_t ad = lds0 + (uint32_t)ch * XB + (uint32_t)(xkh[it] * LW + xcol[it]) * 16u;
                     ds_write128(ad, u32x4{p0[0], p0[1], p0[2], p0[3]});
                     ds_write128(ad + (uint32_t)(2 * LW) * 16u, u32x4{p1[0], p1[1], p1[2], p1[3]});
@@ -580,7 +581,7 @@
         for (int n = 0; n < NW; n++) {
             const int col = (wn * NW + n) * 32 + l31;
             const int t = t1 + col;
-            const bool live = t >= 0 && t < TV;
+            const bool live = INTR || (t >= 0 && t < TV);
 #pragma unroll
             for (int q = 0; q < 4; q++) {
                 float o[4];
@@ -597,8 +598,8 @@
                     o[e] = live ? fmaxf(v, v * msl) : 0.f;
                 }
                 unsigned wa[2], wb[2];
-                split2h_pair_pk(o[0], o[1], wa[0], wa[1], pk);
-                split2h_pair_pk(o[2], o[3], wb[0], wb[1], pk);
+                sx_pair_split(o[0], o[1], wa[0], wa[1], pk);
+                sx_pair_split(o[2], o[3], wb[0], wb[1], pk);
                 const int g = 4 * wm + q;
                 const uint32_t cell = ylds + (uint32_t)(g >> 1) * YC + ((uint32_t)(g & 1) * LW2 + (uint32_t)(col + a.pad2)) * 16u + 8u * hi;
                 asm volatile("ds_write_b64 %0, %1" ::"v"(cell), "v"(u32x2{wa[0], wb[0]}) : "memory");
@@ -646,10 +647,14 @@
 #pragma unroll
                 for (int j = 0; j < 2; j++) {
                     const int t = t1 + (wn * NW + rr * 2 + j) * 32 + l31;
-                    const int tl = t < 0 ? 0 : (t < T ? t : T - 1);
-#pragma unroll
-                    for (int q = 0; q < 4; q++)
-                        adl[j][q] = *reinterpret_cast<const f32x4 *>(rawb + ((int64_t)((row0 >> 3) + q) * T + tl) * 8 + 4 * hi);
+                    const int tl = INTR ? t : (t < 0 ? 0 : (t < T ? t : T - 1));
+#pragma unroll
+                    for (int q = 0; q < 4; q++) {
+                        if constexpr (INTR)
+                            adl[j][q] = *reinterpret_cast<const f32x4 *>(reinterpret_cast<const char *>(rawb + (int64_t)((row0 >> 3) + q) * T * 8) +
+                                                                         ((uint32_t)t * 8u + 4u * (uint32_t)hi) * 4u);
+                        else adl[j][q] = *reinterpret_cast<const f32x4 *>(rawb + ((int64_t)((row0 >> 3) + q) * T + tl) * 8 + 4 * hi);
+                    }
                 }
             }
 #pragma unroll
@@ -657,7 +662,7 @@
                 const int n = rr * 2 + j;
                 const int col = (wn * NW + n) * 32 + l31;
                 const int t = t1 + col;
-                const bool kept = !(col < a.pad2 || col >= a.pad2 + a.BNo || t >= TV);
+                const bool kept = !(col < a.pad2 || col >= a.pad2 + a.BNo || (!INTR && t >= TV));
                 if constexpr (NCH == 1) {
                     if (!kept) continue;
                 }
@@ -687,7 +692,10 @@
                         asm volatile("global_store_dwordx4 %0, %1, off sc1" ::"v"(sp), "v"(sv) : "memory");
                     }
 #else
-                    *reinterpret_cast<f32x4 *>(rawb + ((int64_t)((row0 >> 3) + q) * T + t) * 8 + 4 * hi) = v;
+                    if constexpr (INTR)
+                        *reinterpret_cast<f32x4 *>(reinterpret_cast<char *>(rawb + (int64_t)((row0 >> 3) + q) * T * 8) +
+                                                   ((uint32_t)t * 8u + 4u * (uint32_t)hi) * 4u) = v;
+                    else *reinterpret_cast<f32x4 *>(rawb + ((int64_t)((row0 >> 3) + q) * T + t) * 8 + 4 * hi) = v;
 #endif
                 }
             }
@@ -702,6 +710,21 @@
         atomicAdd(a.prof + 7, 1ull);
     }
 #endif
+}
+
+template <int MW, int NW, int WM, int WN, int EPI, bool CHAIN, int NCH = 1>
+__global__ __launch_bounds__(256, (NW == 2 && !SX_PAIR_EARLY_ACC && NCH == 1) ? SX_PAIR_WGS32 : 2) void conv_sx_pair_kernel(SxPairArgs a) {
+    const int wg_xcd = blockIdx.x & 7, wg_seq = blockIdx.x >> 3;
+    const int tile_nb = __builtin_amdgcn_readfirstlane(sx_xcd_tile(wg_seq, wg_xcd, a.xgs));
+    if (tile_nb >= a.NT * a.B) return;
+    const int b = tile_nb / a.NT, t0 = (tile_nb - b * a.NT) * a.BNo;
+    const int TV = __builtin_amdgcn_readfirstlane(sx_valid_cols(a.rag, b, a.T));
+    if (t0 >= TV) return;
+    const int xl = t0 - a.pad2 - a.pad1;
+    const bool interior = SX_PAIR_INTERIOR != 0 && xl >= 0 && xl + a.LW1 <= TV;
+    float pk = 0.f;
+    if (interior) conv_sx_pair_body<MW, NW, WM, WN, EPI, CHAIN, NCH, true>(a, b, t0, TV, pk);
+    else conv_sx_pair_body<MW, NW, WM, WN, EPI, CHAIN, NCH, false>(a, b, t0, TV, pk);
     if (a.peak) sx_publish_peak(a.peak, (int)blockIdx.x, pk);
 }
 
diff --git a/phoonnx_amd/csrc/sx_split.hip.hpp b/phoonnx_amd/csrc/sx_split.hip.hpp
--- a/phoonnx_amd/csrc/sx_split.hip.hpp
+++ b/phoonnx_amd/csrc/sx_split.hip.hpp
@@ -33,6 +33,35 @@
 __device__ __forceinline__ void split2h_pair_pk(float x, float y, unsigned &w0, unsigned &w1, float &pk) {
     pk = __builtin_fmaxf(pk, __builtin_fmaxf(__builtin_fabsf(x), __builtin_fabsf(y)));
     split2h_pair(x, y, w0, w1);
+}
+__device__ __forceinline__ void split2h_pair_pk_mix(float x, float y, unsigned &w0, unsigned &w1, float &pk) {
+    asm("v_max3_f32 %0, %0, |%1|, |%2|" : "+v"(pk) : "v"(x), "v"(y));
+    x = __builtin_amdgcn_fmed3f(x, -65504.f, 65504.f);
+    y = __builtin_amdgcn_fmed3f(y, -65504.f, 65504.f);
+    w0 = cvt_pk_f16(x, y);
+    const sxf32x2 t = sxf32x2{x, y} * 2048.f;
+    const float c = -2048.f;
+    unsigned r;
+    asm("v_fma_mixlo_f16 %0, %1, %2, %3 op_sel_hi:[1,0,0]" : "=v"(r) : "v"(w0), "v"(c), "v"(t.x));
+    asm("v_fma_mixhi_f16 %0, %1, %2, %3 op_sel:[1,0,0] op_sel_hi:[1,0,0]" : "+v"(r) : "v"(w0), "v"(c), "v"(t.y));
+    w1 = r;
+}
+#ifndef SX_PAIR_MIX
+#define SX_PAIR_MIX 1
+#endif
+__device__ __forceinline__ void sx_pair_split(float x, float y, unsigned &w0, unsigned &w1, float &pk) {
+#if SX_PAIR_MIX
+    split2h_pair_pk_mix(x, y, w0, w1, pk);
+#else
+    split2h_pair_pk(x, y, w0, w1, pk);
+#endif
+}
+
+__device__ __forceinline__ float lrelu_max(float x, float slope) {
+    const float m = x * slope;
+    float r;
+    asm("v_max_f32 %0, %1, %2" : "=v"(r) : "v"(x), "v"(m));
+    return r;
 }
 __device__ __forceinline__ unsigned cvt1h_pair_pk(float x, float y, float &pk) {
     pk = __builtin_fmaxf(pk, __builtin_fmaxf(__builtin_fabsf(x), __builtin_fabsf(y)));
diff --git a/phoonnx_amd/csrc/vitsmi.hip b/phoonnx_amd/csrc/vitsmi.hip
--- a/phoonnx_amd/csrc/vitsmi.hip
+++ b/phoonnx_amd/csrc/vitsmi.hip
@@ -701,21 +701,22 @@
            sx_pair_supported(c1.Cin, c1.cfg, c1.K, c1.dil, c2.K, c2.dil);
 }
 
-void conv_sx_pair(Ctx &c, const ConvDesc &c1, const ConvDesc &c2, const float *x, int T, float *out, int flags, float div,
-                  float slope, bool chain = false) {
+static SxPairArgs sx_pair_args(const ConvDesc &c1, const ConvDesc &c2, const float *A, const float *zeros, const float *x, int T, float *out,
+                               int flags, float div, float slope, SxRagged rag, unsigned *peak) {
     SxPairArgs a{};
+    const auto P = [A](int64_t off) { return off >= 0 ? A + off : nullptr; };
     a.xr = x;
     a.islope = slope;
     a.mslope = slope;
     a.T = T;
-    a.wp1 = reinterpret_cast<const u32x4 *>(c.P(c1.w_off));
-    a.wp2 = reinterpret_cast<const u32x4 *>(c.P(c2.w_off));
-    a.bias1 = c.P(c1.b_off);
-    a.bias2 = c.P(c2.b_off);
+    a.wp1 = reinterpret_cast<const u32x4 *>(P(c1.w_off));
+    a.wp2 = reinterpret_cast<const u32x4 *>(P(c2.w_off));
+    a.bias1 = P(c1.b_off);
+    a.bias2 = P(c2.b_off);
     a.wscale1 = c1.wscale;
     a.wscale2 = c2.wscale;
     a.out_raw = out;
-    a.zeros = c.P(c.m.zeros_off);
+    a.zeros = zeros;
     a.C = c1.Cin;
     a.K1 = c1.K;
     a.dil1 = c1.dil;
@@ -725,9 +726,15 @@
     a.pad2 = c2.padL;
     a.flags = flags & (EPI_ACC | EPI_DIV);
     a.div = div;
+    a.rag = rag;
+    a.peak = peak;
+    return a;
+}
+
+void conv_sx_pair(Ctx &c, const ConvDesc &c1, const ConvDesc &c2, const float *x, int T, float *out, int flags, float div,
+                  float slope, bool chain = false) {
     vits_handle *h = c.h;
-    a.rag = c.rag_at(T);
-    a.peak = range_slots(h, true);
+    SxPairArgs a = sx_pair_args(c1, c2, c.A, c.P(c.m.zeros_off), x, T, out, flags, div, slope, c.rag_at(T), range_slots(h, true));
 #if SX_PAIR_PROF
     {
         static unsigned long long *rows = nullptr;
@@ -4725,6 +4732,109 @@
     return VITS_OK;
 }
 
+int vits_test_conv_pair_sx_epi(int device_id, vits_test_conv_pair_sx_epi_args *p) {
+    if (int rc = test_dev(device_id)) return rc;
+    if (!p) return fail(nullptr, VITS_E_ARG, "no arguments");
+    const auto bad = [](const char *why) { return fail(nullptr, VITS_E_ARG, "pair epilogue hook: %s", why); };
+    const int B = p->B, C = p->C, T = p->T, K = p->K;
+    if (B < 1 || C < 1 || T < 1 || K < 1 || p->dil1 < 1 || p->dil2 < 1 || !p->x || !p->w1 || !p->w2 || !p->out) return bad("bad shape or missing tensor");
+    if (p->flags & ~(VITS_PAIR_EPI_ACC | VITS_PAIR_EPI_DIV)) return bad("unknown flag");
+    if ((p->flags & VITS_PAIR_EPI_ACC) && !p->out_init) return bad("acc without out_init (the accumulate operand is the raw tensor's previous contents)");
+    if (p->lens)
+        for (int b = 0; b < B; b++)
+            if (p->lens[b] < 0 || p->lens[b] > T) return bad("lens outside [0, T]");
+    ConvDesc d1, d2;
+    std::vector<float> arena;
+    const TestPack o = sx_test_pack(SxPack::F16X2);
+    std::string e = pack_test_conv(p->w1, p->b1, C, C, K, p->dil1, p->dil1 * (K - 1) / 2, 3, &d1, &arena, o);
+    if (e.empty()) e = pack_test_conv(p->w2, p->b2, C, C, K, p->dil2, p->dil2 * (K - 1) / 2, 3, &d2, &arena, o);
+    if (!e.empty()) return fail(nullptr, VITS_E_ARG, "%s", e.c_str());
+    if (!d1.rawin || !d2.rawin || d1.cfg != d2.cfg || !sx_pair_supported(C, d1.cfg, d1.K, d1.dil, d2.K, d2.dil))
+        return fail(nullptr, VITS_E_ARG, "this conv pair cannot run fused (C %d, kernel %d, dilations %d, %d)", C, K, p->dil1, p->dil2);
+    const size_t n = (size_t)B * C * T;
+    std::vector<int> l32(B);
+    for (int b = 0; b < B; b++) l32[b] = p->lens ? (int)p->lens[b] : T;
+    DevBufs D;
+    float *dA = D.up(arena.data(), arena.size());
+    float *dx = D.up(p->x, n, 16);
+    float *dxr = D.alloc<float>(n, 16);
+    float *dimg = p->out_init ? D.up(p->out_init, n, 16) : D.fill<float>(n, 0, 16);
+    float *draw = D.alloc<float>(n, 16);
+    float *dout = D.alloc<float>(n, 16);
+    int *dlen = p->lens ? D.up(l32.data(), (size_t)B) : nullptr;
+    TCHECK(D.err);
+    const dim3 grid((T + 255) / 256, C / 8, B);
+    sx_block_kernel<<<grid, 256>>>(dx, (int64_t)C * T, T, nullptr, dxr, C, T);
+    sx_block_kernel<<<grid, 256>>>(dimg, (int64_t)C * T, T, nullptr, draw, C, T);
+    TCHECK(hipGetLastError());
+    const int kflags = ((p->flags & VITS_PAIR_EPI_ACC) ? EPI_ACC : 0) | ((p->flags & VITS_PAIR_EPI_DIV) ? EPI_DIV : 0);
+    const SxRagged rag = dlen ? SxRagged{dlen, 0, 1} : SxRagged{nullptr, 0, 0};
+    const SxPairArgs a = sx_pair_args(d1, d2, dA, dA, dxr, T, draw, kflags, p->div == 0.f ? 1.f : p->div, p->slope, rag, nullptr);
+    const bool name_was_on = g_launch_name_on;
+    g_launch_name_on = true;
+    g_launch_name[0] = 0;
+    const hipError_t le = launch_conv_sx_pair(a, d1.cfg, B, nullptr, p->chain != 0);
+    g_launch_name_on = name_was_on;
+    if (le != hipSuccess) return fail(nullptr, VITS_E_DEVICE, "pair epilogue hook: launch_conv_sx_pair: %s", hipGetErrorString(le));
+    TCHECK(hipDeviceSynchronize());
+    std::snprintf(p->kernel, sizeof p->kernel, "%s", g_launch_name);
+    p->BNo = 256 - (d2.K - 1) * d2.dil;
+    sx_unblock_kernel<<<grid, 256>>>(draw, nullptr, dout, C, T, 1);
+    TCHECK(hipGetLastError());
+    TCHECK(hipDeviceSynchronize());
+    TCHECK(download(p->out, dout, n));
+    return VITS_OK;
+}
+
+static inline void split_identity_one(float x, uint16_t *o, uint16_t *f) {
+    const float v = std::fmin(std::fmax(x, -kF16Max), kF16Max);
+    const _Float16 h0 = (_Float16)v;
+    const _Float16 a = (_Float16)((v - (float)h0) * 2048.f);
+    const _Float16 b = (_Float16)std::fmaf((float)h0, -2048.f, v * 2048.f);
+    *o = __builtin_bit_cast(uint16_t, a);
+    *f = __builtin_bit_cast(uint16_t, b);
+}
+int vits_test_split_identity(const float *x, int64_t n, uint16_t *h1_old, uint16_t *h1_fused) {
+    if (!x || n < 0 || !h1_old || !h1_fused) return fail(nullptr, VITS_E_ARG, "split identity: missing array");
+    for (int64_t i = 0; i < n; i++) split_identity_one(x[i], h1_old + i, h1_fused + i);
+    return VITS_OK;
+}
+int64_t vits_test_split_identity_sweep(uint32_t first, uint64_t count, uint32_t *first_bad) {
+    int64_t bad = 0;
+    for (uint64_t k = 0; k < count; k++) {
+        const uint32_t bits = first + (uint32_t)k;
+        uint16_t o, f;
+        split_identity_one(__builtin_bit_cast(float, bits), &o, &f);
+        const bool nan_o = (o & 0x7fffu) > 0x7c00u, nan_f = (f & 0x7fffu) > 0x7c00u;
+        if (o != f && !(nan_o && nan_f)) {
+            if (bad == 0 && first_bad) *first_bad = bits;
+            bad++;
+        }
+    }
+    return bad;
+}
+
+int vits_test_split_forms(int device_id, const float *x, int n, float slope, int form, uint16_t *h0, uint16_t *h1, float *pk, float *rec) {
+    if (int rc = test_dev(device_id)) return rc;
+    if (!x || n < 2 || (n & 1) || !(slope > 0.f) || slope > 1.f || form < 0 || form > 1 || !h0 || !h1 || !pk || !rec)
+        return fail(nullptr, VITS_E_ARG, "split forms hook: n even and >= 2, 0 < slope <= 1, form 0 or 1, every output given");
+    DevBufs D;
+    float *dx = D.up(x, (size_t)n);
+    uint16_t *d0 = D.alloc<uint16_t>((size_t)n), *d1 = D.alloc<uint16_t>((size_t)n);
+    float *dpk = D.alloc<float>((size_t)n / 2), *drec = D.alloc<float>((size_t)n);
+    TCHECK(D.err);
+    const unsigned blocks = (unsigned)((n / 2 + 255) / 256);
+    if (form == 0) split_forms_kernel<0><<<blocks, 256>>>(dx, n, slope, 1.f / slope, d0, d1, dpk, drec);
+    else split_forms_kernel<1><<<blocks, 256>>>(dx, n, slope, 1.f / slope, d0, d1, dpk, drec);
+    TCHECK(hipGetLastError());
+    TCHECK(hipDeviceSynchronize());
+    TCHECK(download(h0, d0, (size_t)n));
+    TCHECK(download(h1, d1, (size_t)n));
+    TCHECK(download(pk, dpk, (size_t)n / 2));
+    TCHECK(download(rec, drec, (size_t)n));
+    return VITS_OK;
+}
+
 int vits_bench_conv1d_sx(int device_id, int B, int Cin, int Cout, int T, int K, int dil, int dbg, int iters,
                          float *ms_out) {
     if (int rc = test_dev(device_id)) return rc;
diff --git a/phoonnx_amd/session.py b/phoonnx_amd/session.py
--- a/phoonnx_amd/session.py
+++ b/phoonnx_amd/session.py
@@ -2340,6 +2340,48 @@
             "peak": float(a.peak), "guard_ok": bool(a.guard_ok)}
 
 
+def test_split_forms(x, slope=0.1, form="pair", device_id=0):
+    lib = _ffi.load()
+    x = np.ascontiguousarray(x, np.float32)
+    if x.ndim != 1 or x.size < 2 or x.size % 2:
+        raise ValueError("x: one dimension, an even number of values")
+    n = x.size
+    h0, h1 = np.empty(n, np.uint16), np.empty(n, np.uint16)
+    pk, rec = np.empty(n // 2, np.float32), np.empty(n, np.float32)
+    rc = lib.vits_test_split_forms(device_id, _ffi.ptr(x), n, float(slope), {"engine": 0, "pair": 1}[form], _ffi.ptr(h0), _ffi.ptr(h1),
+                                   _ffi.ptr(pk), _ffi.ptr(rec))
+    if rc != 0:
+        raise SessionError(_ffi.last_error(None))
+    return {"h0": h0.view(np.float16), "h1": h1.view(np.float16), "pk": pk, "rec": rec}
+
+
+PAIR_EPI_FLAGS = {"acc": 1, "div": 2}
+
+
+def test_conv_pair_sx_epi(x, w1, b1, w2, b2, flags=(), dil1=1, dil2=1, chain=False, slope=0.1, div=1.0, out_init=None, lens=None,
+                          device_id=0):
+    lib = _ffi.load()
+    f32 = lambda a: None if a is None else np.ascontiguousarray(a, np.float32)
+    x, w1, b1, w2, b2, out_init = (f32(a) for a in (x, w1, b1, w2, b2, out_init))
+    B, Cc, T = x.shape
+    K = w1.shape[2]
+    ln = None if lens is None else np.ascontiguousarray(lens, np.int64)
+    for name, arr, shape in (("w1", w1, (Cc, Cc, K)), ("w2", w2, (Cc, Cc, K)), ("b1", b1, (Cc,)), ("b2", b2, (Cc,)),
+                             ("out_init", out_init, (B, Cc, T)), ("lens", ln, (B,))):
+        if arr is not None and arr.shape != shape:
+            raise ValueError(f"{name} has shape {arr.shape}, the launch needs {shape}")
+    out = np.empty((B, Cc, T), np.float32)
+    a = _ffi.VitsTestConvPairSxEpiArgs()
+    a.B, a.C, a.T, a.K, a.dil1, a.dil2, a.chain = B, Cc, T, K, dil1, dil2, int(bool(chain))
+    a.flags = sum(PAIR_EPI_FLAGS[f] for f in flags)
+    a.slope, a.div = slope, div
+    a.x, a.w1, a.b1, a.w2, a.b2, a.lens, a.out_init, a.out = (_ffi.ptr(v) for v in (x, w1, b1, w2, b2, ln, out_init, out))
+    rc = lib.vits_test_conv_pair_sx_epi(device_id, C.byref(a))
+    if rc != 0:
+        raise SessionError(_ffi.last_error(None))
+    return {"out": out, "kernel": a.kernel.decode(), "BNo": a.BNo}
+
+
 def bench_conv1d_sx(B, Cin, Cout, T, K, dil=1, dbg=0, iters=20, device_id=0):
     lib = _ffi.load()
     res = np.zeros(8, np.float32)
```

New measurement: 144.6 million (median of 6 runs). 1.0% higher.
